# creare-com/pydem

Hardware: AMD Instinct MI355X
Metric: Mcells/s (slope+aspect+UCA+TWI end-to-end) per tile; % HBM roofline (higher is better)
Workload: dtype f64

## Files before the change

pydem_amd/csrc/internal.h:

```cpp
#pragma once
#include <hip/hip_runtime.h>
#include <stdint.h>
#include <stdio.h>
#include <stdlib.h>
#include <string>
#include <vector>
#include <utility>
#include <initializer_list>
#include "../../include/pydem_hip.h"

void pydem_set_error(const char *fmt, ...);
#define HIP_TRY(expr)                                                                          \
    do {                                                                                       \
        hipError_t e_ = (expr);                                                                \
        if (e_ != hipSuccess) {                                                                \
            pydem_set_error("%s:%d: %s -> %s", __FILE__, __LINE__, #expr, hipGetErrorString(e_)); \
            return -1;                                                                         \
        }                                                                                      \
    } while (0)
#define PYDEM_TRY(expr)            \
    do {                           \
        int r_ = (expr);           \
        if (r_ != 0) return r_;    \
    } while (0)

__host__ __device__ constexpr int fe1r(int k) { return k == 1 || k == 2 ? -1 : (k == 5 || k == 6 ? 1 : 0); }
__host__ __device__ constexpr int fe1c(int k) { return k == 0 || k == 7 ? 1 : (k == 3 || k == 4 ? -1 : 0); }
__host__ __device__ constexpr int fe2r(int k) { return k <= 3 ? -1 : 1; }
__host__ __device__ constexpr int fe2c(int k) { return (k == 0 || k == 1 || k == 6 || k == 7) ? 1 : -1; }

struct RowTab {
    double dX, dY;
    double hyp;
    double thA;
    double thB;
    double rdX, rdY, rhyp;
};

struct PitGraph {
    int32_t *raw_src = nullptr, *raw_dst = nullptr; double *raw_w = nullptr;
    int64_t raw_cap = 0, n_raw = 0;
    int64_t n_edges = 0, sorted_cap = 0;
    int32_t *src = nullptr, *dst = nullptr; double *w = nullptr;
    int32_t *in_src = nullptr, *in_dst = nullptr; double *in_w = nullptr;
    void *sort_buf = nullptr; size_t sort_bytes = 0;
};

struct TileBlock { void **slot; size_t bytes; bool cached; };

struct pydem_tile {
    int64_t n = 0, m = 0, NN = 0;
    int device = 0;
    hipStream_t stream = nullptr;
    hipStream_t stream2 = nullptr;
    hipEvent_t ev_fork = nullptr, ev_join = nullptr, ev_snap = nullptr;
    hipEvent_t ev[8] = {};
    double *elev = nullptr, *mag = nullptr, *dir = nullptr, *prop = nullptr, *uca = nullptr, *twi = nullptr;
    double *weight = nullptr, *uca_w = nullptr;
    uint8_t *flats = nullptr, *edge_todo = nullptr, *edge_done = nullptr, *flat0 = nullptr;
    int8_t *section = nullptr;
    bool have[PYDEM_FIELD_COUNT] = {};
    double *dX = nullptr, *dY = nullptr, *dX2 = nullptr, *dY2 = nullptr;
    RowTab *rowtab = nullptr;
    double *sec_theta = nullptr;
    double *row_area = nullptr;
    std::vector<double> h_dX, h_dY, h_dX2, h_dY2;
    bool spacing_set = false;
    int stencil_exact_only = 0;
    bool elev_f32 = false;
    int elev_dtype = 0;
    uint8_t *todo_work = nullptr;
    double *contrib = nullptr;
    uint32_t *cinfo = nullptr;
    int32_t *queue[2] = {nullptr, nullptr}, *labels = nullptr, *flatlist = nullptr;
    int32_t *counters = nullptr;
    int32_t *h_counters = nullptr;
    PitGraph pits;
    int32_t *estamp = nullptr; double *edelta = nullptr, *p_delta = nullptr, *s_data = nullptr;
    uint8_t *p_flags = nullptr, *s_flags = nullptr;
    int32_t eepoch = 0;
    int32_t *eseed = nullptr;
    bool edge_clean = false;
    bool einc_compact = false;
    void *nd_rec = nullptr; size_t nd_bytes = 0; int32_t nd = 0;
    int64_t circular_cells = -1;
    int64_t einc_round = 0;
    bool einc_ready = false;
    std::vector<std::pair<int, int64_t>> watch;
    size_t watch_built = 0;
    bool cond_live = false;
    bool cond_pending = false;
    int32_t cond_nw = 0, cond_nan_cap = 0;
    void *cond_mem = nullptr; size_t cond_bytes = 0;
    void *cond_node = nullptr, *cond_edge = nullptr; double *cond_slot = nullptr;
    int32_t *cond_q0 = nullptr, *cond_q1 = nullptr, *cond_nanq = nullptr, *cond_cnt = nullptr;
    void *cb_mem[3] = {nullptr, nullptr, nullptr}; size_t cb_bytes[3] = {0, 0, 0};
    double *h_strip_d = nullptr; uint8_t *h_strip_f = nullptr; size_t h_strip_cap = 0;
    void *h_stage = nullptr; size_t h_stage_bytes = 0;
    int32_t etodo_prev = 0;
    double *line_stage = nullptr;
    void *lines_stage = nullptr; size_t lines_bytes = 0;
    bool graph_valid = false;
    int flats_state = 0;
    int64_t find_flats_full = 0, find_flats_patch = 0, find_flats_elided = 0;
    bool pit_stash_live = false;
    pydem_options graph_opt = {};
    double *dd_out = nullptr; int32_t *dd_queue = nullptr; uint8_t *dd_mask = nullptr;
    double *ra_seed = nullptr;
    double *fa_mult = nullptr, *fa_cap = nullptr, *fa_inflow = nullptr;
    int32_t *sn_recv = nullptr; uint8_t *sn_code = nullptr;
    uint8_t *ta_sc = nullptr;
    int32_t *dd_ctr = nullptr, *dd_h_ctr = nullptr;
    hipEvent_t dd_ev[2] = {nullptr, nullptr};
    void *scratch = nullptr; size_t scratch_bytes = 0;
    std::vector<pydem_depression> depr;
    std::vector<TileBlock> blocks;
    int64_t device_bytes = 0;
    pydem_timings tm = {};
};

struct ArenaLease {
    int device = -1;
    void *arena = nullptr;
    char *base = nullptr; size_t bytes = 0, off = 0, want = 0;
    std::vector<void *> extra;
    bool held = false;
    ~ArenaLease();
};
int arena_acquire(int device, ArenaLease *L);
void *arena_take(ArenaLease *L, size_t bytes);

int ensure_fields(pydem_tile *t, std::initializer_list<int> fields);
void *plane_take(int device, size_t bytes);
void plane_give(int device, void *q);
hipError_t dev_malloc(void **p, size_t bytes);
void dev_free(void *p);
void devmem_release_all();
struct DevTemp {
    void *p = nullptr;
    ~DevTemp() { dev_free(p); }
    int alloc(size_t bytes) { if (bytes == 0) bytes = 8; HIP_TRY(dev_malloc(&p, bytes)); return 0; }
    template <typename T> T *as() { return (T *)p; }
};
int tile_pinned(pydem_tile *t, size_t bytes, void **out);
int tile_plane_copy(pydem_tile *t, void *dev, void *host, size_t bytes, bool to_host);

int stage_stencil(pydem_tile *t);
int stage_flats(pydem_tile *t);
int stage_section_graph(pydem_tile *t, const pydem_options *opt);
int stage_pits(pydem_tile *t, const pydem_options *opt);
int stage_sweep(pydem_tile *t, const pydem_options *opt);
int stage_uca_weighted(pydem_tile *t, const pydem_options *opt, int scale_by_cell_area);
int stage_twi(pydem_tile *t, const pydem_options *opt);
int stage_edge_update(pydem_tile *t, const pydem_options *opt, const double *const data[4], const uint8_t *const done[4],
                      const uint8_t *const todo[4]);
// ... 38 lines not shown
```

pydem_amd/csrc/tile.hip:

```cpp
#include "internal.h"
#include "uca_graph.h"
#include <cmath>
#include <stdarg.h>
#include <string.h>

static thread_local char g_err[1024] = "";

void pydem_set_error(const char *fmt, ...)
{
    va_list ap;
    va_start(ap, fmt);
    vsnprintf(g_err, sizeof(g_err), fmt, ap);
    va_end(ap);
}

namespace {

template <typename T>
__global__ void k_line_gather(const T *__restrict__ src, int64_t stride, int64_t count, T *__restrict__ dst)
{
    for (int64_t k = (int64_t)blockIdx.x * blockDim.x + threadIdx.x; k < count; k += (int64_t)gridDim.x * blockDim.x) dst[k] = src[k * stride];
}
template <typename T>
__global__ void k_line_scatter(const T *__restrict__ src, int64_t stride, int64_t count, T *__restrict__ dst)
// ... 61 lines not shown
        case PYDEM_F32: return 4;
        case PYDEM_I16: return 2;
        case PYDEM_I32: return 4;
        case PYDEM_U8: return 1;
        case PYDEM_I8: return 1;
    }
    return 0;
}

int field_ptr(pydem_tile *t, int field, void ***pp, size_t *elem)
{
    switch (field) {
        case PYDEM_ELEV: *pp = (void **)&t->elev; *elem = 8; return 0;
        case PYDEM_MAG: *pp = (void **)&t->mag; *elem = 8; return 0;
        case PYDEM_DIRECTION: *pp = (void **)&t->dir; *elem = 8; return 0;
        case PYDEM_FLATS: *pp = (void **)&t->flats; *elem = 1; return 0;
        case PYDEM_SECTION: *pp = (void **)&t->section; *elem = 1; return 0;
        case PYDEM_PROPORTION: *pp = (void **)&t->prop; *elem = 8; return 0;
        case PYDEM_UCA: *pp = (void **)&t->uca; *elem = 8; return 0;
        case PYDEM_TWI: *pp = (void **)&t->twi; *elem = 8; return 0;
        case PYDEM_EDGE_TODO: *pp = (void **)&t->edge_todo; *elem = 1; return 0;
        case PYDEM_EDGE_DONE: *pp = (void **)&t->edge_done; *elem = 1; return 0;
        case PYDEM_WEIGHT: *pp = (void **)&t->weight; *elem = 8; return 0;
        case PYDEM_UCA_WEIGHTED: *pp = (void **)&t->uca_w; *elem = 8; return 0;
    }
    pydem_set_error("unknown field id %d", field);
    return -2;
}

int ensure_field(pydem_tile *t, int field)
{
    void **pp; size_t elem;
    PYDEM_TRY(field_ptr(t, field, &pp, &elem));
    if (elem == 8) return tile_alloc(t, (double **)pp, (size_t)t->NN);
    return tile_alloc(t, (uint8_t **)pp, (size_t)t->NN);
}

}

int ensure_fields(pydem_tile *t, std::initializer_list<int> fields)
{
    for (int f : fields) PYDEM_TRY(ensure_field(t, f));
    return 0;
}

extern "C" {

const char *pydem_hip_last_error(void) { return g_err; }

int pydem_hip_release_scratch(void)
{
    devmem_release_all();
    return 0;
}

int pydem_hip_device_count(int *count)
{
    HIP_TRY(hipGetDeviceCount(count));
    return 0;
}

int pydem_hip_device_memory(int device, int64_t *free_bytes, int64_t *total_bytes)
{
    size_t f = 0, tot = 0;
    HIP_TRY(hipSetDevice(device));
    HIP_TRY(hipMemGetInfo(&f, &tot));
    if (free_bytes) *free_bytes = (int64_t)f;
    if (total_bytes) *total_bytes = (int64_t)tot;
    return 0;
}

int pydem_hip_device_name(int device, char *buf, int buflen)
{
    hipDeviceProp_t p;
    HIP_TRY(hipGetDeviceProperties(&p, device));
    snprintf(buf, buflen, "%s (%s, %d CUs)", p.name, p.gcnArchName, p.multiProcessorCount);
    return 0;
}

static int tile_init(pydem_tile *t)
{
    HIP_TRY(hipStreamCreateWithFlags(&t->stream, hipStreamNonBlocking));
    HIP_TRY(hipStreamCreateWithFlags(&t->stream2, hipStreamNonBlocking));
    HIP_TRY(hipEventCreateWithFlags(&t->ev_fork, hipEventDisableTiming));
    HIP_TRY(hipEventCreateWithFlags(&t->ev_join, hipEventDisableTiming));
    HIP_TRY(hipEventCreateWithFlags(&t->ev_snap, hipEventDisableTiming));
    for (int i = 0; i < 8; i++) HIP_TRY(hipEventCreate(&t->ev[i]));
    PYDEM_TRY(tile_alloc(t, &t->counters, 64));
    HIP_TRY(hipHostMalloc((void **)&t->h_counters, 64 * sizeof(int32_t), hipHostMallocDefault));
    return 0;
}

int pydem_tile_create(int64_t n_rows, int64_t n_cols, int device, pydem_tile **out)
{
    if (n_rows < 3 || n_cols < 3) { pydem_set_error("tile must be at least 3x3 (got %lld x %lld)", (long long)n_rows, (long long)n_cols); return -2; }
    if (n_rows * n_cols >= (int64_t)INT32_MAX) { pydem_set_error("tile too large for int32 cell ids"); return -2; }
    HIP_TRY(hipSetDevice(device));
    pydem_tile *t = new pydem_tile();
    t->n = n_rows; t->m = n_cols; t->NN = n_rows * n_cols; t->device = device;
    const int rc = tile_init(t);
    if (rc != 0) { pydem_tile_destroy(t); return rc; }
    *out = t;
    return 0;
}

int pydem_tile_destroy(pydem_tile *t)
{
    if (!t) return 0;
    (void)hipSetDevice(t->device);
    if (t->stream) (void)hipStreamSynchronize(t->stream);
    if (t->stream2) (void)hipStreamSynchronize(t->stream2);
    tile_release_all(t);
    if (t->h_counters) (void)hipHostFree(t->h_counters);
    if (t->h_strip_d) (void)hipHostFree(t->h_strip_d);
    if (t->h_stage) (void)hipHostFree(t->h_stage);
    if (t->h_strip_f) (void)hipHostFree(t->h_strip_f);
    if (t->dd_h_ctr) (void)hipHostFree(t->dd_h_ctr);
    for (int i = 0; i < 2; i++) if (t->dd_ev[i]) (void)hipEventDestroy(t->dd_ev[i]);
    for (int i = 0; i < 8; i++) if (t->ev[i]) (void)hipEventDestroy(t->ev[i]);
    if (t->ev_fork) (void)hipEventDestroy(t->ev_fork);
    if (t->ev_join) (void)hipEventDestroy(t->ev_join);
    if (t->ev_snap) (void)hipEventDestroy(t->ev_snap);
    if (t->stream2) { (void)hipStreamSynchronize(t->stream2); (void)hipStreamDestroy(t->stream2); }
    if (t->stream) (void)hipStreamDestroy(t->stream);
    delete t;
    return 0;
}

int pydem_tile_set_spacing(pydem_tile *t, const double *dX, const double *dY, const double *dX2, const double *dY2)
{
    HIP_TRY(hipSetDevice(t->device));
    const int64_t n = t->n;
    for (int64_t r = 0; r < n - 1; r++)
        if (!(dX[r] > 0 && dY[r] > 0 && std::isfinite(dX[r]) && std::isfinite(dY[r]))) {
            pydem_set_error("pydem_tile_set_spacing: dX / dY must be finite and > 0 (row %lld: %g, %g)", (long long)r, dX[r], dY[r]);
            return -2;
        }
    for (int64_t r = 0; r < n; r++)
        if (!(dX2[r] * dY2[r] > 0 && std::isfinite(dX2[r] * dY2[r]))) {
            pydem_set_error("pydem_tile_set_spacing: dX2 * dY2 (cell area) must be finite and > 0 (row %lld: %g, %g)", (long long)r, dX2[r], dY2[r]);
            return -2;
        }
    t->h_dX.assign(dX, dX + n - 1); t->h_dY.assign(dY, dY + n - 1);
    t->h_dX2.assign(dX2, dX2 + n); t->h_dY2.assign(dY2, dY2 + n);
    std::vector<RowTab> tab((size_t)(n - 1));
    int exotic = 0;
    for (int64_t r = 0; r < n - 1; r++) {
        RowTab &e = tab[(size_t)r];
        e.dX = dX[r]; e.dY = dY[r];
        e.hyp = sqrt(dX[r] * dX[r] + dY[r] * dY[r]);
        e.thA = atan2(dY[r], dX[r]);
        e.thB = atan2(dX[r], dY[r]);
        e.rdX = 1.0 / e.dX; e.rdY = 1.0 / e.dY; e.rhyp = 1.0 / e.hyp;
        if (!(e.dX > 0x1p-500 && e.dX < 0x1p500 && e.dY > 0x1p-500 && e.dY < 0x1p500 && e.hyp < 0x1p500)) exotic = 1;
    }
    { const char *ev = getenv("PYDEM_STENCIL_EXACT"); if (ev && *ev == '1') exotic = 1; }
    t->stencil_exact_only = exotic;
    std::vector<double> st((size_t)n);
    for (int64_t i = 0; i < n; i++) {
        int64_t r = i - 1;
        if (r < 0) r = 0;
        if (r > n - 3) r = n - 3;
        st[(size_t)i] = atan2(dY[r], dX[r]);
    }
    PYDEM_TRY(tile_alloc(t, &t->dX, (size_t)n)); PYDEM_TRY(tile_alloc(t, &t->dY, (size_t)n));
    PYDEM_TRY(tile_alloc(t, &t->dX2, (size_t)n)); PYDEM_TRY(tile_alloc(t, &t->dY2, (size_t)n));
    PYDEM_TRY(tile_alloc(t, &t->rowtab, (size_t)n)); PYDEM_TRY(tile_alloc(t, &t->sec_theta, (size_t)n));
    HIP_TRY(hipMemcpyAsync(t->dX, dX, (n - 1) * 8, hipMemcpyHostToDevice, t->stream));
    HIP_TRY(hipMemcpyAsync(t->dY, dY, (n - 1) * 8, hipMemcpyHostToDevice, t->stream));
    HIP_TRY(hipMemcpyAsync(t->dX2, dX2, n * 8, hipMemcpyHostToDevice, t->stream));
    HIP_TRY(hipMemcpyAsync(t->dY2, dY2, n * 8, hipMemcpyHostToDevice, t->stream));
    HIP_TRY(hipMemcpyAsync(t->rowtab, tab.data(), (n - 1) * sizeof(RowTab), hipMemcpyHostToDevice, t->stream));
    HIP_TRY(hipMemcpyAsync(t->sec_theta, st.data(), n * 8, hipMemcpyHostToDevice, t->stream));
    HIP_TRY(hipStreamSynchronize(t->stream));
    t->spacing_set = true;
    return 0;
}

int pydem_tile_upload(pydem_tile *t, int field, const void *src, int dtype)
{
    HIP_TRY(hipSetDevice(t->device));
    if (t->einc_ready && field != PYDEM_UCA) PYDEM_TRY(stage_edge_flush(t));
    t->edge_clean = false;
    t->einc_ready = false;
    void **pp; size_t elem;
    PYDEM_TRY(field_ptr(t, field, &pp, &elem));
    PYDEM_TRY(ensure_field(t, field));
    const size_t ds = dtype_size(dtype);
    if (!ds) { pydem_set_error("unknown dtype %d", dtype); return -2; }
    if (ds == elem && (elem == 1 || dtype == PYDEM_F64)) {
        PYDEM_TRY(tile_plane_copy(t, *pp, const_cast<void *>(src), (size_t)t->NN * elem, false));
    } else {
        if (elem != 8) { pydem_set_error("dtype conversion is only supported for float64 fields"); return -2; }
        const size_t bytes = (size_t)t->NN * ds;
        PYDEM_TRY(tile_reserve(t, &t->scratch, &t->scratch_bytes, bytes, bytes, false));
        PYDEM_TRY(tile_plane_copy(t, t->scratch, const_cast<void *>(src), bytes, false));
        const int grid = (int)(cdiv(t->NN, 256) < 8192 ? cdiv(t->NN, 256) : 8192);
        double *dst = (double *)*pp;
        switch (dtype) {
            case PYDEM_F32: hipLaunchKernelGGL(k_convert_to_f64<float>, dim3(grid), dim3(256), 0, t->stream, (const float *)t->scratch, dst, t->NN); break;
            case PYDEM_I16: hipLaunchKernelGGL(k_convert_to_f64<int16_t>, dim3(grid), dim3(256), 0, t->stream, (const int16_t *)t->scratch, dst, t->NN); break;
            case PYDEM_I32: hipLaunchKernelGGL(k_convert_to_f64<int32_t>, dim3(grid), dim3(256), 0, t->stream, (const int32_t *)t->scratch, dst, t->NN); break;
            case PYDEM_U8: hipLaunchKernelGGL(k_convert_to_f64<uint8_t>, dim3(grid), dim3(256), 0, t->stream, (const uint8_t *)t->scratch, dst, t->NN); break;
            case PYDEM_I8: hipLaunchKernelGGL(k_convert_to_f64<int8_t>, dim3(grid), dim3(256), 0, t->stream, (const int8_t *)t->scratch, dst, t->NN); break;
            default: pydem_set_error("bad dtype"); return -2;
// ... 201 lines not shown
int pydem_depressions_table(pydem_tile *t, int64_t rows, pydem_depression *table)
{
    if (rows != (int64_t)t->depr.size() || (rows > 0 && !table)) {
        pydem_set_error("pydem_depressions_table: %lld rows asked, the last pydem_depressions kept %lld", (long long)rows, (long long)t->depr.size());
        return -2;
    }
    if (rows > 0) memcpy(table, t->depr.data(), (size_t)rows * sizeof(pydem_depression));
    return 0;
}

int pydem_pit_candidates(pydem_tile *t, int below_sea, int64_t *npits)
{
    HIP_TRY(hipSetDevice(t->device));
    PYDEM_TRY(need(t, PYDEM_ELEV, "pydem_pit_candidates"));
    t->flats_state = 0;
    return stage_pit_candidates(t, below_sea, npits);
}

int pydem_pit_candidates_read(pydem_tile *t, int64_t npits, int32_t *cells, double *elev)
{
    HIP_TRY(hipSetDevice(t->device));
    return stage_pit_candidates_read(t, npits, cells, elev);
}

int pydem_pit_paths(pydem_tile *t, const int32_t *order, int64_t npits, int max_iter, int max_dist, double max_dist_XY,
                    int64_t *n_failed, int64_t *iter_used, int64_t *rounds, int *needs_host)
{
    t->edge_clean = false;
    t->einc_ready = false;
    HIP_TRY(hipSetDevice(t->device));
    PYDEM_TRY(need(t, PYDEM_ELEV, "pydem_pit_paths"));
    const int dtype_mode = t->elev_dtype == PYDEM_F64 ? 0 : (t->elev_dtype == PYDEM_F32 ? 2 : 1);
    t->graph_valid = false;
    t->flats_state = 0;
    const int r = stage_pit_paths(t, order, npits, max_iter, max_dist, max_dist_XY, n_failed, iter_used, rounds, dtype_mode);
    if (r < 0) return r;
    if (needs_host) *needs_host = r;
    for (int f = PYDEM_MAG; f < PYDEM_FIELD_COUNT; f++) t->have[f] = false;
    return 0;
}

int pydem_find_flats(pydem_tile *t)
{
    t->edge_clean = false;
    HIP_TRY(hipSetDevice(t->device));
    PYDEM_TRY(need(t, PYDEM_MAG, "pydem_find_flats"));
    const bool had_flats = t->flats != nullptr;
    PYDEM_TRY(ensure_field(t, PYDEM_FLATS));
    const bool lean = step_lean();
    if (lean && had_flats && t->have[PYDEM_FLATS] && t->flats_state == 1) {
        t->find_flats_elided++;
    } else if (lean && had_flats && t->have[PYDEM_FLATS] && t->flats_state == 2) {
        if (t->pits.n_raw > 0) {
            const int64_t g = cdiv(t->pits.n_raw, 256);
            hipLaunchKernelGGL(k_find_flats_pits, dim3((unsigned)(g < 1024 ? g : 1024)), dim3(256), 0, t->stream,
                               (const int32_t *)t->pits.raw_src, t->pits.n_raw, t->flats);
            HIP_TRY(hipGetLastError());
        }
        t->find_flats_patch++;
    } else {
        const int grid = (int)(cdiv(t->NN, 256) < 8192 ? cdiv(t->NN, 256) : 8192);
        hipLaunchKernelGGL(k_find_flats, dim3(grid), dim3(256), 0, t->stream, t->mag, t->flats, t->NN);
        HIP_TRY(hipGetLastError());
        if (!lean) HIP_TRY(hipStreamSynchronize(t->stream));
        t->find_flats_full++;
    }
    t->flats_state = 1;
    t->have[PYDEM_FLATS] = true;
    return 0;
}

int pydem_uca(pydem_tile *t, pydem_options *opt)
{
    t->edge_clean = false;
    t->einc_ready = false;
    HIP_TRY(hipSetDevice(t->device));
    PYDEM_TRY(need(t, PYDEM_ELEV, "pydem_uca"));
    PYDEM_TRY(need(t, PYDEM_MAG, "pydem_uca"));
    PYDEM_TRY(need(t, PYDEM_DIRECTION, "pydem_uca"));
    PYDEM_TRY(need(t, PYDEM_FLATS, "pydem_uca"));
    if (!t->spacing_set) { pydem_set_error("pydem_uca: call pydem_tile_set_spacing first"); return -3; }
    PYDEM_TRY(ensure_fields(t, {PYDEM_SECTION, PYDEM_PROPORTION, PYDEM_UCA, PYDEM_EDGE_TODO, PYDEM_EDGE_DONE}));
    t->pit_stash_live = step_lean();
    {
        const int rc = stage_section_graph(t, opt);
        if (rc != 0) { t->pit_stash_live = false; return rc; }
    }
    t->graph_valid = true;
    {
        const int rc = stage_sweep(t, opt);
        t->pit_stash_live = false;
        if (rc != 0) return rc;
    }
    double mn = opt->twi_min_area;
    for (int64_t i = 0; i < t->n; i++) {
        const double a = t->h_dX2[(size_t)i] * t->h_dY2[(size_t)i];
        if (a < mn) mn = a;
    }
    opt->twi_min_area = mn;
    t->have[PYDEM_SECTION] = t->have[PYDEM_PROPORTION] = t->have[PYDEM_UCA] = true;
    t->have[PYDEM_EDGE_TODO] = t->have[PYDEM_EDGE_DONE] = true;
    return 0;
}

static int ensure_graph(pydem_tile *t, pydem_options *opt, const char *who)
{
    if (t->graph_valid) return 0;
    PYDEM_TRY(need(t, PYDEM_ELEV, who));
    PYDEM_TRY(need(t, PYDEM_MAG, who));
    PYDEM_TRY(need(t, PYDEM_DIRECTION, who));
    if (!t->spacing_set) { pydem_set_error("%s: call pydem_tile_set_spacing first", who); return -3; }
    PYDEM_TRY(ensure_fields(t, {PYDEM_SECTION, PYDEM_PROPORTION}));
    t->pit_stash_live = false;
    PYDEM_TRY(stage_section_graph(t, opt));
    t->graph_valid = true;
    t->have[PYDEM_SECTION] = t->have[PYDEM_PROPORTION] = true;
    return 0;
}

static bool same_graph_options(const pydem_options &a, const pydem_options &b)
{
    if (!a.drain_pits && !b.drain_pits) return true;
    const bool xy = (a.drain_pits_max_dist_XY == b.drain_pits_max_dist_XY) ||
                    (a.drain_pits_max_dist_XY != a.drain_pits_max_dist_XY && b.drain_pits_max_dist_XY != b.drain_pits_max_dist_XY);
    return a.drain_pits == b.drain_pits && a.drain_pits_min_border == b.drain_pits_min_border &&
           a.drain_pits_max_iter == b.drain_pits_max_iter && a.drain_pits_max_dist == b.drain_pits_max_dist && xy;
}

int pydem_uca_weighted(pydem_tile *t, pydem_options *opt, int scale_by_cell_area)
{
    HIP_TRY(hipSetDevice(t->device));
    PYDEM_TRY(need(t, PYDEM_WEIGHT, "pydem_uca_weighted"));
    const pydem_timings keep = t->tm;
    const bool own_graph = !t->graph_valid || !same_graph_options(t->graph_opt, *opt);
    DevTemp save, planes;
    struct Kept { void *dst; size_t bytes; size_t off; };
    std::vector<Kept> kept;
    int32_t *save_cells = nullptr;
    double *save_vals = nullptr;
    int64_t nsave = 0;
    if (own_graph) {
        PYDEM_TRY(need(t, PYDEM_FLATS, "pydem_uca_weighted"));
        PYDEM_TRY(need(t, PYDEM_MAG, "pydem_uca_weighted"));
        PYDEM_TRY(ensure_fields(t, {PYDEM_EDGE_TODO, PYDEM_EDGE_DONE}));
        unsigned long long *cnt = reinterpret_cast<unsigned long long *>(t->counters + CS_FLAT_SAVE);
        const int g = (int)(cdiv(t->NN, 256) < 4096 ? cdiv(t->NN, 256) : 4096);
        HIP_TRY(hipMemsetAsync(cnt, 0, 8, t->stream));
        hipLaunchKernelGGL(k_flat_save, dim3(g), dim3(256), 0, t->stream, (const uint8_t *)t->flats, (const double *)t->mag, t->NN,
                           (int32_t *)nullptr, (double *)nullptr, (int64_t)0, cnt);
        unsigned long long hn = 0;
        HIP_TRY(hipMemcpyAsync(&hn, cnt, 8, hipMemcpyDeviceToHost, t->stream));
        HIP_TRY(hipStreamSynchronize(t->stream));
        nsave = (int64_t)hn;
        if (nsave > 0) {
            PYDEM_TRY(save.alloc((size_t)nsave * 12));
            save_vals = (double *)save.p;
            save_cells = (int32_t *)((char *)save.p + (size_t)nsave * 8);
            HIP_TRY(hipMemsetAsync(cnt, 0, 8, t->stream));
            hipLaunchKernelGGL(k_flat_save, dim3(g), dim3(256), 0, t->stream, (const uint8_t *)t->flats, (const double *)t->mag, t->NN,
                               save_cells, save_vals, nsave, cnt);
            HIP_TRY(hipGetLastError());
        }
        size_t off = 0;
        if (t->have[PYDEM_SECTION]) { kept.push_back({t->section, (size_t)t->NN, off}); off += (size_t)t->NN; }
        if (t->have[PYDEM_EDGE_TODO]) { kept.push_back({t->edge_todo, (size_t)t->NN, off}); off += (size_t)t->NN; }
        off = (off + 255) & ~(size_t)255;
        if (t->have[PYDEM_PROPORTION]) { kept.push_back({t->prop, (size_t)t->NN * 8, off}); off += (size_t)t->NN * 8; }
        if (off) PYDEM_TRY(planes.alloc(off));
        for (const Kept &k : kept)
// ... 165 lines not shown
```

pydem_amd/csrc/uca.hip:

```cpp
#include "uca_graph.h"
#include <algorithm>
#include <vector>
#include <math.h>
#include <stdlib.h>
#include <string.h>

#define PI_D 3.141592653589793

namespace {

__global__ __launch_bounds__(256) void k_section_proportion(const double *__restrict__ dir,
                                                            const uint8_t *__restrict__ flats,
                                                            const double *__restrict__ sec_theta, int64_t NN, int n, int m,
                                                            const double *__restrict__ elev,
                                                            int8_t *__restrict__ section, double *__restrict__ prop,
                                                            uint32_t *__restrict__ cinfo)
{
    (void)NN;
    for (int i = blockIdx.y; i < n; i += gridDim.y)
    for (int j = blockIdx.x * blockDim.x + threadIdx.x; j < m; j += gridDim.x * blockDim.x) {
        const int64_t c = (int64_t)i * m + j;
        const double theta = sec_theta[i];
        const double d = dir[c];
        int sec0 = (int)(int8_t)(int)floor(d / PI_D * 2.0);
        const double quadrant = d - PI_D / 2.0 * (double)sec0;
        const int mod2 = sec0 & 1;
        int sec = sec0 * 2 + ((quadrant > theta) && mod2 == 0) + ((quadrant > (PI_D / 2 - theta)) && mod2 == 1);
        sec = (int)(int8_t)sec;
        const bool I1 = sec == 0 || sec == 1 || sec == 4 || sec == 5;
        const double cth = PI_D / 2 - theta;
        const double t1 = I1 ? theta : cth, t2 = I1 ? cth : theta;
        const bool lo = quadrant <= t1, hi = quadrant > t1;
        const double num = lo ? quadrant : quadrant - t1, den = lo ? t1 : t2;
        double p = (lo || hi) ? num / den : NAN;
        if (flats[c]) { sec = -1; p = NAN; }
        if (sec == 8) sec = 0;
        const int a = (sec & 1) ? -1 : 1;
        const double pf = (1 + a) / 2.0 - (double)a * p;
        prop[c] = pf;
        section[c] = (int8_t)sec;
        uint32_t gf = 0;
        if (sec >= 0 && sec <= 7) {
            const double z = elev[c];
            const int i1 = i + fe1r(sec), j1 = j + fe1c(sec), i2 = i + fe2r(sec), j2 = j + fe2c(sec);
            if (i1 >= 0 && i1 < n && j1 >= 0 && j1 < m && keep_edge(pf, elev[(int64_t)i1 * m + j1], z)) gf |= CI_OUT1;
            if (i2 >= 0 && i2 < n && j2 >= 0 && j2 < m && keep_edge(1 - pf, elev[(int64_t)i2 * m + j2], z)) gf |= CI_OUT2;
        }
        cinfo[c] = gf | ((uint32_t)(sec & 7) << CI_SEC_SHIFT);
    }
}

__global__ __launch_bounds__(256) void k_graph_inmask(const double *__restrict__ prop, const double *__restrict__ elev,
                                                      int n, int m, uint32_t *__restrict__ cinfo, uint8_t *__restrict__ todo0,
                                                      uint8_t *__restrict__ todo_work, double *__restrict__ corner_sums)
{
    for (int i = blockIdx.y; i < n; i += gridDim.y)
    for (int j = blockIdx.x * blockDim.x + threadIdx.x; j < m; j += gridDim.x * blockDim.x) {
        const int64_t c = (int64_t)i * m + j;
        const uint32_t cw = cinfo[c] & (CI_OUT1 | CI_OUT2 | (7u << CI_SEC_SHIFT));
        uint32_t im = 0;
#pragma unroll
        for (int d = 0; d < 8; d++) {
            const int ui = i + NB_DI[d], uj = j + NB_DJ[d];
            if (ui < 0 || ui >= n || uj < 0 || uj >= m) continue;
            const uint32_t wu = cinfo[(int64_t)ui * m + uj];
            const int su = (int)((wu >> CI_SEC_SHIFT) & 7u);
            const bool cardinal = (NB_DI[d] == 0) || (NB_DJ[d] == 0);
            if ((su == NB_S0[d] || su == NB_S1[d]) && (wu & (cardinal ? CI_OUT1 : CI_OUT2))) im |= 1u << d;
        }
        cinfo[c] = im | cw | ((im ? CI_LEVEL_INF : 0u) << CI_LEVEL_SHIFT);
        const bool top = i == 0, bot = i == n - 1, left = j == 0, right = j == m - 1;
        if (top || bot || left || right) {
            const double TOL = 1e-2;
            const double p = prop[c], z = elev[c];
            double outsum = 0.0;
            if (cw & CI_OUT1) outsum += p;
            if (cw & CI_OUT2) outsum += 1 - p;
            const int s = (cw & (CI_OUT1 | CI_OUT2)) ? ci_section(cw) : -1;
            bool td = false;
            const bool has_out = outsum > TOL;
            if (left) td = has_out && (s == 6 || s == 7 || s == 0 || s == 1);
            if (right) td = has_out && (s == 2 || s == 3 || s == 4 || s == 5);
            if (top) td = has_out && (s == 4 || s == 5 || s == 6 || s == 7);
            if (bot) td = has_out && (s == 0 || s == 1 || s == 2 || s == 3);
            if ((top || bot) && (left || right)) {
                double insum = 0.0;
                for (int d = 0; d < 8; d++)
                    if (im & (1u << d)) {
                        const int64_t u = (int64_t)(i + NB_DI[d]) * m + (j + NB_DJ[d]);
                        const bool cardinal = (NB_DI[d] == 0) || (NB_DJ[d] == 0);
                        insum += cardinal ? prop[u] : 1 - prop[u];
                    }
                const int q = (top ? 0 : 2) + (left ? 0 : 1);
                corner_sums[q * 3 + 0] = outsum;
                corner_sums[q * 3 + 1] = insum;
                corner_sums[q * 3 + 2] = td ? 1.0 : 0.0;
            }
            if (isnan(z)) td = false;
            todo0[c] = td;
            todo_work[c] = td;
        }
    }
}

template <bool STASH>
__global__ void k_graph_add_pits(const int32_t *__restrict__ src, const int32_t *__restrict__ dst,
                                 const double *__restrict__ w, int64_t ne, int n, int m,
                                 uint32_t *cinfo, double *corner_sums, const int32_t *__restrict__ pin_dst, double *area)
{
    for (int64_t e = (int64_t)blockIdx.x * blockDim.x + threadIdx.x; e < ne; e += (int64_t)gridDim.x * blockDim.x) {
        const int32_t s = src[e], d = dst[e];
        if (STASH) {
            int32_t *slots = reinterpret_cast<int32_t *>(area);
            const int32_t pd = pin_dst[e];
            if (e == 0 || pin_dst[e - 1] != pd) slots[2 * (int64_t)pd] = (int32_t)e;
            if (e == 0 || src[e - 1] != s) slots[2 * (int64_t)s + 1] = (int32_t)e;
        }
        atomicOr(&cinfo[s], CI_PIT_OUT);
        atomicOr(&cinfo[d], CI_PIT_IN | (CI_LEVEL_INF << CI_LEVEL_SHIFT));
        const int corners[4] = {0, m - 1, (n - 1) * m, (n - 1) * m + m - 1};
        for (int q = 0; q < 4; q++) {
            if (s == corners[q]) atomicAdd(&corner_sums[q * 3 + 0], w[e]);
            if (d == corners[q]) atomicAdd(&corner_sums[q * 3 + 1], w[e]);
        }
    }
}

__global__ void k_corner_todo(const double *__restrict__ corner_sums, const double *__restrict__ elev, int n, int m,
                              uint8_t *todo0, uint8_t *todo_work)
{
    const int q = threadIdx.x;
    if (q >= 4) return;
    const int64_t corners[4] = {0, m - 1, (int64_t)(n - 1) * m, (int64_t)(n - 1) * m + m - 1};
    const int64_t c = corners[q];
    bool td = corner_sums[q * 3 + 2] != 0.0;
    td = td || (corner_sums[q * 3 + 0] > 1e-2) || (corner_sums[q * 3 + 1] < 1e-2);
    if (isnan(elev[c])) td = false;
    todo0[c] = td;
    todo_work[c] = td;
}

constexpr int STAGE_CAP = 4096;
constexpr int STAGE_FLUSH = STAGE_CAP - 512;


struct Stage {
    QE buf[STAGE_CAP];
    int32_t cnt;
    int32_t base;
};

__device__ __forceinline__ void stage_push(Stage &S, bool pred, int32_t cell, uint32_t cw)
{
    const unsigned long long bal = __ballot(pred);
    if (bal == 0ull) return;
    const int lane = (int)__lane_id();
    const int leader = __ffsll((long long)bal) - 1;
    int32_t base = 0;
    if (lane == leader) base = atomicAdd(&S.cnt, (int32_t)__popcll(bal));
    base = __shfl(base, leader);
    if (pred) { QE q; q.c = cell; q.cw = cw; S.buf[base + __popcll(bal & ((1ull << lane) - 1ull))] = q; }
}

__device__ __forceinline__ void stage_flush(const SweepArgs &A, Stage &S, QE *__restrict__ qn, int32_t *cn, bool force)
{
    __syncthreads();
    const int32_t c = S.cnt;
    if (c > 0 && (force || c > STAGE_FLUSH)) {
        if (threadIdx.x == 0) S.base = atomicAdd(cn, c);
        __syncthreads();
        const int32_t b = S.base;
        if ((int64_t)b + c <= A.qcap) { for (int32_t k = threadIdx.x; k < c; k += blockDim.x) qn[b + k] = S.buf[k]; }
        else if (threadIdx.x == 0) atomicAdd(A.err, 1);
        __syncthreads();
        if (threadIdx.x == 0) S.cnt = 0;
    }
    __syncthreads();
}

__device__ __forceinline__ int2 pit_stash(const SweepArgs &A, int32_t c) { return reinterpret_cast<const int2 *>(A.area)[c]; }

__global__ void k_pit_stash(const int32_t *__restrict__ pin_dst, const int32_t *__restrict__ pit_src, int64_t ne, double *area)
{
    int32_t *slots = reinterpret_cast<int32_t *>(area);
    for (int64_t e = (int64_t)blockIdx.x * blockDim.x + threadIdx.x; e < ne; e += (int64_t)gridDim.x * blockDim.x) {
        if (e == 0 || pin_dst[e - 1] != pin_dst[e]) slots[2 * (int64_t)pin_dst[e]] = (int32_t)e;
        if (e == 0 || pit_src[e - 1] != pit_src[e]) slots[2 * (int64_t)pit_src[e] + 1] = (int32_t)e;
    }
}

__device__ __forceinline__ void load_upstream_words(const SweepArgs &A, int32_t t, int ti, int tj, uint32_t w[8])
{
#pragma unroll
    for (int d = 0; d < 8; d++) {
        const int ii = ti + NB_DI[d], jj = tj + NB_DJ[d];
        const bool ok = ii >= 0 && ii < A.n && jj >= 0 && jj < A.m;
        w[d] = A.cinfo[ok ? t + NB_DI[d] * A.m + NB_DJ[d] : t];
    }
}

template <bool SPEC>
__device__ __forceinline__ bool owns_target(const SweepArgs &A, int32_t t, int32_t u, uint32_t r, uint32_t ct, const uint32_t w[8],
                                            int32_t in_start)
{
    int32_t owner = -1;
    bool ready = true;
#pragma unroll
    for (int d = 0; d < 8; d++) {
        if (ct & (1u << d)) {
            const int32_t v = t + NB_DI[d] * A.m + NB_DJ[d];
            const uint32_t lv = (v == u) ? r : ci_level(SPEC ? w[d] : A.cinfo[v]);
            ready = ready && (lv <= r);
            if (lv == r) owner = v > owner ? v : owner;
        }
    }
    if (ct & CI_PIT_IN) {
        for (int32_t e = in_start;; e += 4) {
            int32_t d4[4], s4[4];
#pragma unroll
            for (int k = 0; k < 4; k++) {
                const int64_t idx = e + k < A.n_pit ? e + k : A.n_pit - 1;
                d4[k] = A.pin_dst[idx]; s4[k] = A.pin_src[idx];
            }
            uint32_t l4[4];
            bool v4[4];
            bool more = true;
#pragma unroll
            for (int k = 0; k < 4; k++) {
                more = more && e + k < A.n_pit && d4[k] == t;
                v4[k] = more;
                l4[k] = (more && s4[k] != u) ? ci_level(A.cinfo[s4[k]]) : r;
            }
#pragma unroll
            for (int k = 0; k < 4; k++) {
                if (v4[k]) {
                    ready = ready && (l4[k] <= r);
                    if (l4[k] == r) owner = s4[k] > owner ? s4[k] : owner;
                }
            }
            if (!more) break;
        }
    }
    return ready && owner == u;
}

__device__ __forceinline__ void publish_cell(const SweepArgs &A, int32_t c, uint32_t cw, double acc, bool td)
{
    A.area[c] = acc;
    double2 o = make_double2(0.0, 0.0);
    if (cw & (CI_OUT1 | CI_OUT2)) {
        const double p = A.prop[c];
        if (cw & CI_OUT1) o.x = acc * p;
        if (cw & CI_OUT2) o.y = acc * (1 - p);
        if (td) { o.x = -o.x; o.y = -o.y; }
    }
    A.contrib[c] = o;
    if (td) A.todo_work[c] = 1;
}

__device__ __forceinline__ void gather_pit_edges(const SweepArgs &A, int32_t c, int32_t in_start, double &acc, bool &td)
{
    for (int32_t e = in_start;; e += 4) {
        int32_t d4[4], s4[4]; double w4[4];
#pragma unroll
        for (int k = 0; k < 4; k++) {
            const int64_t idx = e + k < A.n_pit ? e + k : A.n_pit - 1;
            d4[k] = A.pin_dst[idx]; s4[k] = A.pin_src[idx]; w4[k] = A.pin_w[idx];
        }
        double a4[4]; uint8_t t4[4];
        bool more = true;
#pragma unroll
        for (int k = 0; k < 4; k++) {
            more = more && e + k < A.n_pit && d4[k] == c;
            a4[k] = more ? A.area[s4[k]] : 0.0;
            t4[k] = more ? A.todo_work[s4[k]] : (uint8_t)0;
        }
        more = true;
#pragma unroll
        for (int k = 0; k < 4; k++) {
            more = more && e + k < A.n_pit && d4[k] == c;
            if (more) { acc += a4[k] * w4[k]; td = td || (t4[k] != 0); }
        }
        if (!more) break;
    }
}

template <bool LOWLAT, typename Push2, typename PushP>
__device__ __forceinline__ void process_cell(const SweepArgs &A, bool active, QE q, uint32_t r, Push2 push2, PushP pushp)
{
    const int32_t c = q.c;
    const uint32_t cw = q.cw;
    int32_t t1 = -1, t2 = -1;
    uint32_t c1 = 0, c2 = 0;
    bool r1 = false, r2 = false;
    int32_t out_start = -1;
    if (active) {
        const int m = A.m;
        const int i = c / m, j = c - i * m;
        const int sct = ci_section(cw);
        uint32_t l1[8], l2[8];
        int2 s1 = make_int2(-1, -1), s2 = make_int2(-1, -1), sc = make_int2(-1, -1);
        if (cw & CI_OUT1) {
            const int dr = fe1r(sct), dc = fe1c(sct);
            t1 = c + dr * m + dc; c1 = A.cinfo[t1];
            if (LOWLAT) { load_upstream_words(A, t1, i + dr, j + dc, l1); s1 = pit_stash(A, t1); }
        }
        if (cw & CI_OUT2) {
            const int dr = fe2r(sct), dc = fe2c(sct);
            t2 = c + dr * m + dc; c2 = A.cinfo[t2];
            if (LOWLAT) { load_upstream_words(A, t2, i + dr, j + dc, l2); s2 = pit_stash(A, t2); }
        }
        if (cw & (CI_PIT_IN | CI_PIT_OUT)) sc = pit_stash(A, c);
        double acc = A.a0[i];
        bool td = (i == 0 || i == A.n - 1 || j == 0 || j == m - 1) && A.todo_work[c] != 0;
#pragma unroll
        for (int d = 0; d < 8; d++) {
            if (cw & (1u << d)) {
                const int32_t u = c + NB_DI[d] * m + NB_DJ[d];
                const bool cardinal = (NB_DI[d] == 0) || (NB_DJ[d] == 0);
                const double x = cardinal ? A.contrib[u].x : A.contrib[u].y;
                acc += fabs(x);
                td = td || (x < 0);
            }
        }
        if (cw & CI_PIT_IN) gather_pit_edges(A, c, sc.x, acc, td);
        out_start = sc.y;
        publish_cell(A, c, cw, acc, td);
        if (t1 >= 0) {
            if (!LOWLAT && (c1 & CI_PIT_IN)) s1 = pit_stash(A, t1);
            r1 = owns_target<LOWLAT>(A, t1, c, r, c1, l1, s1.x);
        }
        if (t2 >= 0) {
            if (!LOWLAT && (c2 & CI_PIT_IN)) s2 = pit_stash(A, t2);
            r2 = owns_target<LOWLAT>(A, t2, c, r, c2, l2, s2.x);
        }
        if (r1) A.cinfo[t1] = ci_with_level(c1, r + 1);
        if (r2) A.cinfo[t2] = ci_with_level(c2, r + 1);
    }
    push2(r1, t1, c1);
    push2(r2, t2, c2);
    if (active && (cw & CI_PIT_OUT)) {
        for (int32_t e = out_start;; e += 4) {
            int32_t s4[4], t4[4];
#pragma unroll
            for (int k = 0; k < 4; k++) {
                const int64_t idx = e + k < A.n_pit ? e + k : A.n_pit - 1;
                s4[k] = A.pit_src[idx]; t4[k] = A.pit_dst[idx];
            }
            bool more = true;
            for (int k = 0; k < 4 && more; k++) {
                more = e + k < A.n_pit && s4[k] == c;
                if (!more) break;
                const int32_t t = t4[k];
                const uint32_t ct = A.cinfo[t];
                const int2 st = pit_stash(A, t);
                uint32_t lw[8];
                load_upstream_words(A, t, t / A.m, t % A.m, lw);
                if (owns_target<true>(A, t, c, r, ct, lw, st.x)) {
                    A.cinfo[t] = ci_with_level(ct, r + 1);
                    pushp(t, ct);
                }
            }
            if (!more) break;
        }
    }
}

#ifdef PYDEM_SWEEP_QUEUE
template <bool LOWLAT>
__global__ __launch_bounds__(256) void k_sweep_round(SweepArgs A, const QE *__restrict__ qc, QE *__restrict__ qn,
                                                     int32_t *cnt3, int r, int32_t *total)
{
    __shared__ Stage S;
    const int32_t nq = cnt3[r % 3];
    if (blockIdx.x == 0 && threadIdx.x == 0) { cnt3[(r + 2) % 3] = 0; if (nq) { atomicAdd(total, nq); atomicAdd(total + 2, 1); } }
    if (nq == 0) return;
    if (threadIdx.x == 0) S.cnt = 0;
    __syncthreads();
    int32_t *cn = &cnt3[(r + 1) % 3];
    for (int32_t base = blockIdx.x * blockDim.x; base < nq; base += gridDim.x * blockDim.x) {
        const int32_t q = base + threadIdx.x;
        const bool active = q < nq;
        QE qe; qe.c = 0; qe.cw = 0;
        if (active) qe = qc[q];
        process_cell<LOWLAT>(A, active, qe, (uint32_t)r,
                             [&](bool pred, int32_t t, uint32_t ct) { stage_push(S, pred, t, ct); },
                             [&](int32_t t, uint32_t ct) {
                                 const int32_t slot = atomicAdd(cn, 1);
                                 if (slot < A.qcap) { QE e; e.c = t; e.cw = ct; qn[slot] = e; }
                                 else atomicAdd(A.err, 1);
                             });
        stage_flush(A, S, qn, cn, false);
    }
    stage_flush(A, S, qn, cn, true);
}

constexpr int SWEEP_SMALL_CAP = 1024;

__global__ __launch_bounds__(1024) void k_sweep_small(SweepArgs A, QE *q0, QE *q1, int32_t *cnt3, int r_start, int r_max,
                                                      int32_t *total, int32_t *state)
{
    __shared__ int s_next;
    int r = r_start;
    int32_t nq = cnt3[r % 3];
    int32_t done = 0, rounds = 0;
    while (nq > 0 && nq <= SWEEP_SMALL_CAP && r < r_max) {
        if (threadIdx.x == 0) s_next = 0;
        __syncthreads();
        const QE *qc = (r % 2) ? q1 : q0;
        QE *qn = (r % 2) ? q0 : q1;
        for (int32_t base = 0; base < nq; base += blockDim.x) {
            const int32_t q = base + threadIdx.x;
            const bool active = q < nq;
            QE qe; qe.c = 0; qe.cw = 0;
            if (active) qe = qc[q];
            auto push = [&](int32_t t, uint32_t ct) {
                const int32_t slot = atomicAdd(&s_next, 1);
                if (slot < A.qcap) { QE e; e.c = t; e.cw = ct; qn[slot] = e; }
                else atomicAdd(A.err, 1);
            };
            process_cell<true>(A, active, qe, (uint32_t)r, [&](bool pred, int32_t t, uint32_t ct) { if (pred) push(t, ct); }, push);
        }
        __syncthreads();
        done += nq; rounds++;
        nq = s_next;
        r++;
        __syncthreads();
    }
    if (threadIdx.x == 0) {
        cnt3[r % 3] = nq; cnt3[(r + 1) % 3] = 0; cnt3[(r + 2) % 3] = 0;
        atomicAdd(total, done); atomicAdd(total + 2, rounds);
        state[0] = r;
    }
}

#endif

#ifndef PYDEM_TH
#define PYDEM_TH 32
#endif
constexpr int TT = 32;
constexpr int TH = PYDEM_TH, HH = TH + 2;
static_assert(TH == 32 || TH == 64, "tile height");
constexpr uint32_t SP_STATE_SHIFT = 14, SP_BLOCKED = 1u << 13;
#ifndef PYDEM_STG_B
#define PYDEM_STG_B 4
#endif
constexpr int TILE_RING = TH == 32 ? 256 : 512;

struct TileW {
    uint32_t cs[TH * TT];
    union {
        unsigned long long fin[HH];
        double a0[TH];
    };
    uint16_t list[TILE_RING];
    int tail;
    int limit;
};

__device__ __forceinline__ uint16_t &sp_of(TileW &L, int idx) { return reinterpret_cast<uint16_t *>(L.cs)[2 * idx]; }
__device__ __forceinline__ uint32_t sp_state(const TileW &L, int idx) { return (L.cs[idx] >> SP_STATE_SHIFT) & 3u; }

__device__ __forceinline__ uint32_t sp_dec(TileW &L, int idx) { return atomicSub(&L.cs[idx], 1u) & 0xFFFFu; }

__device__ __forceinline__ void tile_wave_sync()
{
    __builtin_amdgcn_fence(__ATOMIC_SEQ_CST, "workgroup");
    __builtin_amdgcn_wave_barrier();
}

__device__ __forceinline__ void tile_lds_sync()
{
    __builtin_amdgcn_fence(__ATOMIC_RELEASE, "workgroup", "local");
    __builtin_amdgcn_wave_barrier();
    __builtin_amdgcn_fence(__ATOMIC_ACQUIRE, "workgroup", "local");
}

constexpr int TILE_PEND = 48;
struct TileNext {
    int32_t *flag;
    int32_t *list, *count;
};

__device__ __forceinline__ const double *in_edge_ptr(const SweepArgs &A, int32_t c, int m, int d)
{
    const int q = d + (d >> 2);
    const int di = (q * 11) >> 5;
    const int32_t u = c + (di - 1) * m + (q - 3 * di - 1);
    return reinterpret_cast<const double *>(A.contrib + u) + (((0x5A >> d) & 1) ? 0 : 1);
}
__device__ __forceinline__ double in_edge(const SweepArgs &A, int32_t c, int m, int d) { return *in_edge_ptr(A, c, m, d); }

struct TileBase {
    const char *cinfo, *area, *contrib, *prop, *todo;
    int32_t org;
};
__device__ __forceinline__ TileBase tile_base(const SweepArgs &A, int i0, int j0)
{
    TileBase B;
    const int64_t org = (int64_t)(i0 - 1) * A.m + (j0 - 1);
    B.org = (int32_t)org;
    B.cinfo = reinterpret_cast<const char *>(A.cinfo) + org * 4;
    B.area = reinterpret_cast<const char *>(A.area) + org * 8;
    B.contrib = reinterpret_cast<const char *>(A.contrib) + org * 16;
    B.prop = reinterpret_cast<const char *>(A.prop) + org * 8;
    B.todo = reinterpret_cast<const char *>(A.todo_work) + org;
    return B;
}
template <typename T>
__device__ __forceinline__ T ld_off(const char *base, uint32_t off) { return *reinterpret_cast<const T *>(base + (size_t)off); }
template <typename T>
__device__ __forceinline__ void st_off(const char *base, uint32_t off, T v) { *reinterpret_cast<T *>(const_cast<char *>(base) + (size_t)off) = v; }
__device__ __forceinline__ uint32_t halo_cell(int li, int lj, int m) { return __umul24((uint32_t)li, (uint32_t)m) + (uint32_t)lj; }

__device__ __forceinline__ void fill_nbr16(int32_t *nbr16, int m)
{
    if (threadIdx.x < 8) {
        const int d = threadIdx.x, q = d + (d >> 2), di = q / 3, dj = q - 3 * di;
        nbr16[d] = ((di - 1) * m + (dj - 1)) * 16 + (((0x5A >> d) & 1) ? 0 : 8);
    }
}
__device__ __forceinline__ double in_edge_h(const TileBase &B, const int32_t *nbr16, uint32_t h, int d)
{
#ifdef PYDEM_EXP_AREAONLY
    const uint32_t off16 = h * 16u + (uint32_t)nbr16[d];
    const uint32_t uo = (off16 >> 4) * 8u;
    const double ua = ld_off<double>(B.area, uo), up = ld_off<double>(B.prop, uo);
    return (off16 & 8u) ? ua * (1 - up) : ua * up;
#else
    return ld_off<double>(B.contrib, h * 16u + (uint32_t)nbr16[d]);
#endif
}

__device__ __forceinline__ void tile_stage(const SweepArgs &A, const TileBase &B, TileW &L, uint32_t pass, int i0, int j0, int lane,
                                           uint32_t *hw = nullptr)
{
    const int n = A.n, m = A.m;
    const int half = lane >> 5, l32 = lane & 31;
    constexpr int NSET = TH * TT / 64;
    auto stage_word = [&](int gi, int gj) -> uint32_t {
        return (gi >= 0 && gi < n && gj >= 0 && gj < m) ? A.cinfo[(int64_t)gi * m + gj] : 0xFFFFFFFFu;
    };
    auto final_before = [&](uint32_t w) -> bool {
        if (w == 0xFFFFFFFFu) return true;
        const uint32_t lv = ci_level(w);
        return lv >= 1 && lv < pass;
    };
    unsigned long long colL, colR;
    {
        const uint32_t wr = stage_word(half ? i0 + TH : i0 - 1, j0 + l32);
        uint32_t wk = 0xFFFFFFFFu;
        if (lane < 4) wk = stage_word((lane & 2) ? i0 + TH : i0 - 1, (lane & 1) ? j0 + TT : j0 - 1);
        if (hw) {
            hw[(half ? TT + 2 : 0) + l32 + 1] = wr;
            if (lane < 4) hw[((lane & 2) ? TT + 2 : 0) + ((lane & 1) ? TT + 1 : 0)] = wk;
        }
        if (TH == 32) {
            const uint32_t wc = stage_word(i0 + l32, half ? j0 + TT : j0 - 1);
            if (hw) hw[2 * (TT + 2) + (half ? TH : 0) + l32] = wc;
            const unsigned long long bc = __ballot(final_before(wc));
            colL = bc & 0xFFFFFFFFull; colR = bc >> 32;
        } else {
            const uint32_t wl = stage_word(i0 + lane, j0 - 1), wq = stage_word(i0 + lane, j0 + TT);
            colL = __ballot(final_before(wl)); colR = __ballot(final_before(wq));
        }
        const bool fr = final_before(wr), fk = lane < 4 && final_before(wk);
        const unsigned long long br = __ballot(fr), bk = __ballot(fk);
        if (lane == 0) {
            L.fin[0] = ((br & 0xFFFFFFFFull) << 1) | (bk & 1ull) | (((bk >> 1) & 1ull) << 33);
            L.fin[HH - 1] = ((br >> 32) << 1) | ((bk >> 2) & 1ull) | (((bk >> 3) & 1ull) << 33);
        }
    }
    constexpr int STG_B = PYDEM_STG_B;
#pragma unroll 1
    for (int kb = 0; kb < NSET; kb += STG_B) {
        uint32_t wst[STG_B];
#pragma unroll
        for (int k = 0; k < STG_B; k++) wst[k] = stage_word(i0 + 2 * (kb + k) + half, j0 + l32);
#pragma unroll
        for (int k = 0; k < STG_B; k++) {
            const int r = 2 * (kb + k);
            const bool f = final_before(wst[k]);
            L.cs[lane + 64 * (kb + k)] = ((wst[k] == 0xFFFFFFFFu ? 0u : (wst[k] & CI_STATIC_MASK)) << 16) | ((f ? 1u : 0u) << SP_STATE_SHIFT);
            const unsigned long long b = __ballot(f);
            if (lane == 0) {
                L.fin[r + 1] = ((b & 0xFFFFFFFFull) << 1) | ((colL >> r) & 1ull) | (((colR >> r) & 1ull) << 33);
                L.fin[r + 2] = ((b >> 32) << 1) | ((colL >> (r + 1)) & 1ull) | (((colR >> (r + 1)) & 1ull) << 33);
            }
        }
    }
}

template <bool LISTED, bool WT = false>
__device__ __forceinline__ void sweep_one_tile(const SweepArgs &A, TileW &L, uint32_t pass, int tiles_x, int tid, int lane,
                                               uint8_t *__restrict__ tile_done, int32_t &n_final, const TileNext &N,
                                               int32_t *pend, int &npend, const int32_t *nbr16)
{
    const int by = tid / tiles_x, bx = tid - by * tiles_x;
    const int i0 = by * TH, j0 = bx * TT, n = A.n, m = A.m;
    const TileBase B = tile_base(A, i0, j0);
    const int half = lane >> 5, l32 = lane & 31;
    auto push_ready = [&](int cell, int consumed) {
        const int slot = atomicAdd(&L.tail, 1);
        if (slot - consumed < TILE_RING) L.list[slot % TILE_RING] = (uint16_t)cell;
        else atomicMin(&L.limit, slot);
    };
#ifdef PYDEM_TILE_PROF
    const bool prof = (A.dbg & 4) != 0 && (int)pass >= (A.dbg >> 8);
#else
    constexpr bool prof = false;
#endif
    long long tk0 = 0, tk1 = 0, tk2 = 0, tk3 = 0;
    int nrounds = 0;
    if (prof) tk0 = wall_clock64();
    if (lane == 0) { L.tail = 0; L.limit = INT32_MAX; }
    const double a0_row = (!WT && lane < TH && i0 + lane < n) ? A.a0[i0 + lane] : 0.0;
    constexpr int NSET = TH * TT / 64;
    tile_stage(A, B, L, pass, i0, j0, lane);
    tile_wave_sync();
    if (prof) tk1 = wall_clock64();
    uint32_t pitmask = 0;
    int32_t n_open = 0;
#pragma unroll 2
    for (int k = 0; k < NSET; k++) {
        const int li = 2 * k + half + 1, idx = lane + 64 * k;
        const uint32_t w = L.cs[idx];
        if (!((w >> SP_STATE_SHIFT) & 3u)) {
            const unsigned long long f0 = L.fin[li - 1], f1 = L.fin[li], f2 = L.fin[li + 1];
            const uint32_t nf = ((uint32_t)(f0 >> l32) & 7u) | (((uint32_t)(f1 >> l32) & 1u) << 3) |
                                (((uint32_t)(f1 >> (l32 + 2)) & 1u) << 4) | (((uint32_t)(f2 >> l32) & 7u) << 5);
            const uint32_t pend = __popc((w >> 16) & 0xFFu & ~nf);
            sp_of(L, idx) = (uint16_t)pend;
            n_open++;
            if (w & (CI_PIT_IN << 16)) pitmask |= 1u << k;
            else if (pend == 0) push_ready(lane + 64 * k, 0);
        }
    }
    if (pitmask) {
        constexpr int PB = 4;
#pragma unroll 1
        for (int kb = 0; kb < NSET; kb += PB) {
            if (!((pitmask >> kb) & ((1u << PB) - 1u))) continue;
            int32_t e0[PB];
#pragma unroll
            for (int k = 0; k < PB; k++) {
                e0[k] = 0;
                if (pitmask & (1u << (kb + k))) {
                    const int cell = lane + 64 * (kb + k);
                    e0[k] = ld_off<int2>(B.area, halo_cell((cell >> 5) + 1, (cell & 31) + 1, m) * 8u).x;
                }
            }
#pragma unroll
            for (int k = 0; k < PB; k++) {
                if (!(pitmask & (1u << (kb + k)))) continue;
                const int cell = lane + 64 * (kb + k);
                const int32_t c = B.org + (int32_t)halo_cell((cell >> 5) + 1, (cell & 31) + 1, m);
                const int idx = cell;
                uint32_t pend = sp_of(L, idx);
                for (int32_t e = e0[k];; e += 2) {
                    const int64_t ia = e < A.n_pit ? e : A.n_pit - 1, ib = e + 1 < A.n_pit ? e + 1 : A.n_pit - 1;
                    const int32_t da = A.pin_dst[ia], db = A.pin_dst[ib], sa = A.pin_src[ia], sb = A.pin_src[ib];
                    const bool va = e < A.n_pit && da == c, vb = va && e + 1 < A.n_pit && db == c;
                    auto blocked = [&](int32_t sc) -> uint32_t {
                        const int si = sc / m - i0, sj = sc % m - j0;
                        if (si >= 0 && si < TH && sj >= 0 && sj < TT)
                            return sp_state(L, si * TT + sj) ? 0u : 1u;
                        const uint32_t lv = ci_level(A.cinfo[sc]);
                        return (lv >= 1 && lv < pass) ? 0u : SP_BLOCKED;
                    };
                    uint32_t ba = 0, bb = 0;
                    if (va) ba = blocked(sa);
                    if (vb) bb = blocked(sb);
                    pend = (pend + (ba & 1u) + (bb & 1u)) | ((ba | bb) & SP_BLOCKED);
                    if (!vb) break;
                }
                sp_of(L, idx) = (uint16_t)pend;
                if (pend == 0) push_ready(cell, 0);
            }
        }
    }
    tile_wave_sync();
    if (lane < TH) L.a0[lane] = a0_row;
    tile_wave_sync();
    if (prof) tk2 = wall_clock64();
    int32_t finalized = 0;
    uint32_t wake = 0;
    int head = 0;
    int mycell = -1, cd = -1;
    double cv = 0.0;
    for (;;) {
        const int tail = L.tail < L.limit ? L.tail : L.limit;
        const bool need = mycell < 0;
        const unsigned long long nb = __ballot(need);
        const int rank = __builtin_amdgcn_mbcnt_hi((uint32_t)(nb >> 32), __builtin_amdgcn_mbcnt_lo((uint32_t)nb, 0u));
        const int avail = tail - head, wanted = __popcll(nb);
        if (need && rank < avail) { mycell = L.list[(head + rank) % TILE_RING]; cd = -1; }
        head += wanted < avail ? wanted : avail;
        if (!__ballot(mycell >= 0)) break;
        nrounds++;
        int next = -1, nd = -1;
        double nv = 0.0;
        if (mycell >= 0) {
            const int cell = mycell;
            const int li = (cell >> 5) + 1, lj = (cell & 31) + 1, idx = cell;
            const int gi = i0 + li - 1, gj = j0 + lj - 1;
            const uint32_t h = halo_cell(li, lj, m);
            const int32_t c = B.org + (int32_t)h;
            const uint32_t cw = L.cs[idx] >> 16;
            double pv = 0.0;
            if (cw & (CI_OUT1 | CI_OUT2)) pv = ld_off<double>(B.prop, h * 8u);
            int2 po = make_int2(0, 0);
            if (cw & (CI_PIT_IN | CI_PIT_OUT)) po = ld_off<int2>(B.area, h * 8u);
            uint32_t mm = cw & 0xFFu;
            double xs[4];
#pragma unroll
            for (int q = 0; q < 4; q++) {
                xs[q] = 0.0;
                if (mm) {
                    const int d = __ffs(mm) - 1; mm &= mm - 1u;
                    if (d == cd) xs[q] = cv; else xs[q] = in_edge_h(B, nbr16, h, d);
                }
            }
            double a;
            bool td;
            if constexpr (WT) {
                a = A.a0[c];
                td = false;
#pragma unroll
                for (int q = 0; q < 4; q++) a += xs[q];
            } else {
                a = L.a0[li - 1];
                td = (gi == 0 || gi == n - 1 || gj == 0 || gj == m - 1) && ld_off<uint8_t>(B.todo, h) != 0;
#pragma unroll
                for (int q = 0; q < 4; q++) { a += fabs(xs[q]); td = td || (xs[q] < 0); }
            }
            while (mm) {
                const int d = __ffs(mm) - 1; mm &= mm - 1u;
                const double x = (d == cd) ? cv : in_edge_h(B, nbr16, h, d);
                if constexpr (WT) a += x;
                else { a += fabs(x); td = td || (x < 0); }
            }
            if (cw & CI_PIT_IN)
                for (int32_t e = po.x; e < A.n_pit && A.pin_dst[e] == c; e++) {
                    const int32_t sc = A.pin_src[e];
                    a += A.area[sc] * A.pin_w[e];
                    if constexpr (!WT) td = td || (A.todo_work[sc] != 0);
                }
            double2 o = make_double2(0.0, 0.0);
            if (cw & CI_OUT1) o.x = a * pv;
            if (cw & CI_OUT2) o.y = a * (1 - pv);
            if (td) { o.x = -o.x; o.y = -o.y; }
            st_off<double>(B.area, h * 8u, a);
#ifndef PYDEM_EXP_NOCONTRIB
            st_off<double2>(B.contrib, h * 16u, o);
#endif
            if (LISTED) st_off<uint32_t>(B.cinfo, h * 4u, ci_with_level(cw, pass));
            if (td) st_off<uint8_t>(B.todo, h, (uint8_t)1);
            sp_of(L, idx) = (uint16_t)(2u << SP_STATE_SHIFT);
            finalized++;
            auto release = [&](int ti, int tj, double share, bool chainable) {
                if (ti >= 1 && ti <= TH && tj >= 1 && tj <= TT) {
                    const int tcell = (ti - 1) * TT + (tj - 1);
                    if (sp_dec(L, tcell) == 1u) {
                        if (chainable && next < 0) {
                            const int q = (li - ti + 1) * 3 + (lj - tj + 1);
                            next = tcell; nd = q - (q > 4 ? 1 : 0); nv = share;
                        } else push_ready(tcell, head);
                    }
                } else if (LISTED) {
                    const int dti = ti < 1 ? -1 : (ti > TH ? 1 : 0), dtj = tj < 1 ? -1 : (tj > TT ? 1 : 0);
                    if (ti >= 1 - TH && ti <= 2 * TH && tj >= 1 - TT && tj <= 2 * TT) wake |= 1u << ((dti + 1) * 3 + dtj + 1);
                    else {
                        const int tt = ((i0 + ti - 1) / TH) * tiles_x + (j0 + tj - 1) / TT;
                        if (atomicExch(&N.flag[tt], (int32_t)pass + 1) != (int32_t)pass + 1) N.list[atomicAdd(N.count, 1)] = tt;
                    }
                }
            };
            const int sct = ci_section(cw);
            if (cw & CI_OUT1) release(li + fe1r(sct), lj + fe1c(sct), o.x, true);
            if (cw & CI_OUT2) release(li + fe2r(sct), lj + fe2c(sct), o.y, true);
            if (cw & CI_PIT_OUT)
                for (int32_t e = po.y; e < A.n_pit && A.pit_src[e] == c; e++) {
                    const int32_t dc = A.pit_dst[e];
                    const int ti = dc / m - i0 + 1, tj = dc % m - j0 + 1;
                    release(ti, tj, 0.0, false);
                }
        }
        mycell = next; cd = nd; cv = nv;
        tile_wave_sync();
    }
    if (prof) tk3 = wall_clock64();
    if (!LISTED)
        for (int k = 0; k < NSET; k++) {
            const int li = 2 * k + half + 1, idx = lane + 64 * k;
            const uint32_t w = L.cs[idx];
            if (((w >> SP_STATE_SHIFT) & 3u) == 2u) A.cinfo[(int64_t)(i0 + li - 1) * m + j0 + l32] = ci_with_level(w >> 16, pass);
        }
    for (int off = 32; off > 0; off >>= 1) { finalized += __shfl_down(finalized, off); n_open += __shfl_down(n_open, off); }
    if (LISTED) {
        for (int off = 32; off > 0; off >>= 1) wake |= __shfl_xor(wake, off);
        bool win = false;
        int tt = 0;
        if (lane < 9 && ((wake >> lane) & 1u)) { tt = tid + (lane / 3 - 1) * tiles_x + (lane % 3 - 1); win = true; }
        if (lane == 9 && L.limit != INT32_MAX) { tt = tid; win = true; }
        if (win) win = atomicExch(&N.flag[tt], (int32_t)pass + 1) != (int32_t)pass + 1;
        const unsigned long long bw = __ballot(win);
        if (win) pend[npend + __popcll(bw & ((1ull << lane) - 1ull))] = tt;
        npend += __popcll(bw);
    }
    if (lane == 0) {
        n_final += finalized;
        if (finalized == n_open) tile_done[tid] = 1;
        A.tile_open[tid] = n_open - finalized;
        if (prof) {
            const long long tk4 = wall_clock64();
            unsigned long long *acc = reinterpret_cast<unsigned long long *>(A.err + (CS_TILE_PROF - CS_QUEUE_ERR));
            atomicAdd(acc + 0, (unsigned long long)(tk1 - tk0)); atomicAdd(acc + 1, (unsigned long long)(tk2 - tk1));
            atomicAdd(acc + 2, (unsigned long long)(tk3 - tk2)); atomicAdd(acc + 3, (unsigned long long)(tk4 - tk3));
            atomicAdd(acc + 4, (unsigned long long)nrounds); atomicAdd(acc + 5, 1ull);
            if (finalized == 0) atomicAdd(acc + 6, 1ull);
        }
    }
    tile_wave_sync();
}

#include "uca_sym.inl"

#ifndef PYDEM_SWEEP_STEAL
#define PYDEM_SWEEP_STEAL 1
#endif
#ifndef PYDEM_FULL_WPB
#define PYDEM_FULL_WPB 4
#endif
constexpr int FWPB = PYDEM_FULL_WPB;
template <bool LISTED, bool WT = false>
__global__ __launch_bounds__(64 * FWPB, 32 / FWPB) void k_sweep_tiles(SweepArgs A, uint32_t pass, int tiles_x, int tiles_total,
                                                     uint8_t *__restrict__ tile_done, int32_t *n_final, TileNext N, int32_t *work8)
{
    __shared__ TileW L[FWPB];
    __shared__ int32_t s_pend[FWPB][TILE_PEND];
    __shared__ int32_t s_nbr16[8];
    fill_nbr16(s_nbr16, A.m);
    __syncthreads();
    const int wave = __builtin_amdgcn_readfirstlane(threadIdx.x >> 6), lane = threadIdx.x & 63;
    int32_t fin = 0;
    int npend = 0;
    auto flush = [&]() {
        tile_wave_sync();
        int32_t base = 0;
        if (lane == 0) base = atomicAdd(N.count, npend);
        base = __shfl(base, 0);
        if (lane < npend) N.list[base + lane] = s_pend[wave][lane];
        npend = 0;
        tile_wave_sync();
    };
#ifdef PYDEM_SWEEP_STATIC
    (void)work8;
    const int per4 = (gridDim.x >> 3) * 4;
    for (int tid = (blockIdx.x & 7) * per4 + (blockIdx.x >> 3) * 4 + wave, once = 0; once < 1; once++) {
        if (tid < tiles_total && !tile_done[tid])
            sweep_one_tile<LISTED, WT>(A, L[wave], pass, tiles_x, tid, lane, tile_done, fin, N, s_pend[wave], npend, s_nbr16);
    }
#else
    const int per = (tiles_total + 7) >> 3;
    for (int st = 0; st < PYDEM_SWEEP_STEAL; st++) {
        const int xcd = (int)((blockIdx.x + st) & 7);
        for (;;) {
            int32_t q = 0;
            if (lane == 0) q = atomicAdd(&work8[xcd], 1);
            q = __builtin_amdgcn_readfirstlane(__shfl(q, 0));
            const int tid = xcd * per + q;
            if (q >= per || tid >= tiles_total) break;
            if (tile_done[tid]) continue;
            sweep_one_tile<LISTED, WT>(A, L[wave], pass, tiles_x, tid, lane, tile_done, fin, N, s_pend[wave], npend, s_nbr16);
            if (LISTED && npend > TILE_PEND - 10) flush();
        }
    }
#endif
    if (LISTED && npend) flush();
    if (lane == 0 && fin) atomicAdd(n_final, fin);
}

#ifndef PYDEM_LISTED_OCC
#define PYDEM_LISTED_OCC 6
#endif
#ifndef PYDEM_LISTED_WPB
#define PYDEM_LISTED_WPB 2
#endif
constexpr int LWPB = PYDEM_LISTED_WPB;
template <bool WT = false>
__global__ __launch_bounds__(64 * LWPB, PYDEM_LISTED_OCC) void k_sweep_tiles_listed(SweepArgs A, uint32_t pass, int tiles_x, const int32_t *__restrict__ list_in,
                                                            const int32_t *n_in, uint8_t *__restrict__ tile_done, int32_t *n_final,
                                                            TileNext N, int32_t *clear_count, int32_t *work3, SymArgs Y)
{
    __shared__ TileW L[LWPB];
    __shared__ SymLight SL[LWPB];
    const int wave = threadIdx.x >> 6, lane = threadIdx.x & 63;
    const int32_t nt = *n_in;
#ifdef PYDEM_LISTED_DYNAMIC
    if (blockIdx.x == 0 && threadIdx.x < 8) work3[((pass + 1) % 3) * 8 + threadIdx.x] = 0;
#endif
    if (blockIdx.x == 0 && threadIdx.x == 0) *clear_count = 0;
    __shared__ int32_t s_pend[LWPB][TILE_PEND];
    __shared__ int32_t s_nbr16[8];
    fill_nbr16(s_nbr16, A.m);
    __syncthreads();
    int32_t fin = 0;
    int npend = 0;
    auto flush = [&]() {
        tile_wave_sync();
        int32_t base = 0;
        if (lane == 0) base = atomicAdd(N.count, npend);
        base = __shfl(base, 0);
        if (lane < npend) N.list[base + lane] = s_pend[wave][lane];
        npend = 0;
        tile_wave_sync();
    };
#ifndef PYDEM_LISTED_DYNAMIC
    (void)work3;
    for (int32_t k = __builtin_amdgcn_readfirstlane(blockIdx.x * LWPB + wave); k < nt; k += gridDim.x * LWPB) {
#else
    const int xcd = blockIdx.x & 7;
    const int32_t per = (nt + 7) >> 3;
    int32_t *wk = &work3[(pass % 3) * 8 + xcd];
    for (;;) {
        int32_t k = 0;
        if (lane == 0) k = atomicAdd(wk, 1);
        k = __builtin_amdgcn_readfirstlane(__shfl(k, 0));
        (void)per;
        k = k * 8 + xcd;
        if (k >= nt) break;
#endif
        const int tid = __builtin_amdgcn_readfirstlane(list_in[k]);
        const uint32_t blk = Y.tile_sym ? __builtin_amdgcn_readfirstlane(Y.tile_sym[tid]) : SYM_NONE;
        if (blk != SYM_NONE) sym_light_visit<WT>(A, Y, SL[wave], pass, tiles_x, tid, lane, blk, fin, N, s_pend[wave], npend);
        else sweep_one_tile<true, WT>(A, L[wave], pass, tiles_x, tid, lane, tile_done, fin, N, s_pend[wave], npend, s_nbr16);
        if (npend > TILE_PEND - 10) flush();
    }
    if (npend) flush();
    if (lane == 0 && fin) atomicAdd(n_final, fin);
}

constexpr int DENSE_BAND = 64;
__global__ __launch_bounds__(256) void k_sweep_dense_level(SweepArgs A, uint32_t p, int32_t *n_final)
{
    const int n = A.n, m = A.m;
    int32_t fin = 0;
    const int j = blockIdx.x * blockDim.x + threadIdx.x;
    const int i_end = min(n, (int)(blockIdx.y + 1) * DENSE_BAND);
    if (j < m)
    for (int i = blockIdx.y * DENSE_BAND; i < i_end; i++) {
        const int32_t c = i * m + j;
        const uint32_t w = A.cinfo[c];
        const uint32_t lv = ci_level(w);
        if (lv >= 1 && lv != CI_LEVEL_INF) continue;
        const uint32_t cw = w & CI_STATIC_MASK;
        bool ready = true;
#pragma unroll
        for (int d = 0; d < 8; d++)
            if (cw & (1u << d)) {
                const uint32_t lu = ci_level(A.cinfo[c + NB_DI[d] * m + NB_DJ[d]]);
                ready = ready && lu >= 1 && lu < p;
            }
        if (!ready) continue;
        int2 po = make_int2(0, 0);
        if (cw & CI_PIT_IN) {
            po = pit_stash(A, c);
            for (int32_t e = po.x; e < A.n_pit && A.pin_dst[e] == c; e++) {
                const uint32_t lu = ci_level(A.cinfo[A.pin_src[e]]);
                ready = ready && lu >= 1 && lu < p;
            }
            if (!ready) continue;
        }
        double a = A.a0[i];
        bool td = (i == 0 || i == n - 1 || j == 0 || j == m - 1) && A.todo_work[c] != 0;
#pragma unroll
        for (int d = 0; d < 8; d++)
            if (cw & (1u << d)) { const double x = in_edge(A, c, m, d); a += fabs(x); td = td || (x < 0); }
        if (cw & CI_PIT_IN)
            for (int32_t e = po.x; e < A.n_pit && A.pin_dst[e] == c; e++) {
                const int32_t sc = A.pin_src[e];
                a += A.area[sc] * A.pin_w[e];
                td = td || (A.todo_work[sc] != 0);
            }
        double2 o = make_double2(0.0, 0.0);
        if (cw & (CI_OUT1 | CI_OUT2)) {
            const double pv = A.prop[c];
            if (cw & CI_OUT1) o.x = a * pv;
            if (cw & CI_OUT2) o.y = a * (1 - pv);
            if (td) { o.x = -o.x; o.y = -o.y; }
        }
        A.area[c] = a;
        A.contrib[c] = o;
        A.cinfo[c] = ci_with_level(cw, p);
        if (td) A.todo_work[c] = 1;
        fin++;
    }
    for (int off = 32; off > 0; off >>= 1) fin += __shfl_down(fin, off);
    __shared__ int32_t s_fin;
    if (threadIdx.x == 0) s_fin = 0;
    __syncthreads();
    if ((threadIdx.x & 63) == 0 && fin) atomicAdd(&s_fin, fin);
    __syncthreads();
    if (threadIdx.x == 0 && s_fin) atomicAdd(n_final, s_fin);
}

constexpr int RCAP = 256;
constexpr uint32_t RS_TAINT = 1u << 19, RS_FIN = 1u << 20;
constexpr int RS_OPEN_SHIFT = 11, RS_FINAL_SHIFT = 21;
constexpr uint32_t RS_CELL = (1u << RS_OPEN_SHIFT) - 1u, RS_CELL_OPEN = (1u << 19) - 1u;

struct TileR {
    TileW W;
    uint16_t map[TH * TT];
    double Kd[RCAP];
    double Pd[RCAP];
    uint32_t sm[RCAP];
};

__device__ __forceinline__ int nb_local(int cell, int d)
{
    const int q = d + (d >> 2);
    const int di = (q * 11) >> 5;
    return cell + (di - 1) * TT + (q - 3 * di - 1);
}

template <bool WT = false>
__device__ __forceinline__ void sweep_tile_resident(const SweepArgs &A, TileR &R, uint32_t pass, int tiles_x, int tid, int lane,
                                                    uint8_t *__restrict__ tile_done, int32_t &n_final, const TileNext &N,
                                                    int32_t *pend, int &npend)
{
    TileW &L = R.W;
    const int by = tid / tiles_x, bx = tid - by * tiles_x;
    const int i0 = by * TH, j0 = bx * TT, n = A.n, m = A.m;
    const int half = lane >> 5, l32 = lane & 31;
    constexpr int NSET = TH * TT / 64;
    if (lane == 0) L.tail = 0;
    const double a0_row = (!WT && lane < TH && i0 + lane < n) ? A.a0[i0 + lane] : 0.0;
    tile_stage(A, tile_base(A, i0, j0), L, pass, i0, j0, lane);
    tile_wave_sync();
    uint32_t pitmask = 0;
    int nslot = 0;
#pragma unroll 2
    for (int k = 0; k < NSET; k++) {
        const int li = 2 * k + half + 1, idx = lane + 64 * k;
        const uint32_t w = L.cs[idx];
        const bool open = !((w >> SP_STATE_SHIFT) & 3u);
        const unsigned long long bo = __ballot(open);
        if (open) {
            const unsigned long long f0 = L.fin[li - 1], f1 = L.fin[li], f2 = L.fin[li + 1];
            const uint32_t nf = ((uint32_t)(f0 >> l32) & 7u) | (((uint32_t)(f1 >> l32) & 1u) << 3) |
                                (((uint32_t)(f1 >> (l32 + 2)) & 1u) << 4) | (((uint32_t)(f2 >> l32) & 7u) << 5);
            const uint32_t im = (w >> 16) & 0xFFu;
            const uint32_t cnt = __popc(im & ~nf);
            sp_of(L, idx) = (uint16_t)cnt;
            const int s = nslot + __popcll(bo & ((1ull << lane) - 1ull));
            R.map[idx] = (uint16_t)s;
            R.sm[s] = (uint32_t)idx | ((im & ~nf) << RS_OPEN_SHIFT) | ((im & nf) << RS_FINAL_SHIFT);
            if (w & (CI_PIT_IN << 16)) pitmask |= 1u << k;
            else if (cnt == 0) L.list[atomicAdd(&L.tail, 1)] = (uint16_t)s;
        }
        nslot += __popcll(bo);
    }
    if (pitmask) {
#pragma unroll 1
        for (int k = 0; k < NSET; k++) {
            if (!(pitmask & (1u << k))) continue;
            const int cell = lane + 64 * k;
            const int32_t c = (i0 + (cell >> 5)) * m + j0 + (cell & 31);
            uint32_t cnt = sp_of(L, cell);
            for (int32_t e = pit_stash(A, c).x; e < A.n_pit && A.pin_dst[e] == c; e++) {
                const int32_t sc = A.pin_src[e];
                const int si = sc / m - i0, sj = sc % m - j0;
                if (si >= 0 && si < TH && sj >= 0 && sj < TT) cnt += sp_state(L, si * TT + sj) ? 0u : 1u;
                else { const uint32_t lv = ci_level(A.cinfo[sc]); if (!(lv >= 1 && lv < pass)) cnt |= SP_BLOCKED; }
            }
            sp_of(L, cell) = (uint16_t)cnt;
            if (cnt == 0) L.list[atomicAdd(&L.tail, 1)] = R.map[cell];
        }
    }
    tile_wave_sync();
    if (lane < TH) L.a0[lane] = a0_row;
    tile_wave_sync();
    for (int s = lane; s < nslot; s += 64) {
        uint32_t smv = R.sm[s];
        const int cell = smv & RS_CELL;
        const int gi = i0 + (cell >> 5), gj = j0 + (cell & 31);
        const int32_t c = gi * m + gj;
        const uint32_t cw = L.cs[cell] >> 16;
        double pv = 0.0;
        if (cw & (CI_OUT1 | CI_OUT2)) pv = A.prop[c];
        bool td = !WT && (gi == 0 || gi == n - 1 || gj == 0 || gj == m - 1) && A.todo_work[c] != 0;
        uint32_t mm = (smv >> RS_FINAL_SHIFT) & 0xFFu;
        double xs[4];
#pragma unroll
        for (int q = 0; q < 4; q++) {
            xs[q] = 0.0;
            if (mm) { const int d = __ffs(mm) - 1; mm &= mm - 1u; xs[q] = in_edge(A, c, m, d); }
        }
        double K;
        if constexpr (WT) {
            K = A.a0[c];
#pragma unroll
            for (int q = 0; q < 4; q++) K += xs[q];
            while (mm) { const int d = __ffs(mm) - 1; mm &= mm - 1u; K += in_edge(A, c, m, d); }
        } else {
            K = L.a0[cell >> 5];
#pragma unroll
            for (int q = 0; q < 4; q++) { K += fabs(xs[q]); td = td || (xs[q] < 0); }
            while (mm) { const int d = __ffs(mm) - 1; mm &= mm - 1u; const double x = in_edge(A, c, m, d); K += fabs(x); td = td || (x < 0); }
        }
        R.Kd[s] = K; R.Pd[s] = pv;
        R.sm[s] = (smv & RS_CELL_OPEN) | (td ? RS_TAINT : 0u);
    }
    tile_lds_sync();
    uint32_t wake = 0;
    int head = 0;
    for (;;) {
        const int tail = L.tail;
        if (head >= tail) break;
        const int idx = head + lane;
        if (idx < tail) {
            const int s = L.list[idx];
            const uint32_t smv = R.sm[s];
            const int cell = smv & RS_CELL, li = cell >> 5, lj = cell & 31;
            const uint32_t cw = L.cs[cell] >> 16;
            double a = R.Kd[s];
            bool td = (smv & RS_TAINT) != 0u;
            uint32_t mm = (smv >> RS_OPEN_SHIFT) & 0xFFu;
            while (mm) {
                const int d = __ffs(mm) - 1; mm &= mm - 1u;
                const int ss = R.map[nb_local(cell, d)];
                const double as = R.Kd[ss], ps = R.Pd[ss];
                a += ((0x5A >> d) & 1) ? as * ps : as * (1 - ps);
                td = td || (R.sm[ss] & RS_TAINT);
            }
            const int32_t c = (i0 + li) * m + j0 + lj;
            int2 po = make_int2(0, 0);
            if (cw & (CI_PIT_IN | CI_PIT_OUT)) po = pit_stash(A, c);
            if (cw & CI_PIT_IN)
                for (int32_t e = po.x; e < A.n_pit && A.pin_dst[e] == c; e++) {
                    const int32_t sc = A.pin_src[e];
                    const int si = sc / m - i0, sj = sc % m - j0;
                    bool here = false;
                    if (si >= 0 && si < TH && sj >= 0 && sj < TT) here = sp_state(L, si * TT + sj) == 2u;
                    if (here) { const int ss = R.map[si * TT + sj]; a += R.Kd[ss] * A.pin_w[e]; td = td || (R.sm[ss] & RS_TAINT); }
                    else { a += A.area[sc] * A.pin_w[e]; if constexpr (!WT) td = td || (A.todo_work[sc] != 0); }
                }
            R.Kd[s] = a;
            R.sm[s] = (smv & RS_CELL) | (td ? RS_TAINT : 0u) | RS_FIN;
            sp_of(L, cell) = (uint16_t)(2u << SP_STATE_SHIFT);
            auto release = [&](int ti, int tj) {
                if (ti >= 0 && ti < TH && tj >= 0 && tj < TT) {
                    const int tcell = ti * TT + tj;
                    if (sp_dec(L, tcell) == 1u) L.list[atomicAdd(&L.tail, 1)] = R.map[tcell];
                } else {
                    const int dti = ti < 0 ? -1 : (ti >= TH ? 1 : 0), dtj = tj < 0 ? -1 : (tj >= TT ? 1 : 0);
                    if (ti >= -TH && ti < 2 * TH && tj >= -TT && tj < 2 * TT) wake |= 1u << ((dti + 1) * 3 + dtj + 1);
                    else {
                        const int tt = ((i0 + ti) / TH) * tiles_x + (j0 + tj) / TT;
                        if (atomicExch(&N.flag[tt], (int32_t)pass + 1) != (int32_t)pass + 1) N.list[atomicAdd(N.count, 1)] = tt;
                    }
                }
            };
            const int sct = ci_section(cw);
            if (cw & CI_OUT1) release(li + fe1r(sct), lj + fe1c(sct));
            if (cw & CI_OUT2) release(li + fe2r(sct), lj + fe2c(sct));
            if (cw & CI_PIT_OUT)
                for (int32_t e = po.y; e < A.n_pit && A.pit_src[e] == c; e++) {
                    const int32_t dc = A.pit_dst[e];
                    release(dc / m - i0, dc % m - j0);
                }
        }
        head = tail < head + 64 ? tail : head + 64;
        tile_lds_sync();
    }
    int nfin = 0;
    for (int s = lane; s < nslot; s += 64) {
        const uint32_t smv = R.sm[s];
        if (!(smv & RS_FIN)) continue;
        const int cell = smv & RS_CELL;
        const int32_t c = (i0 + (cell >> 5)) * m + j0 + (cell & 31);
        const uint32_t cw = L.cs[cell] >> 16;
        const double a = R.Kd[s], pv = R.Pd[s];
        double2 o = make_double2(0.0, 0.0);
        if (cw & CI_OUT1) o.x = a * pv;
        if (cw & CI_OUT2) o.y = a * (1 - pv);
        if (smv & RS_TAINT) { o.x = -o.x; o.y = -o.y; A.todo_work[c] = 1; }
        A.area[c] = a;
        A.contrib[c] = o;
        A.cinfo[c] = ci_with_level(cw, pass);
        nfin++;
    }
    for (int off = 32; off > 0; off >>= 1) { nfin += __shfl_down(nfin, off); wake |= __shfl_xor(wake, off); }
    bool win = false;
    int tt = 0;
    if (lane < 9 && ((wake >> lane) & 1u)) { tt = tid + (lane / 3 - 1) * tiles_x + (lane % 3 - 1); win = true; }
    if (win) win = atomicExch(&N.flag[tt], (int32_t)pass + 1) != (int32_t)pass + 1;
    const unsigned long long bw = __ballot(win);
    if (win) pend[npend + __popcll(bw & ((1ull << lane) - 1ull))] = tt;
    npend += __popcll(bw);
    if (lane == 0) {
        n_final += nfin;
        A.tile_open[tid] = nslot - nfin;
        if (nfin == nslot) tile_done[tid] = 1;
    }
    tile_wave_sync();
}

template <bool WT = false>
__global__ __launch_bounds__(64) void k_sweep_tiles_resident(SweepArgs A, uint32_t pass, int tiles_x, const int32_t *__restrict__ list_in,
                                                             const int32_t *n_in, uint8_t *__restrict__ tile_done, int32_t *n_final,
                                                             TileNext N, int32_t *clear_count, SymArgs Y)
{
    __shared__ TileR R;
    __shared__ SymLight SL;
    __shared__ int32_t s_pend[TILE_PEND];
    __shared__ int32_t s_nbr16[8];
    fill_nbr16(s_nbr16, A.m);
    __syncthreads();
    const int lane = threadIdx.x;
    const int32_t nt = *n_in;
    if (blockIdx.x == 0 && lane == 0) *clear_count = 0;
    int32_t fin = 0;
    int npend = 0;
    auto flush = [&]() {
        tile_wave_sync();
        int32_t base = 0;
        if (lane == 0) base = atomicAdd(N.count, npend);
        base = __shfl(base, 0);
        if (lane < npend) N.list[base + lane] = s_pend[lane];
        npend = 0;
        tile_wave_sync();
    };
    for (int32_t k = blockIdx.x; k < nt; k += gridDim.x) {
        const int tid = __builtin_amdgcn_readfirstlane(list_in[k]);
        const uint32_t blk = Y.tile_sym ? __builtin_amdgcn_readfirstlane(Y.tile_sym[tid]) : SYM_NONE;
        if (blk != SYM_NONE) sym_light_visit<WT>(A, Y, SL, pass, tiles_x, tid, lane, blk, fin, N, s_pend, npend);
        else if (__builtin_amdgcn_readfirstlane(A.tile_open[tid]) <= RCAP)
            sweep_tile_resident<WT>(A, R, pass, tiles_x, tid, lane, tile_done, fin, N, s_pend, npend);
        else
            sweep_one_tile<true, WT>(A, R.W, pass, tiles_x, tid, lane, tile_done, fin, N, s_pend, npend, s_nbr16);
        if (npend > TILE_PEND - 10) flush();
    }
    if (npend) flush();
    if (lane == 0 && fin) atomicAdd(n_final, fin);
}

constexpr uint32_t FC_COUNT = 0xFu, FC_BLOCKED = 1u << 8, FC_DONE = 1u << 9, FC_TODO = 1u << 10;

struct TileFirst {
    double2 slot[TT * TT];
    uint32_t cs[TT * TT];
    double a0[TT];
};

__device__ __forceinline__ void lds_sync()
{
    __builtin_amdgcn_fence(__ATOMIC_RELEASE, "workgroup", "local");
    __builtin_amdgcn_s_barrier();
    __builtin_amdgcn_fence(__ATOMIC_ACQUIRE, "workgroup", "local");
}

__global__ __launch_bounds__(256) void k_sweep_first(SweepArgs A, int tiles_x, int tiles_total, uint8_t *__restrict__ tile_done,
                                                     int32_t *n_final)
{
    __shared__ TileFirst L;
    __shared__ int32_t s_fin[2], s_any[2];
    const int t = threadIdx.x;
    const int per = gridDim.x >> 3;
    const int tid = (blockIdx.x & 7) * per + (blockIdx.x >> 3);
    if (tid >= tiles_total) return;
    const int by = tid / tiles_x, bx = tid - by * tiles_x;
    const int i0 = by * TT, j0 = bx * TT, n = A.n, m = A.m;
    const int r0 = t >> 5, l32 = t & 31;
    const int gj = j0 + l32;
    constexpr int NSET = TT * TT / 256;
    uint32_t ingrid = 0;
    if (t < 2) { s_fin[t] = 0; s_any[t] = 0; }
    {
        uint32_t cw[NSET];
        double pv[NSET];
#pragma unroll
        for (int k = 0; k < NSET; k++) {
            const int gi = i0 + 8 * k + r0;
            const bool ok = gi < n && gj < m;
            const int64_t c = (int64_t)gi * m + gj;
            cw[k] = ok ? A.cinfo[c] : 0xFFFFFFFFu;
            pv[k] = ok ? A.prop[c] : 0.0;
        }
        if (t < TT) L.a0[t] = (i0 + t < n) ? A.a0[i0 + t] : 0.0;
        const uint32_t out_col = (l32 == 0 ? 0x29u : 0u) | (l32 == TT - 1 ? 0x94u : 0u);
        const bool edge_col = gj == 0 || gj == m - 1;
#pragma unroll
        for (int k = 0; k < NSET; k++) {
            const int r = 8 * k + r0, gi = i0 + r;
            const uint32_t w = cw[k];
            uint32_t word = FC_BLOCKED;
            if (w != 0xFFFFFFFFu) {
                ingrid |= 1u << k;
                const uint32_t outside = out_col | (r == 0 ? 0x07u : 0u) | (r == TT - 1 ? 0xE0u : 0u);
                const bool blocked = ((w & 0xFFu & outside) != 0u) || (w & (CI_PIT_IN | CI_PIT_OUT));
                word = ((w & CI_STATIC_MASK) << 16) | __popc(w & 0xFFu) | (blocked ? FC_BLOCKED : 0u);
                if (!blocked && (edge_col || gi == 0 || gi == n - 1) && A.todo_work[(int64_t)gi * m + gj] != 0) word |= FC_TODO;
            }
            L.cs[t + 256 * k] = word;
            L.slot[t + 256 * k].x = pv[k];
        }
    }
    lds_sync();
    int ph = 0;
    for (;;) {
        uint32_t ready = 0;
#pragma unroll
        for (int k = 0; k < NSET; k++)
            if ((L.cs[t + 256 * k] & (FC_COUNT | FC_BLOCKED | FC_DONE)) == 0u) ready |= 1u << k;
        if (ready) s_any[ph] = 1;
        lds_sync();
        const bool go = s_any[ph] != 0;
        if (t == 0) s_any[ph ^ 1] = 0;
        ph ^= 1;
        if (!go) break;
        while (ready) {
            const int k = __ffs(ready) - 1; ready &= ready - 1u;
            int cur = t + 256 * k;
            do {
                const int r = cur >> 5, cl = cur & 31;
                const uint32_t word = L.cs[cur], w = word >> 16;
                const double pv = L.slot[cur].x;
                double a = L.a0[r];
                bool td = (word & FC_TODO) != 0u;
                uint32_t mm = w & 0xFFu;
                while (mm) {
                    const int d = __ffs(mm) - 1; mm &= mm - 1u;
                    const int q = d + (d >> 2), di = (q * 11) >> 5;
                    const double2 u = L.slot[cur + (di - 1) * TT + (q - 3 * di - 1)];
                    const double x = ((0x5A >> d) & 1) ? u.x : u.y;
                    a += fabs(x); td = td || (x < 0);
                }
                double2 o = make_double2(0.0, 0.0);
                if (w & CI_OUT1) o.x = a * pv;
                if (w & CI_OUT2) o.y = a * (1 - pv);
                if (td) { o.x = -o.x; o.y = -o.y; }
                L.slot[cur] = o;
                L.cs[cur] = word | FC_DONE | (td ? FC_TODO : 0u);
                A.area[(int64_t)(i0 + r) * m + j0 + cl] = a;
                __builtin_amdgcn_fence(__ATOMIC_RELEASE, "workgroup", "local");
                const int sct = ci_section(w);
                int next = -1;
                if (w & CI_OUT1) {
                    const int tr = r + fe1r(sct), tc = cl + fe1c(sct);
                    if (tr >= 0 && tr < TT && tc >= 0 && tc < TT &&
                        (atomicSub(&L.cs[tr * TT + tc], 1u) & (FC_COUNT | FC_BLOCKED)) == 1u) next = tr * TT + tc;
                }
                if (w & CI_OUT2) {
                    const int tr = r + fe2r(sct), tc = cl + fe2c(sct);
                    if (tr >= 0 && tr < TT && tc >= 0 && tc < TT &&
                        (atomicSub(&L.cs[tr * TT + tc], 1u) & (FC_COUNT | FC_BLOCKED)) == 1u && next < 0) next = tr * TT + tc;
                }
                cur = next;
            } while (cur >= 0);
        }
        lds_sync();
    }
    uint32_t done = 0;
#pragma unroll
    for (int k = 0; k < NSET; k++) {
        const uint32_t word = L.cs[t + 256 * k];
        if (!(word & FC_DONE)) continue;
        done |= 1u << k;
        const int64_t c = (int64_t)(i0 + 8 * k + r0) * m + gj;
        A.contrib[c] = L.slot[t + 256 * k];
        A.cinfo[c] = ci_with_level(word >> 16, 1u);
        if (word & FC_TODO) A.todo_work[c] = 1;
    }
    const int32_t finalized = __popc(done), n_cells = __popc(ingrid);
    if (finalized) atomicAdd(&s_fin[0], finalized);
    if (n_cells) atomicAdd(&s_fin[1], n_cells);
    __syncthreads();
    if (t == 0) {
        if (s_fin[0]) atomicAdd(n_final, s_fin[0]);
        if (s_fin[0] == s_fin[1]) tile_done[tid] = 1;
    }
}

#ifdef PYDEM_SWEEP_QUEUE
__global__ void k_tiles_of_frontier(const QE *__restrict__ q, const int32_t *nq, int m, int tiles_x, int32_t stamp, TileNext N)
{
    const int32_t n = *nq;
    for (int32_t k = blockIdx.x * blockDim.x + threadIdx.x; k < n; k += gridDim.x * blockDim.x) {
        const int32_t c = q[k].c;
        const int tt = (c / m / TH) * tiles_x + (c % m) / TT;
        if (atomicExch(&N.flag[tt], stamp) != stamp) N.list[atomicAdd(N.count, 1)] = tt;
    }
}

__global__ __launch_bounds__(256) void k_sweep_rebuild_frontier(SweepArgs A, uint32_t r, QE *__restrict__ qn, int32_t *cn)
{
    __shared__ Stage S;
    if (threadIdx.x == 0) S.cnt = 0;
    __syncthreads();
    const int64_t NN = (int64_t)A.n * A.m;
    for (int64_t base = (int64_t)blockIdx.x * blockDim.x; base < NN; base += (int64_t)gridDim.x * blockDim.x) {
        const int64_t c = base + threadIdx.x;
        bool push = false;
        uint32_t cw = 0;
        if (c < NN) {
            cw = A.cinfo[c];
            const uint32_t lv = ci_level(cw);
            if (lv == 0 || lv == CI_LEVEL_INF) {
                bool ready = true;
#pragma unroll
                for (int d = 0; d < 8; d++)
                    if (cw & (1u << d)) {
                        const uint32_t lu = ci_level(A.cinfo[c + NB_DI[d] * A.m + NB_DJ[d]]);
                        ready = ready && (lu >= 1 && lu < r);
                    }
                if (ready && (cw & CI_PIT_IN))
                    for (int32_t e = pit_stash(A, (int32_t)c).x; e < A.n_pit && A.pin_dst[e] == (int32_t)c; e++) {
                        const uint32_t lu = ci_level(A.cinfo[A.pin_src[e]]);
                        ready = ready && (lu >= 1 && lu < r);
                    }
                if (ready) { A.cinfo[c] = ci_with_level(cw, r); push = true; }
            }
        }
        stage_push(S, push, (int32_t)c, cw);
        stage_flush(A, S, qn, cn, false);
    }
    stage_flush(A, S, qn, cn, true);
}

#endif

__global__ void k_row_area(const double *__restrict__ dX2, const double *__restrict__ dY2, int n, double *a0)
{
    const int i = blockIdx.x * blockDim.x + threadIdx.x;
    if (i < n) a0[i] = dX2[i] * dY2[i];
}

__global__ void k_weight_seed(const double *__restrict__ dX2, const double *__restrict__ dY2, int n, int m, double *__restrict__ w)
{
    for (int i = blockIdx.y; i < n; i += gridDim.y) {
        const double a0 = dX2[i] * dY2[i];
        for (int j = blockIdx.x * blockDim.x + threadIdx.x; j < m; j += gridDim.x * blockDim.x) w[(int64_t)i * m + j] *= a0;
    }
}

__global__ void k_sweep_rearm(uint32_t *__restrict__ cinfo, int64_t NN)
{
    for (int64_t c = (int64_t)blockIdx.x * blockDim.x + threadIdx.x; c < NN; c += (int64_t)gridDim.x * blockDim.x) {
        const uint32_t w = cinfo[c] & CI_STATIC_MASK;
        cinfo[c] = w | (((w & (0xFFu | CI_PIT_IN)) ? CI_LEVEL_INF : 0u) << CI_LEVEL_SHIFT);
    }
}

__global__ void k_uca_weighted_finalize(double *__restrict__ uca_w, const uint8_t *__restrict__ flats, int64_t NN)
{
    for (int64_t c = (int64_t)blockIdx.x * blockDim.x + threadIdx.x; c < NN; c += (int64_t)gridDim.x * blockDim.x)
        if (flats[c]) uca_w[c] = NAN;
}

struct ReseedCell { int32_t c; int32_t pin_first; int32_t pout_first; int32_t pad; };

__device__ __forceinline__ bool ci_unfinished(uint32_t w) { const uint32_t lv = ci_level(w); return lv == 0 || lv == CI_LEVEL_INF; }

template <bool WT = false>
__device__ void gather_finished(const SweepArgs &A, int32_t c, uint32_t cw, int32_t pin_first, double &a, bool &td)
{
    const int m = A.m, gi = c / m, gj = c - gi * m;
    a = WT ? A.a0[c] : A.a0[gi];
    td = !WT && (gi == 0 || gi == A.n - 1 || gj == 0 || gj == m - 1) && A.todo_work[c] != 0;
    for (int d = 0; d < 8; d++)
        if (cw & (1u << d)) {
            const int32_t u = c + NB_DI[d] * m + NB_DJ[d];
            if (ci_unfinished(A.cinfo[u])) continue;
            const bool cardinal = (NB_DI[d] == 0) || (NB_DJ[d] == 0);
            const double x = cardinal ? A.contrib[u].x : A.contrib[u].y;
            if constexpr (WT) a += x;
            else { a += fabs(x); td = td || (x < 0); }
        }
    if (cw & CI_PIT_IN)
        for (int32_t e = pin_first; e < A.n_pit && A.pin_dst[e] == c; e++) {
            const int32_t sc = A.pin_src[e];
            if (ci_unfinished(A.cinfo[sc])) continue;
            a += A.area[sc] * A.pin_w[e];
            if constexpr (!WT) td = td || (A.todo_work[sc] != 0);
        }
}

__global__ __launch_bounds__(256) void k_reseed_collect(SweepArgs A, ReseedCell *__restrict__ list, int32_t *count, int32_t cap,
                                                        const double *__restrict__ elev, int32_t *nan_flag)
{
    const int64_t NN = (int64_t)A.n * A.m;
    for (int64_t c64 = (int64_t)blockIdx.x * blockDim.x + threadIdx.x; c64 < NN; c64 += (int64_t)gridDim.x * blockDim.x) {
        const int32_t c = (int32_t)c64;
        if (elev[c] != elev[c]) *nan_flag = 1;
        const uint32_t w = A.cinfo[c];
        if (!ci_unfinished(w)) continue;
        int2 po = make_int2(0, 0);
        if (w & (CI_PIT_IN | CI_PIT_OUT)) po = pit_stash(A, c);
        const int32_t slot = atomicAdd(count, 1);
        if (slot < cap) { list[slot].c = c; list[slot].pin_first = po.x; list[slot].pout_first = po.y; list[slot].pad = 0; }
    }
}

__device__ __forceinline__ int reseed_find(const ReseedCell *U, int32_t nU, int32_t c)
{
    int lo = 0, hi = nU - 1;
    while (lo <= hi) { const int mid = (lo + hi) >> 1; if (U[mid].c == c) return mid; if (U[mid].c < c) lo = mid + 1; else hi = mid - 1; }
    return -1;
}

template <bool WT = false>
__global__ void k_reseed_replay(SweepArgs A, const ReseedCell *__restrict__ U, int32_t nU, const double *__restrict__ elev,
                                const double *__restrict__ pit_w, uint8_t *__restrict__ st, uint8_t *__restrict__ tdf,
                                int tile_has_nan, int maxcount, uint32_t pass, int32_t *n_final, int32_t *n_done_out)
{
    if (blockIdx.x != 0 || threadIdx.x != 0) return;
    const int n = A.n, m = A.m;
    auto on_edge = [&](int32_t c) { const int i = c / m, j = c - i * m; return i == 0 || i == n - 1 || j == 0 || j == m - 1; };
    auto is_done = [&](int32_t c) -> bool {
        if (!ci_unfinished(A.cinfo[c])) return true;
        const int k = reseed_find(U, nU, c);
        return k >= 0 && (st[k] & 1u);
    };
    for (int k = 0; k < nU; k++) {
        double a; bool td;
        gather_finished<WT>(A, U[k].c, A.cinfo[U[k].c] & CI_STATIC_MASK, U[k].pin_first, a, td);
        A.area[U[k].c] = a; tdf[k] = td; st[k] = 0;
    }
    int32_t n_done = 0, done_prev = -1;
    for (int count = 2; n_done < nU && count < maxcount && n_done != done_prev; count++) {
        done_prev = n_done;
        double mx = 0.0;
        for (int k = 0; k < nU; k++) if (!(st[k] & 1u) && elev[U[k].c] > mx) mx = elev[U[k].c];
        if (tile_has_nan) mx = NAN;
        for (int k = 0; k < nU; k++) {
            const double v = (st[k] & 1u) ? 0.0 : elev[U[k].c];
            st[k] = (uint8_t)((st[k] & 1u) | (((v - mx) / mx > -0.01) ? 2u : 0u));
        }
        for (int64_t guard = 0; guard < 8 * (int64_t)nU + 64; guard++) {
            for (int k = 0; k < nU; k++) if (st[k] & 2u) { if (!(st[k] & 1u)) n_done++; st[k] |= 1u; }
            for (int k = 0; k < nU; k++) st[k] = (uint8_t)((st[k] & 1u) | ((st[k] & 2u) ? 4u : 0u));
            for (int k = 0; k < nU; k++) {
                if (!(st[k] & 4u)) continue;
                const int32_t i = U[k].c;
                const uint32_t cw = A.cinfo[i] & CI_STATIC_MASK;
                int32_t tg[2]; double fc[2]; int nt = 0;
                if (cw & (CI_OUT1 | CI_OUT2)) {
                    const int sct = ci_section(cw);
                    const double pv = A.prop[i];
                    if (cw & CI_OUT1) { tg[nt] = i + fe1r(sct) * m + fe1c(sct); fc[nt] = pv; nt++; }
                    if (cw & CI_OUT2) { tg[nt] = i + fe2r(sct) * m + fe2c(sct); fc[nt] = 1 - pv; nt++; }
                    if (nt == 2 && tg[1] < tg[0]) { const int32_t tt = tg[0]; tg[0] = tg[1]; tg[1] = tt; const double ff = fc[0]; fc[0] = fc[1]; fc[1] = ff; }
                }
                int32_t e = (cw & CI_PIT_OUT) ? U[k].pout_first : 0;
                for (int q = 0;; q++) {
                    int32_t row; double factor;
                    if (cw & CI_PIT_OUT) { if (!(e < A.n_pit && A.pit_src[e] == i)) break; row = A.pit_dst[e]; factor = pit_w[e]; e++; }
                    else { if (q >= nt) break; row = tg[q]; factor = fc[q]; }
                    const int kr = reseed_find(U, nU, row);
                    if (kr < 0) continue;
                    if ((st[kr] & 1u) && on_edge(row)) continue;
                    A.area[row] += A.area[i] * factor;
                    if (tdf[k]) tdf[kr] = 1;
                    bool wait = false;
                    const uint32_t cwr = A.cinfo[row] & CI_STATIC_MASK;
                    for (int d = 0; d < 8 && !wait; d++)
                        if ((cwr & (1u << d)) && !is_done(row + NB_DI[d] * m + NB_DJ[d])) wait = true;
                    if (!wait && (cwr & CI_PIT_IN))
                        for (int32_t e2 = U[kr].pin_first; e2 < A.n_pit && A.pin_dst[e2] == row; e2++)
                            if (!is_done(A.pin_src[e2])) { wait = true; break; }
                    if (!wait) st[kr] |= 2u;
                }
            }
            bool changed = false;
            for (int k = 0; k < nU; k++) if (((st[k] >> 1) & 1u) != ((st[k] >> 2) & 1u)) changed = true;
            if (!changed) break;
        }
        for (int k = 0; k < nU; k++) st[k] &= 1u;
    }
    for (int k = 0; k < nU; k++) {
        const int32_t c = U[k].c;
        if (tdf[k]) A.todo_work[c] = 1;
        if (st[k] & 1u) A.cinfo[c] = ci_with_level(A.cinfo[c], pass);
    }
    atomicAdd(n_final, n_done);
    *n_done_out = n_done;
}

struct ReseedHost { int32_t c; uint32_t cw; int32_t pin_first, pout_first; double area, elev, prop; int32_t td, pad; };
template <bool WT = false>
__global__ __launch_bounds__(256) void k_reseed_gather(SweepArgs A, const ReseedCell *__restrict__ U, int32_t nU, const double *__restrict__ elev,
                                                       ReseedHost *__restrict__ out)
{
    for (int32_t k = blockIdx.x * blockDim.x + threadIdx.x; k < nU; k += gridDim.x * blockDim.x) {
        ReseedHost h;
        h.c = U[k].c; h.cw = A.cinfo[h.c] & CI_STATIC_MASK; h.pin_first = U[k].pin_first; h.pout_first = U[k].pout_first;
        double a; bool td;
        gather_finished<WT>(A, h.c, h.cw, h.pin_first, a, td);
        h.area = a; h.td = td; h.pad = 0; h.elev = elev[h.c]; h.prop = (h.cw & (CI_OUT1 | CI_OUT2)) ? A.prop[h.c] : 0.0;
        out[k] = h;
    }
}
struct ReseedBack { int32_t c; int32_t flags; double area; };
__global__ __launch_bounds__(256) void k_reseed_scatter(SweepArgs A, const ReseedBack *__restrict__ B, int32_t nU, uint32_t pass)
{
    for (int32_t k = blockIdx.x * blockDim.x + threadIdx.x; k < nU; k += gridDim.x * blockDim.x) {
        const int32_t c = B[k].c;
        A.area[c] = B[k].area;
        if (B[k].flags & 2) A.todo_work[c] = 1;
        if (B[k].flags & 1) A.cinfo[c] = ci_with_level(A.cinfo[c], pass);
    }
}

__device__ __forceinline__ bool finalize_cell(double *__restrict__ uca, const double *__restrict__ elev, int64_t c, uint32_t f, uint32_t td,
                                              int apply_limit, double limit)
{
    if (f) uca[c] = NAN;
    bool dn = !td;
    if (td && isnan(elev[c])) dn = true;
    if (apply_limit && !f && uca[c] > limit) dn = true;
    return dn;
}

__global__ __launch_bounds__(256) void k_uca_finalize(double *__restrict__ uca, const uint8_t *__restrict__ flats,
                                                      const uint8_t *__restrict__ todo_work, const double *__restrict__ elev,
                                                      uint8_t *__restrict__ edge_done, int64_t NN, int apply_limit, double limit)
{
    const int64_t nvec = NN >> 4, stride = (int64_t)gridDim.x * blockDim.x, t0 = (int64_t)blockIdx.x * blockDim.x + threadIdx.x;
    for (int64_t v = t0; v < nvec; v += stride) {
        const uint4 f4 = reinterpret_cast<const uint4 *>(flats)[v], t4 = reinterpret_cast<const uint4 *>(todo_work)[v];
        const uint32_t fw[4] = {f4.x, f4.y, f4.z, f4.w}, tw[4] = {t4.x, t4.y, t4.z, t4.w};
        uint32_t dw[4];
#pragma unroll
        for (int q = 0; q < 4; q++) {
            uint32_t d = 0;
#pragma unroll
            for (int b = 0; b < 4; b++)
                d |= (finalize_cell(uca, elev, v * 16 + q * 4 + b, (fw[q] >> (8 * b)) & 0xFFu, (tw[q] >> (8 * b)) & 0xFFu, apply_limit, limit) ? 1u : 0u) << (8 * b);
            dw[q] = d;
        }
        reinterpret_cast<uint4 *>(edge_done)[v] = make_uint4(dw[0], dw[1], dw[2], dw[3]);
    }
    for (int64_t c = (nvec << 4) + t0; c < NN; c += stride)
        edge_done[c] = finalize_cell(uca, elev, c, flats[c], todo_work[c], apply_limit, limit);
}

__global__ __launch_bounds__(256) void k_twi(const double *__restrict__ uca, const double *__restrict__ mag,
                                             double *__restrict__ twi, int64_t NN, double min_slope, int lim_uca,
                                             double uca_cap, int lim_twi, double twi_cap)
{
    for (int64_t c = (int64_t)blockIdx.x * blockDim.x + threadIdx.x; c < NN; c += (int64_t)gridDim.x * blockDim.x) {
        double t = uca[c];
        if (lim_uca && t > uca_cap) t = uca_cap;
        t = log(t / (mag[c] + min_slope));
        if (lim_twi && t > twi_cap) t = twi_cap;
        twi[c] = t;
    }
}

}

int stage_section_graph(pydem_tile *t, const pydem_options *opt)
{
    const int n = (int)t->n, m = (int)t->m;
    t->graph_opt = *opt;
    t->edge_clean = false;
    t->einc_ready = false;
    PYDEM_TRY(tile_alloc(t, &t->todo_work, (size_t)t->NN));
    PYDEM_TRY(tile_alloc(t, &t->cinfo, (size_t)t->NN));
    const dim3 grid2((unsigned)(cdiv(m, 256) < 64 ? cdiv(m, 256) : 64), (unsigned)(n < 16384 ? n : 16384));
    t->tm.n_pit_edges = 0; t->tm.n_pits_undrained = 0; t->tm.pits_ms = 0;
    t->pits.n_edges = 0; t->pits.n_raw = 0;
    if (t->flats_state == 2) t->flats_state = 0;
    double *corner_sums = (double *)(t->counters + CS_WORK);
    HIP_TRY(hipEventRecord(t->ev_fork, t->stream));
    HIP_TRY(hipStreamWaitEvent(t->stream2, t->ev_fork, 0));
    HIP_TRY(hipMemcpyAsync(t->todo_work, t->flats, (size_t)t->NN, hipMemcpyDeviceToDevice, t->stream2));
    HIP_TRY(hipEventRecord(t->ev_snap, t->stream2));
    HIP_TRY(hipStreamWaitEvent(t->stream, t->ev_snap, 0));
    hipLaunchKernelGGL(k_section_proportion, grid2, dim3(256), 0, t->stream2, t->dir, (const uint8_t *)t->todo_work, t->sec_theta,
                       t->NN, n, m, t->elev, t->section, t->prop, t->cinfo);
    HIP_TRY(hipMemsetAsync(t->counters + CS_WORK, 0, CS_WORK_WORDS * sizeof(int32_t), t->stream2));
    HIP_TRY(hipMemsetAsync(t->edge_todo, 0, (size_t)t->NN, t->stream2));
    HIP_TRY(hipMemsetAsync(t->todo_work, 0, (size_t)t->NN, t->stream2));
    hipLaunchKernelGGL(k_graph_inmask, grid2, dim3(256), 0, t->stream2, t->prop, t->elev, n, m,
                       t->cinfo, t->edge_todo, t->todo_work, corner_sums);
    HIP_TRY(hipEventRecord(t->ev_join, t->stream2));
    static int graph_serial = -1;
    if (graph_serial < 0) { const char *e = getenv("PYDEM_GRAPH_SERIAL"); graph_serial = e ? atoi(e) : 0; }
    if (graph_serial) HIP_TRY(hipStreamWaitEvent(t->stream, t->ev_join, 0));
    HIP_TRY(hipEventRecord(t->ev[0], t->stream));
    if (opt->drain_pits) PYDEM_TRY(stage_pits(t, opt));
    HIP_TRY(hipEventRecord(t->ev[2], t->stream));
    HIP_TRY(hipStreamWaitEvent(t->stream, t->ev_join, 0));
    const bool stash = t->pit_stash_live && t->uca != nullptr;
    t->pit_stash_live = false;
    if (t->pits.n_edges > 0) {
        if (stash) {
            hipLaunchKernelGGL(k_graph_add_pits<true>, dim3(grid_for(t->pits.n_edges, 1024)), dim3(256), 0, t->stream, t->pits.src,
                               t->pits.dst, t->pits.w, t->pits.n_edges, n, m, t->cinfo, corner_sums, (const int32_t *)t->pits.in_dst, t->uca);
            t->pit_stash_live = true;
        } else {
            hipLaunchKernelGGL(k_graph_add_pits<false>, dim3(grid_for(t->pits.n_edges, 1024)), dim3(256), 0, t->stream, t->pits.src,
                               t->pits.dst, t->pits.w, t->pits.n_edges, n, m, t->cinfo, corner_sums, (const int32_t *)nullptr, (double *)nullptr);
        }
    }
    hipLaunchKernelGGL(k_corner_todo, dim3(1), dim3(64), 0, t->stream, corner_sums, t->elev, n, m, t->edge_todo, t->todo_work);
    HIP_TRY(hipEventRecord(t->ev[3], t->stream));
    HIP_TRY(hipGetLastError());
    HIP_TRY(hipEventSynchronize(t->ev[3]));
    float a = 0, b = 0;
    HIP_TRY(hipEventElapsedTime(&a, t->ev[0], t->ev[2]));
    HIP_TRY(hipEventElapsedTime(&b, t->ev[2], t->ev[3]));
    (void)a;
    t->tm.graph_ms = b;
    return 0;
}


static int64_t reseed_replay_host(std::vector<ReseedHost> &H, std::vector<uint8_t> &done, int n, int m, int maxcount, bool tile_has_nan,
                                  const std::vector<int32_t> &pit_src, const std::vector<int32_t> &pit_dst, const std::vector<double> &pit_w,
                                  const std::vector<int32_t> &pin_dst, const std::vector<int32_t> &pin_src)
{
    const int32_t nU = (int32_t)H.size();
    const int64_t n_pit = (int64_t)pit_src.size();
    static const int DI[8] = {-1, -1, -1, 0, 0, 1, 1, 1}, DJ[8] = {-1, 0, 1, -1, 1, -1, 0, 1};
    auto find = [&](int32_t c) -> int32_t {
        int32_t lo = 0, hi = nU - 1;
        while (lo <= hi) { const int32_t mid = (lo + hi) >> 1; if (H[(size_t)mid].c == c) return mid; if (H[(size_t)mid].c < c) lo = mid + 1; else hi = mid - 1; }
        return -1;
    };
    auto on_edge = [&](int32_t c) { const int i = c / m, j = c - i * m; return i == 0 || i == n - 1 || j == 0 || j == m - 1; };
    auto is_done = [&](int32_t c) -> bool { const int32_t k = find(c); return k < 0 || done[(size_t)k]; };
    done.assign((size_t)nU, 0);
    std::vector<uint8_t> in_cur((size_t)nU, 0);
    std::vector<int32_t> cur, prev;
    int64_t n_done = 0, done_prev = -1;
    for (int count = 2; n_done < nU && count < maxcount && n_done != done_prev; count++) {
        done_prev = n_done;
        double mx = 0.0;
        for (int32_t k = 0; k < nU; k++) if (!done[(size_t)k] && H[(size_t)k].elev > mx) mx = H[(size_t)k].elev;
        if (tile_has_nan) mx = NAN;
        cur.clear();
        for (int32_t k = 0; k < nU; k++) {
            const double v = done[(size_t)k] ? 0.0 : H[(size_t)k].elev;
            if ((v - mx) / mx > -0.01) cur.push_back(k);
        }
        for (int64_t guard = 0; guard < 8 * (int64_t)nU + 64; guard++) {
            for (int32_t k : cur) { if (!done[(size_t)k]) n_done++; done[(size_t)k] = 1; }
            prev.swap(cur); cur.clear();
            for (int32_t k : prev) {
                const ReseedHost &S = H[(size_t)k];
                const int32_t i = S.c;
                int32_t tg[2]; double fc[2]; int nt = 0;
                if (S.cw & (CI_OUT1 | CI_OUT2)) {
                    const int sct = (int)((S.cw >> CI_SEC_SHIFT) & 7u);
                    if (S.cw & CI_OUT1) { tg[nt] = i + fe1r(sct) * m + fe1c(sct); fc[nt] = S.prop; nt++; }
                    if (S.cw & CI_OUT2) { tg[nt] = i + fe2r(sct) * m + fe2c(sct); fc[nt] = 1 - S.prop; nt++; }
                    if (nt == 2 && tg[1] < tg[0]) { std::swap(tg[0], tg[1]); std::swap(fc[0], fc[1]); }
                }
                int64_t e = (S.cw & CI_PIT_OUT) ? S.pout_first : 0;
                for (int q = 0;; q++) {
                    int32_t row; double factor;
                    if (S.cw & CI_PIT_OUT) { if (!(e < n_pit && pit_src[(size_t)e] == i)) break; row = pit_dst[(size_t)e]; factor = pit_w[(size_t)e]; e++; }
                    else { if (q >= nt) break; row = tg[q]; factor = fc[q]; }
                    const int32_t kr = find(row);
                    if (kr < 0) continue;
                    if (done[(size_t)kr] && on_edge(row)) continue;
                    H[(size_t)kr].area += S.area * factor;
                    if (S.td) H[(size_t)kr].td = 1;
                    bool wait = false;
                    const uint32_t cwr = H[(size_t)kr].cw;
                    for (int d = 0; d < 8 && !wait; d++)
                        if ((cwr & (1u << d)) && !is_done(row + DI[d] * m + DJ[d])) wait = true;
                    if (!wait && (cwr & CI_PIT_IN))
                        for (int64_t e2 = H[(size_t)kr].pin_first; e2 < n_pit && pin_dst[(size_t)e2] == row; e2++)
                            if (!is_done(pin_src[(size_t)e2])) { wait = true; break; }
                    if (!wait && !in_cur[(size_t)kr]) { in_cur[(size_t)kr] = 1; cur.push_back(kr); }
                }
            }
            std::sort(cur.begin(), cur.end());
            for (int32_t k : cur) in_cur[(size_t)k] = 0;
            if (cur == prev) break;
        }
        cur.clear();
    }
    return n_done;
}

template <bool WT>
static int sweep_schedule(pydem_tile *t, const pydem_options *opt, double *seed)
{
    const int n = (int)t->n, m = (int)t->m;
    if (m >= (1 << 22)) { pydem_set_error("uca: tiles wider than 4 194 303 columns are not supported (this one has %d)", m); return -2; }
    PYDEM_TRY(tile_alloc(t, &t->queue[0], (size_t)t->NN));
    PYDEM_TRY(tile_alloc(t, &t->queue[1], (size_t)t->NN));
    PYDEM_TRY(tile_alloc(t, &t->row_area, (size_t)t->n));
    PYDEM_TRY(tile_alloc(t, &t->contrib, (size_t)t->NN * 2));
    t->circular_cells = 0;
    int32_t *total = t->counters + CS_PROCESSED;
#ifdef PYDEM_SWEEP_QUEUE
    int32_t *cnt3 = t->counters + CS_FRONTIER;
    int32_t *nsrc = t->counters + CS_SOURCES;
    int64_t done_prev = 0;
#endif
    HIP_TRY(hipEventRecord(t->ev[0], t->stream));
    HIP_TRY(hipMemsetAsync(t->counters, 0, CS_WINDOW * sizeof(int32_t), t->stream));
    if (!WT) hipLaunchKernelGGL(k_row_area, dim3((unsigned)cdiv(n, 256)), dim3(256), 0, t->stream, t->dX2, t->dY2, n, t->row_area);
    SweepArgs A;
    fill_sweep_args(t, A);
    if (WT) { A.a0 = seed; A.area = t->uca_w; }
    const bool stashed = !WT && t->pit_stash_live;
    if (!WT) t->pit_stash_live = false;
    if (A.n_pit > 0 && !stashed)
        hipLaunchKernelGGL(k_pit_stash, dim3(grid_for(A.n_pit, 2048)), dim3(256), 0, t->stream, A.pin_dst, A.pit_src, A.n_pit, A.area);
    const int tiles_x = (int)cdiv(m, TT), tiles_total = tiles_x * (int)cdiv(n, TH);
    const size_t tiles_pad = ((size_t)tiles_total + 255) & ~(size_t)255;
    const size_t scratch_need = tiles_pad * (1 + 4 + 4 + 4 + 4 + 4) + 64 * sizeof(int32_t);
    PYDEM_TRY(tile_reserve(t, &t->scratch, &t->scratch_bytes, scratch_need, scratch_need, false));
    uint8_t *tile_done = (uint8_t *)t->scratch;
    int32_t *tile_flag = (int32_t *)(tile_done + tiles_pad);
    int32_t *tile_list[2] = {tile_flag + tiles_pad, tile_flag + 2 * tiles_pad};
    int32_t *cntT = t->counters + CS_TILE_LIST;
    A.tile_open = tile_flag + 3 * tiles_pad;
    static int64_t sym_switch = -1;
    if (sym_switch < 0) { const char *e = getenv("PYDEM_SWEEP_SYM"); sym_switch = e ? atoll(e) : 4096; if (sym_switch < 0) sym_switch = 0; }
    SymArgs Y;
    memset(&Y, 0, sizeof(Y));
    int32_t *symc = tile_flag + 4 * tiles_pad + tiles_pad;
    const bool sym_on = sym_switch > 0 && TH == 32 && t->NN / 2 < ((int64_t)1 << 31);
    if (sym_on) {
        Y.pool0 = (double *)t->queue[0]; Y.pool1 = (double *)t->queue[1];
        Y.nreg = t->NN >= ((int64_t)1 << 22) ? 16 : 2;
        Y.reg_cap = (uint32_t)((t->NN / 2) / (Y.nreg / 2));
        Y.ctr = symc; Y.tile_sym = (uint32_t *)(tile_flag + 4 * tiles_pad); Y.stat = symc + 32;
        HIP_TRY(hipMemsetAsync(Y.tile_sym, 0xff, tiles_pad * 4, t->stream));
        HIP_TRY(hipMemsetAsync(symc, 0, 64 * sizeof(int32_t), t->stream));
    }
    HIP_TRY(hipMemsetAsync(tile_done, 0, tiles_pad * 5, t->stream));
    HIP_TRY(hipMemsetAsync(A.tile_open, 0x7f, tiles_pad * 4, t->stream));
    HIP_TRY(hipMemsetAsync(cntT, 0, 4 * sizeof(int32_t), t->stream));
    if (A.dbg & 4) HIP_TRY(hipMemsetAsync(t->counters + CS_TILE_PROF, 0, CS_TILE_PROF_WORDS * sizeof(int32_t), t->stream));
    int64_t launches = 0;
    uint32_t pass = 0;
    int32_t *work16 = t->counters + CS_WORK, *work3 = t->counters + CS_WORK;
    HIP_TRY(hipMemsetAsync(work16, 0, 16 * sizeof(int32_t), t->stream));
    static int lds_pad = -1;
    if (lds_pad < 0) { const char *e = getenv("PYDEM_TILE_LDS_PAD"); lds_pad = e ? atoi(e) : 0; }
    static int res_switch = -1;
    if (res_switch < 0) { const char *e = getenv("PYDEM_SWEEP_RESIDENT"); res_switch = e ? atoi(e) : 4096; }
    int64_t listed_left = 0;
    auto run_listed = [&](int p, int64_t ntiles, int64_t stop_at) -> int {
        TileNext N;
        N.flag = tile_flag;
        listed_left = ntiles;
        while (ntiles > stop_at) {
            static int dbg_each = -1;
            if (dbg_each < 0) { const char *e = getenv("PYDEM_SWEEP_DEBUG"); dbg_each = (e && atoi(e) >= 2) ? 1 : 0; }
            const int batch = dbg_each ? 1 : ntiles < 2048 ? 16 : 8;
#ifndef PYDEM_LISTED_DYNAMIC
            const int grid = (int)(ntiles < 8192 ? (ntiles > 64 ? ntiles : 64) : 8192) * (4 / LWPB);
#else
            const int64_t want = cdiv(ntiles, 4);
            const int grid = (int)(want < 256 * PYDEM_LISTED_OCC ? (want > 16 ? want : 16) : 256 * PYDEM_LISTED_OCC);
#endif
            const bool resident = ntiles <= res_switch;
            for (int b = 0; b < batch; b++, p++) {
                N.list = tile_list[(p + 1) % 2]; N.count = &cntT[(p + 1) % 3];
                if (resident)
                    hipLaunchKernelGGL(HIP_KERNEL_NAME(k_sweep_tiles_resident<WT>), dim3((unsigned)(ntiles > 256 ? ntiles : 256)), dim3(64), 0, t->stream, A, (uint32_t)p, tiles_x,
                                       (const int32_t *)tile_list[p % 2], (const int32_t *)&cntT[p % 3], tile_done, total, N,
                                       &cntT[(p + 2) % 3], Y);
                else
                    hipLaunchKernelGGL(HIP_KERNEL_NAME(k_sweep_tiles_listed<WT>), dim3(grid), dim3(64 * LWPB), (size_t)lds_pad, t->stream, A, (uint32_t)p, tiles_x,
                                       (const int32_t *)tile_list[p % 2], (const int32_t *)&cntT[p % 3], tile_done, total, N,
                                       &cntT[(p + 2) % 3], work3, Y);
                launches++;
            }
            if (hipMemcpyAsync(t->h_counters, t->counters, CS_END * sizeof(int32_t), hipMemcpyDeviceToHost, t->stream) != hipSuccess) return -1;
            if (hipStreamSynchronize(t->stream) != hipSuccess) return -1;
            ntiles = t->h_counters[CS_TILE_LIST + p % 3];
            listed_left = ntiles;
            if (getenv("PYDEM_SWEEP_DEBUG")) fprintf(stderr, "listed tile pass %d: %lld tiles listed next, processed %d\n", p, (long long)ntiles, t->h_counters[CS_PROCESSED]);
            if (p > (int)CI_LEVEL_INF - 256) return -2;
        }
        return p;
    };
    auto replay_unfinished = [&](uint32_t pass) -> int {
        HIP_TRY(hipMemcpyAsync(t->h_counters, t->counters, CS_END * sizeof(int32_t), hipMemcpyDeviceToHost, t->stream));
        HIP_TRY(hipStreamSynchronize(t->stream));
        if ((int64_t)t->h_counters[CS_PROCESSED] >= t->NN) return 0;
        {
            ReseedCell *U = (ReseedCell *)t->queue[0];
            const int64_t cap64 = std::min<int64_t>(t->NN * 4 / (int64_t)sizeof(ReseedCell), (int64_t)1 << 22);
// ... 27 lines not shown
                std::vector<ReseedHost> H((size_t)nU);
                HIP_TRY(hipMemcpyAsync(H.data(), dH, (size_t)nU * sizeof(ReseedHost), hipMemcpyDeviceToHost, t->stream));
                HIP_TRY(hipMemcpyAsync(t->h_counters, t->counters, CS_END * sizeof(int32_t), hipMemcpyDeviceToHost, t->stream));
                HIP_TRY(hipStreamSynchronize(t->stream));
                const bool has_nan = t->h_counters[CS_RESEED + 1] != 0;
                std::sort(H.begin(), H.end(), [](const ReseedHost &a, const ReseedHost &b) { return a.c < b.c; });
                const size_t np = (size_t)A.n_pit;
                std::vector<int32_t> h_ps(np), h_pd(np), h_is(np), h_id(np); std::vector<double> h_pw(np);
                if (np) {
                    HIP_TRY(hipMemcpy(h_ps.data(), A.pit_src, np * 4, hipMemcpyDeviceToHost));
                    HIP_TRY(hipMemcpy(h_pd.data(), A.pit_dst, np * 4, hipMemcpyDeviceToHost));
                    HIP_TRY(hipMemcpy(h_pw.data(), t->pits.w, np * 8, hipMemcpyDeviceToHost));
                    HIP_TRY(hipMemcpy(h_id.data(), A.pin_dst, np * 4, hipMemcpyDeviceToHost));
                    HIP_TRY(hipMemcpy(h_is.data(), A.pin_src, np * 4, hipMemcpyDeviceToHost));
                }
                std::vector<uint8_t> dn;
                const int64_t n_done = reseed_replay_host(H, dn, n, m, (int)opt->circular_ref_maxcount, has_nan, h_ps, h_pd, h_pw, h_id, h_is);
                std::vector<ReseedBack> back((size_t)nU);
                for (int32_t k = 0; k < nU; k++) { back[(size_t)k].c = H[(size_t)k].c; back[(size_t)k].area = H[(size_t)k].area; back[(size_t)k].flags = (dn[(size_t)k] ? 1 : 0) | (H[(size_t)k].td ? 2 : 0); }
                static_assert(sizeof(ReseedBack) <= sizeof(ReseedHost), "the gather buffer is reused for the results");
                HIP_TRY(hipMemcpy(dH, back.data(), (size_t)nU * sizeof(ReseedBack), hipMemcpyHostToDevice));
                hipLaunchKernelGGL(k_reseed_scatter, dim3(grid_for(nU, 1024)), dim3(256), 0, t->stream, A, (const ReseedBack *)dH, nU, pass);
                HIP_TRY(hipStreamSynchronize(t->stream));
                t->h_counters[CS_PROCESSED] += (int32_t)n_done;
                HIP_TRY(hipMemcpy(t->counters + CS_PROCESSED, t->h_counters + CS_PROCESSED, sizeof(int32_t), hipMemcpyHostToDevice));
                if (getenv("PYDEM_SWEEP_DEBUG")) fprintf(stderr, "circular drainage: %lld unfinished cells, %lld finished by the re-seed replay on the host\n", (long long)unfinished, (long long)n_done);
                return 0;
            }
            std::vector<ReseedCell> hu((size_t)unfinished);
            HIP_TRY(hipMemcpyAsync(hu.data(), U, hu.size() * sizeof(ReseedCell), hipMemcpyDeviceToHost, t->stream));
            HIP_TRY(hipStreamSynchronize(t->stream));
            std::sort(hu.begin(), hu.end(), [](const ReseedCell &a, const ReseedCell &b) { return a.c < b.c; });
            HIP_TRY(hipMemcpyAsync(U, hu.data(), hu.size() * sizeof(ReseedCell), hipMemcpyHostToDevice, t->stream));
            hipLaunchKernelGGL(HIP_KERNEL_NAME(k_reseed_replay<WT>), dim3(1), dim3(64), 0, t->stream, A, (const ReseedCell *)U, (int32_t)unfinished,
                               (const double *)t->elev, (const double *)t->pits.w, stf, stf + unfinished, t->h_counters[CS_RESEED + 1],
                               (int)opt->circular_ref_maxcount, pass, total, rc + 2);
            launches += 2;
            HIP_TRY(hipMemcpyAsync(t->h_counters, t->counters, CS_END * sizeof(int32_t), hipMemcpyDeviceToHost, t->stream));
            HIP_TRY(hipStreamSynchronize(t->stream));
            if (getenv("PYDEM_SWEEP_DEBUG")) fprintf(stderr, "circular drainage: %lld unfinished cells, %d finished by the re-seed replay\n", (long long)unfinished, t->h_counters[CS_RESEED + 2]);
        }
        return 0;
    };
#ifdef PYDEM_SWEEP_QUEUE
    static int sweep_mode = -1;
    if (sweep_mode < 0) { const char *e = getenv("PYDEM_SWEEP_MODE"); sweep_mode = (e && !strcmp(e, "queue")) ? 1 : 0; }
    if (WT && sweep_mode == 1) { pydem_set_error("pydem_uca_weighted: PYDEM_SWEEP_MODE=queue is not supported (the weighted sweep runs the tile passes)"); return -6; }
#else
    constexpr int sweep_mode = 0;
#endif
#ifdef PYDEM_SWEEP_STATIC
    const unsigned full_grid = (unsigned)(((tiles_total + 31) / 32) * 8);
#else
    const unsigned full_grid = (unsigned)std::min<int64_t>(((tiles_total + 31) / 32) * 8, 256 * (32 / FWPB));
#endif

    if (sweep_mode == 0) {
        static int first_kind = -1;
        if (first_kind < 0) { const char *e = getenv("PYDEM_SWEEP_FIRST"); first_kind = (e && !strcmp(e, "lds")) ? 1 : 0; }
        static int dense_levels = -1;
        if (dense_levels < 0) { const char *e = getenv("PYDEM_SWEEP_DENSE"); dense_levels = e ? atoi(e) : 0; if (dense_levels < 0) dense_levels = 0; }
        for (int lv = 1; !WT && lv <= dense_levels; lv++) {
            hipLaunchKernelGGL(k_sweep_dense_level, dim3((unsigned)cdiv(m, 256), (unsigned)cdiv(n, DENSE_BAND)), dim3(256), 0, t->stream,
                               A, (uint32_t)lv, total);
            launches++;
        }
        const uint32_t pb = WT ? 0u : (uint32_t)dense_levels;
        if (!WT && first_kind == 1 && TH == 32 && pb == 0)
            hipLaunchKernelGGL(k_sweep_first, dim3((unsigned)(((tiles_total + 7) / 8) * 8)), dim3(256), 0, t->stream, A, tiles_x, tiles_total, tile_done, total);
        else {
            TileNext N0; N0.flag = nullptr; N0.list = nullptr; N0.count = nullptr;
            hipLaunchKernelGGL(HIP_KERNEL_NAME(k_sweep_tiles<false, WT>), dim3(full_grid), dim3(64 * FWPB), (size_t)lds_pad, t->stream, A, pb + 1u, tiles_x, tiles_total, tile_done, total, N0, work16);
        }
        TileNext N; N.flag = tile_flag; N.list = tile_list[(pb + 3) % 2]; N.count = &cntT[(pb + 3) % 3];
        hipLaunchKernelGGL(HIP_KERNEL_NAME(k_sweep_tiles<true, WT>), dim3(full_grid), dim3(64 * FWPB), (size_t)lds_pad, t->stream, A, pb + 2u, tiles_x, tiles_total, tile_done, total, N, work16 + 8);
        HIP_TRY(hipMemsetAsync(work3, 0, CS_WORK_WORDS * sizeof(int32_t), t->stream));
        launches += 2;
        HIP_TRY(hipMemcpyAsync(t->h_counters, t->counters, CS_END * sizeof(int32_t), hipMemcpyDeviceToHost, t->stream));
        HIP_TRY(hipStreamSynchronize(t->stream));
        if (getenv("PYDEM_SWEEP_DEBUG")) fprintf(stderr, "tile passes %u-%u: %d cells of %lld, %d tiles listed\n", pb + 1, pb + 2, t->h_counters[CS_PROCESSED], (long long)t->NN, t->h_counters[CS_TILE_LIST + (pb + 3) % 3]);
        int p_end = run_listed((int)pb + 3, t->h_counters[CS_TILE_LIST + (pb + 3) % 3], sym_on ? sym_switch : 0);
        if (sym_on && p_end > 0 && listed_left > 0) {
            const uint32_t ps = (uint32_t)p_end;
            TileNext N3; N3.flag = tile_flag; N3.list = tile_list[(ps + 1) % 2]; N3.count = &cntT[(ps + 1) % 3];
            HIP_TRY(hipMemsetAsync(&cntT[(ps + 2) % 3], 0, sizeof(int32_t), t->stream));
            int32_t *cand = tile_list[ps % 2];
            hipLaunchKernelGGL(k_sym_candidates, dim3((unsigned)cdiv(tiles_total, 256)), dim3(256), 0, t->stream, (const uint8_t *)tile_done, (const int32_t *)A.tile_open,
                               tiles_total, 256, cand, symc + 16);
            HIP_TRY(hipEventRecord(t->ev_fork, t->stream));
            HIP_TRY(hipStreamWaitEvent(t->stream2, t->ev_fork, 0));
            hipLaunchKernelGGL(HIP_KERNEL_NAME(k_sweep_sym<256, WT>), dim3(256 * 32), dim3(64), 0, t->stream, A, Y, ps, tiles_x, tiles_total, tile_done, total, N3, (const int32_t *)cand, (const int32_t *)(symc + 16), 0, 0);
            hipLaunchKernelGGL(HIP_KERNEL_NAME(k_sweep_sym<1024, WT>), dim3(256 * 16), dim3(64), 0, t->stream2, A, Y, ps, tiles_x, tiles_total, tile_done, total, N3, (const int32_t *)cand, (const int32_t *)(symc + 17), 1, 256);
            HIP_TRY(hipEventRecord(t->ev_join, t->stream2));
            HIP_TRY(hipStreamWaitEvent(t->stream, t->ev_join, 0));
            launches += 4;
            HIP_TRY(hipMemcpyAsync(t->h_counters, t->counters, CS_END * sizeof(int32_t), hipMemcpyDeviceToHost, t->stream));
            HIP_TRY(hipStreamSynchronize(t->stream));
            if (getenv("PYDEM_SWEEP_DEBUG")) fprintf(stderr, "symbolic pass %u: %d cells of %lld, %d tiles listed\n", ps, t->h_counters[CS_PROCESSED], (long long)t->NN, t->h_counters[CS_TILE_LIST + (ps + 1) % 3]);
            p_end = run_listed((int)ps + 1, t->h_counters[CS_TILE_LIST + (ps + 1) % 3], 0);
        }
        if (p_end == -1) { pydem_set_error("HIP error in the listed tile passes"); return -4; }
        if (p_end == -2) { pydem_set_error("flow paths longer than %u passes are not supported", CI_LEVEL_INF); return -5; }
        pass = (uint32_t)p_end;
        t->tm.sweep_tile_passes = (int64_t)pass;
        if (sym_on) {
            hipLaunchKernelGGL(HIP_KERNEL_NAME(k_sym_finish<WT>), dim3((unsigned)std::min<int64_t>(tiles_total, 256 * 16)), dim3(64), 0, t->stream, A, Y, pass, tiles_x, tiles_total, total);
            launches++;
            if (getenv("PYDEM_SWEEP_DEBUG")) {
                int32_t hs[64];
                HIP_TRY(hipMemcpyAsync(hs, symc, sizeof(hs), hipMemcpyDeviceToHost, t->stream));
                HIP_TRY(hipStreamSynchronize(t->stream));
                int64_t used = 0;
                for (int r = 0; r < Y.nreg; r++) used += hs[r];
                fprintf(stderr, "two-level solve: %d symbolic tiles (%d fell back to numeric visits), %d outlets, %d symbolic cells, pool %lld of %lld doubles\n",
                        hs[32], hs[33], hs[34], hs[35], (long long)used, (long long)Y.reg_cap * Y.nreg);
#ifdef PYDEM_SYM_PROF
                {
                    const unsigned long long *acc = (const unsigned long long *)(hs + 40);
                    const double v = acc[8] ? (double)acc[8] : 1.0;
                    fprintf(stderr, "symbolic visits: %llu, %.1f open cells, %.1f rounds, %.1f pool entries each; us per visit: stage %.1f, inlets %.1f, set-up %.1f, constants %.1f, "
                            "rounds %.1f (%.2f us per round), end %.1f\n", acc[8], acc[9] / v, acc[6] / v, acc[7] / v, acc[0] / v / 100, acc[1] / v / 100, acc[2] / v / 100,
                            acc[3] / v / 100, acc[4] / v / 100, acc[6] ? acc[4] / 100.0 / (double)acc[6] : 0.0, acc[5] / v / 100);
                }
#endif
            }
        }
        HIP_TRY(hipMemcpyAsync(t->h_counters, t->counters, CS_END * sizeof(int32_t), hipMemcpyDeviceToHost, t->stream));
        HIP_TRY(hipStreamSynchronize(t->stream));
        PYDEM_TRY(replay_unfinished(pass));
        if (A.dbg & 4) {
            const unsigned long long *acc = (const unsigned long long *)(t->h_counters + CS_TILE_PROF);
            fprintf(stderr, "tile phases (10 ns ticks summed over %llu tile runs, %llu of them finished nothing): stage %llu, setup %llu, rounds %llu (%llu rounds), stamp %llu\n",
                    acc[5], acc[6], acc[0], acc[1], acc[2], acc[4], acc[3]);
        }
    }
#ifdef PYDEM_SWEEP_QUEUE
    if (sweep_mode == 1) {
    static int max_passes = -1;
    if (max_passes < 0) { const char *e = getenv("PYDEM_TILE_PASSES"); max_passes = e ? atoi(e) : 1; if (max_passes < 1) max_passes = 1; }
    for (;;) {
        pass++;
        { TileNext N0; N0.flag = nullptr; N0.list = nullptr; N0.count = nullptr;
          HIP_TRY(hipMemsetAsync(work16, 0, 16 * sizeof(int32_t), t->stream));
          hipLaunchKernelGGL(k_sweep_tiles<false>, dim3(full_grid), dim3(256), 0, t->stream, A, pass, tiles_x, tiles_total, tile_done, total, N0, work16); }
        launches++;
        HIP_TRY(hipMemcpyAsync(t->h_counters, t->counters, CS_WINDOW * sizeof(int32_t), hipMemcpyDeviceToHost, t->stream));
        HIP_TRY(hipStreamSynchronize(t->stream));
        const int64_t done_now = t->h_counters[CS_PROCESSED];
        const int64_t gained = done_now - done_prev;
        if (getenv("PYDEM_SWEEP_DEBUG")) fprintf(stderr, "tile pass %u: +%lld cells (%.2f%%), total %.2f%%\n", pass, (long long)gained, 100.0 * gained / t->NN, 100.0 * done_now / t->NN);
        done_prev = done_now;
        if (done_now >= t->NN || gained * 64 < t->NN || (int)pass >= max_passes) break;
    }
    t->tm.sweep_tile_passes = (int64_t)pass;
    int r = (int)pass + 1;
    int64_t last = 0;
    if (done_prev < t->NN) {
        hipLaunchKernelGGL(k_sweep_rebuild_frontier, dim3(grid_for(t->NN, 4096)), dim3(256), 0, t->stream, A, (uint32_t)r,
                           (QE *)t->queue[r % 2], &cnt3[r % 3]);
        launches++;
        HIP_TRY(hipMemcpyAsync(t->h_counters, t->counters, CS_WINDOW * sizeof(int32_t), hipMemcpyDeviceToHost, t->stream));
        HIP_TRY(hipStreamSynchronize(t->stream));
        last = t->h_counters[CS_FRONTIER + r % 3];
        if (getenv("PYDEM_SWEEP_DEBUG")) fprintf(stderr, "after rebuild: frontier %lld, processed %d of %lld\n", (long long)last, t->h_counters[CS_PROCESSED], (long long)t->NN);
    }
    (void)nsrc;
// ... 131 lines not shown
```

pydem_amd/csrc/uca_edge.hip:

```cpp
#include "uca_graph.h"
#include <hipcub/hipcub.hpp>
#include <algorithm>
#include <functional>
#include <memory>
#include <thread>
#include <vector>
#include <math.h>
#include <stdlib.h>
#include <string.h>
#include <time.h>

namespace {

constexpr uint32_t EF_S = 1u, EF_SEED = 2u, EF_T = 4u, EF_DONE = 8u;
constexpr uint32_t CI_ESEED = 1u << 31, CI_EONE = 1u << CI_LEVEL_SHIFT;
__device__ __forceinline__ uint32_t ci_ecount(uint32_t w) { return (w >> CI_LEVEL_SHIFT) & 0xFFFFu; }

struct EdgeArgs {
    SweepArgs G;
    uint32_t *flag;
    double *delta;
    const uint8_t *flats;
    uint8_t *edge_done;
    uint8_t *p_done, *p_seed;
// ... 843 lines not shown

__global__ __launch_bounds__(256) void k_cinc_apply(CIncArgs E)
{
    for (int32_t k = blockIdx.x * blockDim.x + threadIdx.x; k < E.nd; k += gridDim.x * blockDim.x) {
        NDRec &R = E.rec[k];
        const uint32_t f = R.flag;
        if ((f & NF_DONE) && !(f & NF_APPLIED)) {
            if (!(f & NF_SEED)) E.uca[R.cell] += R.delta;
            if (E.set_done) E.edge_done[R.cell] = 1;
            R.flag = f | NF_APPLIED;
        }
    }
}


#include "uca_cond.inl"
#include "uca_cbuild.inl"

}

static double host_now_ms()
{
    struct timespec ts;
    clock_gettime(CLOCK_MONOTONIC, &ts);
    return ts.tv_sec * 1e3 + ts.tv_nsec * 1e-6;
}

template <typename Launch>
static int edge_wide_levels(pydem_tile *t, int32_t cap, int &r, int32_t &last, Launch launch)
{
    while (last > cap) {
        const int batch = last > 65536 ? 4 : 16;
        const int grid = grid_for(last, 1024);
        for (int b = 0; b < batch; b++, r++) launch(r, grid);
        HIP_TRY(hipMemcpyAsync(t->h_counters, t->counters, CS_WINDOW * sizeof(int32_t), hipMemcpyDeviceToHost, t->stream));
        HIP_TRY(hipStreamSynchronize(t->stream));
        last = t->h_counters[CS_FRONTIER + r % 3];
        if (r > (1 << 24)) { pydem_set_error("edge update: flow paths too long"); return -5; }
    }
    return 0;
}

struct CascadeDbg {
    int levels = 0, wide = 0, handovers = 0;
    int prev = -1;
    void ran(int kind, int from, int to)
    {
        if (to <= from) return;
        if (prev >= 0 && prev != kind) handovers++;
        if (kind == 1) wide += to - from;
        prev = kind; levels = to;
    }
};

int stage_edge_update(pydem_tile *t, const pydem_options *opt, const double *const data[4], const uint8_t *const done[4],
                      const uint8_t *const todo[4])
{
    (void)opt;
    if (t->einc_ready) PYDEM_TRY(stage_edge_flush(t));
    const double t_begin = host_now_ms();
    const int n = (int)t->n, m = (int)t->m;
    PYDEM_TRY(tile_alloc(t, &t->row_area, (size_t)t->n));
    const int L = n > m ? n : m;
    const int64_t nper = 2 * (int64_t)m + 2 * (int64_t)(n - 2);
    PYDEM_TRY(tile_alloc(t, &t->estamp, (size_t)t->NN));
    PYDEM_TRY(tile_alloc(t, &t->edelta, (size_t)t->NN));
    PYDEM_TRY(tile_alloc(t, &t->labels, (size_t)t->NN));
    PYDEM_TRY(tile_alloc(t, &t->flatlist, (size_t)t->NN));
    PYDEM_TRY(tile_alloc(t, &t->queue[0], (size_t)t->NN));
    PYDEM_TRY(tile_alloc(t, &t->queue[1], (size_t)t->NN));
    PYDEM_TRY(tile_alloc(t, &t->eseed, (size_t)(nper > 0 ? nper : 1) * 2));
    PYDEM_TRY(tile_alloc(t, &t->p_delta, (size_t)nper));
    PYDEM_TRY(tile_alloc(t, &t->p_flags, (size_t)nper * 2));
    PYDEM_TRY(tile_alloc(t, &t->s_data, (size_t)L * 4));
    PYDEM_TRY(tile_alloc(t, &t->s_flags, (size_t)L * 8));
    EdgeArgs E;
    SweepArgs &A = E.G;
    fill_sweep_args(t, A);
    E.flag = (uint32_t *)t->estamp; E.delta = t->edelta; E.flats = t->flats; E.edge_done = t->edge_done;
    E.p_done = t->p_flags; E.p_seed = t->p_flags + nper; E.p_delta = t->p_delta;
    E.rlist = t->labels; E.rcount = t->counters + CS_EDGE_REACHED;
    E.tlist = t->flatlist; E.tcount = t->counters + CS_EDGE_CLEARED;
    PYDEM_TRY(tile_alloc(t, &t->contrib, (size_t)t->NN * 2));
    E.pit_off = reinterpret_cast<const int2 *>(t->contrib);
    if (!t->edge_clean) {
        if (A.n_pit > 0)
            hipLaunchKernelGGL(k_pit_offsets, dim3(grid_for(A.n_pit, 2048)), dim3(256), 0, t->stream, A.pin_dst, A.pit_src, A.n_pit,
                               reinterpret_cast<int2 *>(t->contrib));
        HIP_TRY(hipMemsetAsync(t->estamp, 0, (size_t)t->NN * 4, t->stream));
        hipLaunchKernelGGL(k_edge_clear_levels, dim3(grid_for(t->NN, 8192)), dim3(256), 0, t->stream, A.cinfo, t->NN);
        HIP_TRY(hipMemsetAsync(t->edge_todo, 0, (size_t)t->NN, t->stream));
        HIP_TRY(hipMemsetAsync(t->edge_done, 1, (size_t)t->NN, t->stream));
        t->edge_clean = true;
    } else if (t->etodo_prev > 0) {
        hipLaunchKernelGGL(k_edge_restore, dim3(grid_for(t->etodo_prev, 1024)), dim3(256), 0, t->stream, t->flatlist, t->etodo_prev,
                           t->edge_done);
    }
    if (data) {
        if (t->h_strip_cap < (size_t)L) {
            if (t->h_strip_d) { (void)hipHostFree(t->h_strip_d); (void)hipHostFree(t->h_strip_f); }
            HIP_TRY(hipHostMalloc((void **)&t->h_strip_d, (size_t)L * 4 * sizeof(double)));
            HIP_TRY(hipHostMalloc((void **)&t->h_strip_f, (size_t)L * 8));
            t->h_strip_cap = (size_t)L;
        }
        double *hd = t->h_strip_d;
        uint8_t *hf = t->h_strip_f;
        memset(hd, 0, (size_t)L * 4 * sizeof(double));
        memset(hf, 0, (size_t)L * 8);
        for (int s = 0; s < 4; s++) {
            const int len = s < 2 ? n : m;
            for (int k = 0; k < len; k++) {
                hd[(size_t)s * L + k] = data[s][k];
                hf[(size_t)s * L + k] = done[s][k] != 0;
                hf[(size_t)(4 + s) * L + k] = todo[s][k] != 0;
            }
        }
        HIP_TRY(hipMemcpyAsync(t->s_data, hd, (size_t)L * 4 * 8, hipMemcpyHostToDevice, t->stream));
        HIP_TRY(hipMemcpyAsync(t->s_flags, hf, (size_t)L * 8, hipMemcpyHostToDevice, t->stream));
    }
    HIP_TRY(hipMemsetAsync(t->counters, 0, CS_WINDOW * sizeof(int32_t), t->stream));
    int32_t *cnt3 = t->counters + CS_FRONTIER;
    int32_t *n_seed = t->counters + CS_EDGE_SEEDS;
    QE *q0 = (QE *)t->queue[0], *q1 = (QE *)t->queue[1];
    hipLaunchKernelGGL(k_edge_init, dim3((unsigned)cdiv(nper, 128)), dim3(128), 0, t->stream, E, t->s_data, t->s_flags,
                       t->s_flags + (size_t)4 * L, L, t->uca, t->edge_todo, q0, &cnt3[0], (QE *)t->eseed, n_seed);
    HIP_TRY(hipMemcpyAsync(t->h_counters, t->counters, CS_WINDOW * sizeof(int32_t), hipMemcpyDeviceToHost, t->stream));
    HIP_TRY(hipStreamSynchronize(t->stream));
    const int32_t nflood = t->h_counters[CS_FRONTIER], nseed = t->h_counters[CS_EDGE_SEEDS];
    CascadeDbg dbg[2];
    auto run_levels = [&](int which, int32_t first) -> int {
        int r = 0;
        int32_t last = first;
        int32_t *state = t->counters + CS_CASCADE_STATE;
        static int small_cap = -1;
        if (small_cap < 0) { const char *e = getenv("PYDEM_EDGE_SMALL_CAP"); small_cap = e ? atoi(e) : SMALL_CAP; if (small_cap > SMALL_CAP) small_cap = SMALL_CAP; }
        while (last > 0) {
            if (last <= small_cap) {
                if (which == 0) hipLaunchKernelGGL(k_edge_small<0>, dim3(1), dim3(1024), 0, t->stream, E, q0, q1, cnt3, r, state);
                else hipLaunchKernelGGL(k_edge_small<1>, dim3(1), dim3(1024), 0, t->stream, E, q0, q1, cnt3, r, state);
                HIP_TRY(hipMemcpyAsync(t->h_counters, t->counters, CS_WINDOW * sizeof(int32_t), hipMemcpyDeviceToHost, t->stream));
                HIP_TRY(hipStreamSynchronize(t->stream));
                const int r0 = r;
                r = t->h_counters[CS_CASCADE_STATE];
                last = t->h_counters[CS_FRONTIER + r % 3];
                dbg[which].ran(0, r0, r);
                continue;
            }
            const int r0 = r;
            PYDEM_TRY(edge_wide_levels(t, std::max(small_cap, 0), r, last, [&](int lv, int grid) {
                if (which == 0) hipLaunchKernelGGL(k_edge_level<0>, dim3(grid), dim3(256), 0, t->stream, E, (lv % 2) ? q1 : q0, (lv % 2) ? q0 : q1, cnt3, lv);
                else hipLaunchKernelGGL(k_edge_level<1>, dim3(grid), dim3(256), 0, t->stream, E, (lv % 2) ? q1 : q0, (lv % 2) ? q0 : q1, cnt3, lv);
            }));
            dbg[which].ran(1, r0, r);
        }
        return 0;
    };
    if (nflood > 0) PYDEM_TRY(run_levels(0, nflood));
    if (nseed > 0) {
        int32_t three[3] = {nseed, 0, 0};
        HIP_TRY(hipMemcpyAsync(q0, t->eseed, (size_t)nseed * sizeof(QE), hipMemcpyDeviceToDevice, t->stream));
        HIP_TRY(hipMemcpyAsync(cnt3, three, sizeof(three), hipMemcpyHostToDevice, t->stream));
        PYDEM_TRY(run_levels(1, nseed));
        hipLaunchKernelGGL(k_edge_apply, dim3(grid_for(t->NN < (1 << 20) ? t->NN : (1 << 20), 1024)), dim3(256), 0, t->stream, E, t->uca,
                           E.rcount);
    }
    hipLaunchKernelGGL(k_edge_apply_perimeter, dim3((unsigned)cdiv(nper, 128)), dim3(128), 0, t->stream, E, t->uca);
    hipLaunchKernelGGL(k_edge_cleanup, dim3(256), dim3(256), 0, t->stream, E, (const int32_t *)E.rcount, (const int32_t *)E.tcount);
    HIP_TRY(hipMemcpyAsync(t->h_counters, t->counters, CS_WINDOW * sizeof(int32_t), hipMemcpyDeviceToHost, t->stream));
    HIP_TRY(hipGetLastError());
    HIP_TRY(hipStreamSynchronize(t->stream));
    t->etodo_prev = t->h_counters[CS_EDGE_CLEARED];
    if (getenv("PYDEM_EDGE_DEBUG"))
        fprintf(stderr, "edge round: %d seeds, %d todo cells, %d cells reached; levels: floods %d (%d wide), sweep %d (%d wide); hand-overs %d + %d; %.3f ms\n",
                nseed, t->h_counters[CS_EDGE_CLEARED], t->h_counters[CS_EDGE_REACHED], dbg[0].levels, dbg[0].wide, dbg[1].levels, dbg[1].wide,
                dbg[0].handovers, dbg[1].handovers, host_now_ms() - t_begin);
    return 0;
}

static int einc_args(pydem_tile *t, IncArgs &E)
{
    PYDEM_TRY(tile_alloc(t, &t->row_area, (size_t)t->n));
    PYDEM_TRY(tile_alloc(t, &t->estamp, (size_t)t->NN));
    PYDEM_TRY(tile_alloc(t, &t->edelta, (size_t)t->NN));
    PYDEM_TRY(tile_alloc(t, &t->queue[0], (size_t)t->NN));
    PYDEM_TRY(tile_alloc(t, &t->queue[1], (size_t)t->NN));
    PYDEM_TRY(tile_alloc(t, &t->contrib, (size_t)t->NN * 2));
    fill_sweep_args(t, E.G);
    E.flag = (uint32_t *)t->estamp; E.delta = t->edelta; E.flats = t->flats; E.edge_done = t->edge_done; E.edge_todo = t->edge_todo;
    E.uca = t->uca; E.pit_off = reinterpret_cast<const int2 *>(t->contrib); E.set_done = 1;
    E.prof = t->counters + CS_EINC_PROF;
    E.nanq = reinterpret_cast<int32_t *>(t->queue[1]); E.n_nan = t->counters + CS_NAN_SEEDS;
    E.round16 = (uint32_t)(t->einc_round % 65535) + 1u;
    return 0;
}

static int einc_cascade(pydem_tile *t, const IncArgs &E, CascadeDbg *dbg)
{
    int32_t *cnt3 = t->counters + CS_FRONTIER;
    int32_t *state = t->counters + CS_CASCADE_STATE;
    QE *q0 = (QE *)t->queue[0], *q1 = (QE *)t->queue[1];
    int r = 0;
    for (;;) {
        static int einc_block = -1;
        if (einc_block < 0) { const char *e = getenv("PYDEM_EINC_BLOCK"); einc_block = e ? atoi(e) : 1024; }
        hipLaunchKernelGGL(k_einc_small, dim3(1), dim3(einc_block), 0, t->stream, E, q0, q1, cnt3, r, state);
        HIP_TRY(hipMemcpyAsync(t->h_counters, t->counters, CS_WINDOW * sizeof(int32_t), hipMemcpyDeviceToHost, t->stream));
        HIP_TRY(hipStreamSynchronize(t->stream));
        const int r_small = r;
        r = t->h_counters[CS_CASCADE_STATE];
        if (dbg) dbg->ran(0, r_small, r);
        int32_t last = t->h_counters[CS_FRONTIER + r % 3];
        if (last == 0) break;
        const int r_wide = r;
        PYDEM_TRY(edge_wide_levels(t, SMALL_CAP, r, last, [&](int lv, int grid) {
            hipLaunchKernelGGL(k_einc_level, dim3(grid), dim3(256), 0, t->stream, E, (lv % 2) ? q1 : q0, (lv % 2) ? q0 : q1, cnt3, lv);
        }));
        if (dbg) dbg->ran(1, r_wide, r);
        if (last == 0) break;
    }
    HIP_TRY(hipGetLastError());
    return 0;
}


static int cinc_args(pydem_tile *t, CIncArgs &E)
{
    fill_sweep_args(t, E.G);
    E.rec = (NDRec *)t->nd_rec; E.nd = t->nd; E.cid = t->estamp;
    E.pit_off = reinterpret_cast<const int2 *>(t->contrib);
    E.flats = t->flats; E.edge_done = t->edge_done; E.edge_todo = t->edge_todo; E.uca = t->uca; E.set_done = 1;
    E.prof = t->counters + CS_EINC_PROF;
    E.nanq = reinterpret_cast<int32_t *>(t->edelta); E.n_nan = t->counters + CS_NAN_SEEDS;
    E.round16 = (uint32_t)(t->einc_round % 65535) + 1u;
    return 0;
}

static int cinc_cascade(pydem_tile *t, const CIncArgs &E, CascadeDbg *dbg)
{
    int32_t *cnt3 = t->counters + CS_FRONTIER;
    int32_t *state = t->counters + CS_CASCADE_STATE;
    QE *q0 = (QE *)t->queue[0], *q1 = (QE *)t->queue[1];
    int r = 0;
    for (;;) {
        static int cinc_block = -1;
        if (cinc_block < 0) { const char *e = getenv("PYDEM_EINC_BLOCK"); cinc_block = e ? atoi(e) : 1024; }
        static int cinc_cap = -1;
        if (cinc_cap < 0) { const char *e = getenv("PYDEM_CINC_SMALL"); cinc_cap = e ? std::max(1, std::min(atoi(e), SMALL_CAP)) : 1024; }
        hipLaunchKernelGGL(k_cinc_small, dim3(1), dim3(cinc_block), 0, t->stream, E, q0, q1, cnt3, r, state, cinc_cap);
        hipLaunchKernelGGL(k_cinc_apply, dim3(grid_for(E.nd, 1024)), dim3(256), 0, t->stream, E);
        HIP_TRY(hipMemcpyAsync(t->h_counters, t->counters, CS_WINDOW * sizeof(int32_t), hipMemcpyDeviceToHost, t->stream));
        HIP_TRY(hipStreamSynchronize(t->stream));
        const int r_small = r;
        r = t->h_counters[CS_CASCADE_STATE];
        if (dbg) dbg->ran(0, r_small, r);
        int32_t last = t->h_counters[CS_FRONTIER + r % 3];
        if (last == 0) break;
        const bool wide = last > cinc_cap;
        const int r_wide = r;
        PYDEM_TRY(edge_wide_levels(t, cinc_cap, r, last, [&](int lv, int grid) {
            hipLaunchKernelGGL(k_cinc_level, dim3(grid), dim3(256), 0, t->stream, E, (lv % 2) ? q1 : q0, (lv % 2) ? q0 : q1, cnt3, lv);
        }));
        if (dbg) dbg->ran(1, r_wide, r);
        if (last == 0) {
            if (wide) { hipLaunchKernelGGL(k_cinc_apply, dim3(grid_for(E.nd, 1024)), dim3(256), 0, t->stream, E); HIP_TRY(hipStreamSynchronize(t->stream)); }
            break;
        }
    }
    HIP_TRY(hipGetLastError());
    return 0;
// ... 804 lines not shown
```

pydem_amd/csrc/uca_graph.h:

```cpp
#pragma once
#include "internal.h"
#include <stdlib.h>

namespace {

constexpr uint32_t CI_OUT1 = 1u << 8, CI_OUT2 = 1u << 9, CI_PIT_OUT = 1u << 10, CI_PIT_IN = 1u << 11;
constexpr int CI_SEC_SHIFT = 12, CI_LEVEL_SHIFT = 15;
constexpr uint32_t CI_LEVEL_INF = 0x1FFFFu, CI_STATIC_MASK = 0x7FFFu;
__device__ __forceinline__ uint32_t ci_level(uint32_t w) { return w >> CI_LEVEL_SHIFT; }
__device__ __forceinline__ int ci_section(uint32_t w) { return (int)((w >> CI_SEC_SHIFT) & 7u); }
__device__ __forceinline__ uint32_t ci_with_level(uint32_t w, uint32_t lv) { return (w & CI_STATIC_MASK) | (lv << CI_LEVEL_SHIFT); }

__device__ __constant__ const int NB_DI[8] = {-1, -1, -1, 0, 0, 1, 1, 1};
__device__ __constant__ const int NB_DJ[8] = {-1, 0, 1, -1, 1, -1, 0, 1};
__device__ __constant__ const int NB_S0[8] = {6, 5, 4, 0, 3, 0, 1, 2};
__device__ __constant__ const int NB_S1[8] = {7, 6, 5, 7, 4, 1, 2, 3};

__device__ __forceinline__ bool keep_edge(double w, double z_to, double z_from)
{
    return !isnan(w) && (w > 1e-8) && (z_to <= z_from);
}

struct SweepArgs {
    uint32_t *cinfo;
    const double *prop, *a0;
    double *area;
    double2 *contrib;
    uint8_t *todo_work;
    int n, m;
    const int32_t *pit_src, *pit_dst;
    const int32_t *pin_dst, *pin_src; const double *pin_w;
    int64_t n_pit;
    int dbg;
    int32_t qcap;
    int32_t *err;
    int32_t *tile_open;
};

struct QE { int32_t c; uint32_t cw; };

enum CounterSlot : int {
    CS_FRONTIER = 0,
    CS_PROCESSED = 3,
    CS_SOURCES = 4,
    CS_ROUNDS = 5,
    CS_EDGE_REACHED = 6,
    CS_EDGE_CLEARED = 7,
    CS_EDGE_SEEDS = 8,
    CS_CASCADE_STATE = 12,
    CS_SWEEP_STATE = 14,
    CS_QUEUE_ERR = 15,
    CS_WINDOW = 16,
    CS_H_CB_TOTALS = 16,
    CS_WORK = 16, CS_WORK_WORDS = 24,
    CS_TILE_PROF = 32, CS_TILE_PROF_WORDS = 24,
    CS_EINC_PROF = 40,
    CS_ND_COUNT = 48,
    CS_ND_NEXT = 50,
    CS_NAN_SEEDS = 53,
    CS_COND_EDGES = 54,
    CS_TILE_LIST = 56,
    CS_RESEED = 60,
    CS_FLAT_SAVE = 62,
    CS_END = 64
};
static_assert(CS_FRONTIER + 3 <= CS_PROCESSED && CS_ROUNDS == CS_PROCESSED + 2, "kernels reach the round count through the processed-cells pointer");
static_assert(CS_ROUNDS < CS_EDGE_REACHED && CS_EDGE_SEEDS < CS_CASCADE_STATE && CS_CASCADE_STATE < CS_SWEEP_STATE && CS_SWEEP_STATE < CS_QUEUE_ERR,
              "the scalars of a cascade are live together");
static_assert(CS_QUEUE_ERR < CS_WINDOW && CS_WINDOW <= CS_WORK, "one copy of the window shows the host every scalar of a cascade, and no scratch");
static_assert(CS_WORK + CS_WORK_WORDS <= CS_EINC_PROF, "zeroing the per-tile scratch leaves the fix-up's words alone");
static_assert(CS_TILE_PROF + CS_TILE_PROF_WORDS <= CS_TILE_LIST, "the visit profile ends before the tile lists");
static_assert(CS_EINC_PROF + 8 <= CS_ND_COUNT && CS_ND_COUNT + 2 <= CS_ND_NEXT && CS_ND_NEXT < CS_NAN_SEEDS && CS_NAN_SEEDS < CS_COND_EDGES
              && CS_COND_EDGES < CS_TILE_LIST, "the fix-up's words are live together and stay clear of the sweep's");
static_assert(CS_TILE_LIST + 4 <= CS_RESEED && CS_RESEED + 3 <= CS_END && CS_FLAT_SAVE + 2 <= CS_END, "the sweep's lists and replay words are live together");

inline int grid_for(int64_t work, int cap) { const int64_t g = cdiv(work, 256); return (int)(g < cap ? (g > 0 ? g : 1) : cap); }
}

static void fill_sweep_args(pydem_tile *t, SweepArgs &A)
{
    A.cinfo = t->cinfo; A.prop = t->prop; A.a0 = t->row_area; A.area = t->uca;
    A.contrib = (double2 *)t->contrib; A.todo_work = t->todo_work; A.n = (int)t->n; A.m = (int)t->m;
    A.pit_src = t->pits.src; A.pit_dst = t->pits.dst; A.n_pit = t->pits.n_edges;
    A.pin_dst = t->pits.in_dst; A.pin_src = t->pits.in_src; A.pin_w = t->pits.in_w;
    A.qcap = (int32_t)(t->NN / 2 < INT32_MAX ? t->NN / 2 : INT32_MAX);
    A.err = t->counters + CS_QUEUE_ERR;
    A.tile_open = nullptr;
    { const char *e = getenv("PYDEM_TILE_DEBUG"); A.dbg = e ? atoi(e) : 0; }
}
```

Measured before the change: 5811.

## Replace per-cell contrib outputs with precomputed in-edge weights and signed area

The sweep no longer writes a 16-byte contrib (area times outgoing proportion, negated when tainted) for every finished cell. A new kernel instead precomputes each cell's first two incoming edge weights into the same buffer, running on a third stream that overlaps graph staging. Receivers now form contributions from the upstream area and weights, and the taint is carried in the sign of the stored area, which is made positive again at finalisation. This cuts per-cell write traffic in the sweep, at the cost of extra reads of neighbour area and prop for the third and later in-edges, plus an additional precompute pass.

```diff
diff --git a/pydem_amd/csrc/internal.h b/pydem_amd/csrc/internal.h
--- a/pydem_amd/csrc/internal.h
+++ b/pydem_amd/csrc/internal.h
@@ -53,7 +53,8 @@
     int device = 0;
     hipStream_t stream = nullptr;
     hipStream_t stream2 = nullptr;
-    hipEvent_t ev_fork = nullptr, ev_join = nullptr, ev_snap = nullptr;
+    hipStream_t stream3 = nullptr;
+    hipEvent_t ev_fork = nullptr, ev_join = nullptr, ev_snap = nullptr, ev_inw = nullptr;
     hipEvent_t ev[8] = {};
     double *elev = nullptr, *mag = nullptr, *dir = nullptr, *prop = nullptr, *uca = nullptr, *twi = nullptr;
     double *weight = nullptr, *uca_w = nullptr;
@@ -71,6 +72,8 @@
     int elev_dtype = 0;
     uint8_t *todo_work = nullptr;
     double *contrib = nullptr;
+    bool inw_live = false;
+    bool inw_wanted = false;
     uint32_t *cinfo = nullptr;
     int32_t *queue[2] = {nullptr, nullptr}, *labels = nullptr, *flatlist = nullptr;
     int32_t *counters = nullptr;
diff --git a/pydem_amd/csrc/tile.hip b/pydem_amd/csrc/tile.hip
--- a/pydem_amd/csrc/tile.hip
+++ b/pydem_amd/csrc/tile.hip
@@ -167,9 +167,11 @@
 {
     HIP_TRY(hipStreamCreateWithFlags(&t->stream, hipStreamNonBlocking));
     HIP_TRY(hipStreamCreateWithFlags(&t->stream2, hipStreamNonBlocking));
+    HIP_TRY(hipStreamCreateWithFlags(&t->stream3, hipStreamNonBlocking));
     HIP_TRY(hipEventCreateWithFlags(&t->ev_fork, hipEventDisableTiming));
     HIP_TRY(hipEventCreateWithFlags(&t->ev_join, hipEventDisableTiming));
     HIP_TRY(hipEventCreateWithFlags(&t->ev_snap, hipEventDisableTiming));
+    HIP_TRY(hipEventCreateWithFlags(&t->ev_inw, hipEventDisableTiming));
     for (int i = 0; i < 8; i++) HIP_TRY(hipEventCreate(&t->ev[i]));
     PYDEM_TRY(tile_alloc(t, &t->counters, 64));
     HIP_TRY(hipHostMalloc((void **)&t->h_counters, 64 * sizeof(int32_t), hipHostMallocDefault));
@@ -195,6 +197,7 @@
     (void)hipSetDevice(t->device);
     if (t->stream) (void)hipStreamSynchronize(t->stream);
     if (t->stream2) (void)hipStreamSynchronize(t->stream2);
+    if (t->stream3) (void)hipStreamSynchronize(t->stream3);
     tile_release_all(t);
     if (t->h_counters) (void)hipHostFree(t->h_counters);
     if (t->h_strip_d) (void)hipHostFree(t->h_strip_d);
@@ -206,6 +209,8 @@
     if (t->ev_fork) (void)hipEventDestroy(t->ev_fork);
     if (t->ev_join) (void)hipEventDestroy(t->ev_join);
     if (t->ev_snap) (void)hipEventDestroy(t->ev_snap);
+    if (t->ev_inw) (void)hipEventDestroy(t->ev_inw);
+    if (t->stream3) { (void)hipStreamSynchronize(t->stream3); (void)hipStreamDestroy(t->stream3); }
     if (t->stream2) { (void)hipStreamSynchronize(t->stream2); (void)hipStreamDestroy(t->stream2); }
     if (t->stream) (void)hipStreamDestroy(t->stream);
     delete t;
@@ -573,9 +578,11 @@
     if (!t->spacing_set) { pydem_set_error("pydem_uca: call pydem_tile_set_spacing first"); return -3; }
     PYDEM_TRY(ensure_fields(t, {PYDEM_SECTION, PYDEM_PROPORTION, PYDEM_UCA, PYDEM_EDGE_TODO, PYDEM_EDGE_DONE}));
     t->pit_stash_live = step_lean();
+    t->inw_wanted = true;
     {
         const int rc = stage_section_graph(t, opt);
-        if (rc != 0) { t->pit_stash_live = false; return rc; }
+        t->inw_wanted = false;
+        if (rc != 0) { t->pit_stash_live = false; t->inw_live = false; return rc; }
     }
     t->graph_valid = true;
     {
diff --git a/pydem_amd/csrc/uca.hip b/pydem_amd/csrc/uca.hip
--- a/pydem_amd/csrc/uca.hip
+++ b/pydem_amd/csrc/uca.hip
@@ -103,6 +103,25 @@
     }
 }
 
+__global__ __launch_bounds__(256) void k_graph_inweights(const uint32_t *__restrict__ cinfo, const double *__restrict__ prop, int n, int m,
+                                                         double2 *__restrict__ inw)
+{
+    for (int i = blockIdx.y; i < n; i += gridDim.y)
+    for (int j = blockIdx.x * blockDim.x + threadIdx.x; j < m; j += gridDim.x * blockDim.x) {
+        const int64_t c = (int64_t)i * m + j;
+        uint32_t mm = cinfo[c] & 0xFFu;
+        double w[2] = {0.0, 0.0};
+#pragma unroll
+        for (int q = 0; q < 2; q++)
+            if (mm) {
+                const int d = __ffs(mm) - 1; mm &= mm - 1u;
+                const double pv = prop[c + (int64_t)NB_DI[d] * m + NB_DJ[d]];
+                w[q] = ((0x5A >> d) & 1) ? pv : 1 - pv;
+            }
+        inw[c] = make_double2(w[0], w[1]);
+    }
+}
+
 template <bool STASH>
 __global__ void k_graph_add_pits(const int32_t *__restrict__ src, const int32_t *__restrict__ dst,
                                  const double *__restrict__ w, int64_t ne, int n, int m,
@@ -244,17 +263,18 @@
     return ready && owner == u;
 }
 
-__device__ __forceinline__ void publish_cell(const SweepArgs &A, int32_t c, uint32_t cw, double acc, bool td)
-{
-    A.area[c] = acc;
-    double2 o = make_double2(0.0, 0.0);
-    if (cw & (CI_OUT1 | CI_OUT2)) {
-        const double p = A.prop[c];
-        if (cw & CI_OUT1) o.x = acc * p;
-        if (cw & CI_OUT2) o.y = acc * (1 - p);
-        if (td) { o.x = -o.x; o.y = -o.y; }
-    }
-    A.contrib[c] = o;
+__device__ __forceinline__ double in_edge(const SweepArgs &A, int32_t c, int m, int d)
+{
+    const int q = d + (d >> 2);
+    const int di = (q * 11) >> 5;
+    const int32_t u = c + (di - 1) * m + (q - 3 * di - 1);
+    const double ua = A.area[u], up = A.prop[u];
+    return ((0x5A >> d) & 1) ? ua * up : ua * (1 - up);
+}
+
+__device__ __forceinline__ void publish_cell(const SweepArgs &A, int32_t c, double acc, bool td)
+{
+    A.area[c] = td ? -acc : acc;
     if (td) A.todo_work[c] = 1;
 }
 
@@ -279,7 +299,7 @@
 #pragma unroll
         for (int k = 0; k < 4; k++) {
             more = more && e + k < A.n_pit && d4[k] == c;
-            if (more) { acc += a4[k] * w4[k]; td = td || (t4[k] != 0); }
+            if (more) { acc += fabs(a4[k]) * w4[k]; td = td || (t4[k] != 0); }
         }
         if (!more) break;
     }
@@ -316,16 +336,14 @@
 #pragma unroll
         for (int d = 0; d < 8; d++) {
             if (cw & (1u << d)) {
-                const int32_t u = c + NB_DI[d] * m + NB_DJ[d];
-                const bool cardinal = (NB_DI[d] == 0) || (NB_DJ[d] == 0);
-                const double x = cardinal ? A.contrib[u].x : A.contrib[u].y;
+                const double x = in_edge(A, c, m, d);
                 acc += fabs(x);
                 td = td || (x < 0);
             }
         }
         if (cw & CI_PIT_IN) gather_pit_edges(A, c, sc.x, acc, td);
         out_start = sc.y;
-        publish_cell(A, c, cw, acc, td);
+        publish_cell(A, c, acc, td);
         if (t1 >= 0) {
             if (!LOWLAT && (c1 & CI_PIT_IN)) s1 = pit_stash(A, t1);
             r1 = owns_target<LOWLAT>(A, t1, c, r, c1, l1, s1.x);
@@ -483,17 +501,39 @@
     int32_t *list, *count;
 };
 
-__device__ __forceinline__ const double *in_edge_ptr(const SweepArgs &A, int32_t c, int m, int d)
-{
-    const int q = d + (d >> 2);
-    const int di = (q * 11) >> 5;
-    const int32_t u = c + (di - 1) * m + (q - 3 * di - 1);
-    return reinterpret_cast<const double *>(A.contrib + u) + (((0x5A >> d) & 1) ? 0 : 1);
-}
-__device__ __forceinline__ double in_edge(const SweepArgs &A, int32_t c, int m, int d) { return *in_edge_ptr(A, c, m, d); }
+template <bool WT>
+__device__ __forceinline__ void gather_final_edges(const SweepArgs &A, int32_t c, int m, uint32_t im, uint32_t mm, double &K, bool &td)
+{
+    double2 wv = make_double2(0.0, 0.0);
+    if (mm) wv = A.inw[c];
+    const uint32_t first2 = im & ~((im & (im - 1u)) & ((im & (im - 1u)) - 1u));
+    const uint32_t b0 = im & (0u - im);
+    auto share = [&](int d) -> double {
+        if (!(first2 & (1u << d))) return in_edge(A, c, m, d);
+        const int q = d + (d >> 2), di = (q * 11) >> 5;
+        return A.area[c + (di - 1) * m + (q - 3 * di - 1)] * (((b0 >> d) & 1u) ? wv.x : wv.y);
+    };
+    double xs[4];
+#pragma unroll
+    for (int q = 0; q < 4; q++) {
+        xs[q] = 0.0;
+        if (mm) { const int d = __ffs(mm) - 1; mm &= mm - 1u; xs[q] = share(d); }
+    }
+#pragma unroll
+    for (int q = 0; q < 4; q++) {
+        if constexpr (WT) K += xs[q];
+        else { K += fabs(xs[q]); td = td || (xs[q] < 0); }
+    }
+    while (mm) {
+        const int d = __ffs(mm) - 1; mm &= mm - 1u;
+        const double x = share(d);
+        if constexpr (WT) K += x;
+        else { K += fabs(x); td = td || (x < 0); }
+    }
+}
 
 struct TileBase {
-    const char *cinfo, *area, *contrib, *prop, *todo;
+    const char *cinfo, *area, *inw, *prop, *todo;
     int32_t org;
 };
 __device__ __forceinline__ TileBase tile_base(const SweepArgs &A, int i0, int j0)
@@ -503,7 +543,7 @@
     B.org = (int32_t)org;
     B.cinfo = reinterpret_cast<const char *>(A.cinfo) + org * 4;
     B.area = reinterpret_cast<const char *>(A.area) + org * 8;
-    B.contrib = reinterpret_cast<const char *>(A.contrib) + org * 16;
+    B.inw = reinterpret_cast<const char *>(A.inw) + org * 16;
     B.prop = reinterpret_cast<const char *>(A.prop) + org * 8;
     B.todo = reinterpret_cast<const char *>(A.todo_work) + org;
     return B;
@@ -514,23 +554,17 @@
 __device__ __forceinline__ void st_off(const char *base, uint32_t off, T v) { *reinterpret_cast<T *>(const_cast<char *>(base) + (size_t)off) = v; }
 __device__ __forceinline__ uint32_t halo_cell(int li, int lj, int m) { return __umul24((uint32_t)li, (uint32_t)m) + (uint32_t)lj; }
 
-__device__ __forceinline__ void fill_nbr16(int32_t *nbr16, int m)
+__device__ __forceinline__ void fill_nbr8(int32_t *nbr8, int m)
 {
     if (threadIdx.x < 8) {
         const int d = threadIdx.x, q = d + (d >> 2), di = q / 3, dj = q - 3 * di;
-        nbr16[d] = ((di - 1) * m + (dj - 1)) * 16 + (((0x5A >> d) & 1) ? 0 : 8);
-    }
-}
-__device__ __forceinline__ double in_edge_h(const TileBase &B, const int32_t *nbr16, uint32_t h, int d)
-{
-#ifdef PYDEM_EXP_AREAONLY
-    const uint32_t off16 = h * 16u + (uint32_t)nbr16[d];
-    const uint32_t uo = (off16 >> 4) * 8u;
-    const double ua = ld_off<double>(B.area, uo), up = ld_off<double>(B.prop, uo);
-    return (off16 & 8u) ? ua * (1 - up) : ua * up;
-#else
-    return ld_off<double>(B.contrib, h * 16u + (uint32_t)nbr16[d]);
-#endif
+        nbr8[d] = ((di - 1) * m + (dj - 1)) * 8;
+    }
+}
+__device__ __forceinline__ double in_weight_h(const TileBase &B, const int32_t *nbr8, uint32_t h, int d)
+{
+    const double up = ld_off<double>(B.prop, h * 8u + (uint32_t)nbr8[d]);
+    return ((0x5A >> d) & 1) ? up : 1 - up;
 }
 
 __device__ __forceinline__ void tile_stage(const SweepArgs &A, const TileBase &B, TileW &L, uint32_t pass, int i0, int j0, int lane,
@@ -595,7 +629,7 @@
 template <bool LISTED, bool WT = false>
 __device__ __forceinline__ void sweep_one_tile(const SweepArgs &A, TileW &L, uint32_t pass, int tiles_x, int tid, int lane,
                                                uint8_t *__restrict__ tile_done, int32_t &n_final, const TileNext &N,
-                                               int32_t *pend, int &npend, const int32_t *nbr16)
+                                               int32_t *pend, int &npend, const int32_t *nbr8)
 {
     const int by = tid / tiles_x, bx = tid - by * tiles_x;
     const int i0 = by * TH, j0 = bx * TT, n = A.n, m = A.m;
@@ -708,20 +742,26 @@
             const uint32_t h = halo_cell(li, lj, m);
             const int32_t c = B.org + (int32_t)h;
             const uint32_t cw = L.cs[idx] >> 16;
-            double pv = 0.0;
-            if (cw & (CI_OUT1 | CI_OUT2)) pv = ld_off<double>(B.prop, h * 8u);
+            uint32_t mm = cw & 0xFFu;
+            double2 wv = make_double2(0.0, 0.0);
+            if (mm) wv = ld_off<double2>(B.inw, h * 16u);
             int2 po = make_int2(0, 0);
             if (cw & (CI_PIT_IN | CI_PIT_OUT)) po = ld_off<int2>(B.area, h * 8u);
-            uint32_t mm = cw & 0xFFu;
-            double xs[4];
+            double ua[4], up[2] = {0.0, 0.0};
+            uint32_t card = 0;
 #pragma unroll
             for (int q = 0; q < 4; q++) {
-                xs[q] = 0.0;
+                ua[q] = 0.0;
                 if (mm) {
                     const int d = __ffs(mm) - 1; mm &= mm - 1u;
-                    if (d == cd) xs[q] = cv; else xs[q] = in_edge_h(B, nbr16, h, d);
+                    const uint32_t uo = h * 8u + (uint32_t)nbr8[d];
+                    if (d == cd) ua[q] = cv; else ua[q] = ld_off<double>(B.area, uo);
+                    if (q >= 2) { up[q - 2] = ld_off<double>(B.prop, uo); card |= (uint32_t)((0x5A >> d) & 1) << q; }
                 }
             }
+            double xs[4];
+            xs[0] = ua[0] * wv.x; xs[1] = ua[1] * wv.y;
+            xs[2] = ua[2] * ((card & 4u) ? up[0] : 1 - up[0]); xs[3] = ua[3] * ((card & 8u) ? up[1] : 1 - up[1]);
             double a;
             bool td;
             if constexpr (WT) {
@@ -737,24 +777,19 @@
             }
             while (mm) {
                 const int d = __ffs(mm) - 1; mm &= mm - 1u;
-                const double x = (d == cd) ? cv : in_edge_h(B, nbr16, h, d);
+                const double ua = (d == cd) ? cv : ld_off<double>(B.area, h * 8u + (uint32_t)nbr8[d]);
+                const double x = ua * in_weight_h(B, nbr8, h, d);
                 if constexpr (WT) a += x;
                 else { a += fabs(x); td = td || (x < 0); }
             }
             if (cw & CI_PIT_IN)
                 for (int32_t e = po.x; e < A.n_pit && A.pin_dst[e] == c; e++) {
                     const int32_t sc = A.pin_src[e];
-                    a += A.area[sc] * A.pin_w[e];
-                    if constexpr (!WT) td = td || (A.todo_work[sc] != 0);
+                    if constexpr (WT) a += A.area[sc] * A.pin_w[e];
+                    else { a += fabs(A.area[sc]) * A.pin_w[e]; td = td || (A.todo_work[sc] != 0); }
                 }
-            double2 o = make_double2(0.0, 0.0);
-            if (cw & CI_OUT1) o.x = a * pv;
-            if (cw & CI_OUT2) o.y = a * (1 - pv);
-            if (td) { o.x = -o.x; o.y = -o.y; }
-            st_off<double>(B.area, h * 8u, a);
-#ifndef PYDEM_EXP_NOCONTRIB
-            st_off<double2>(B.contrib, h * 16u, o);
-#endif
+            const double sa = td ? -a : a;
+            st_off<double>(B.area, h * 8u, sa);
             if (LISTED) st_off<uint32_t>(B.cinfo, h * 4u, ci_with_level(cw, pass));
             if (td) st_off<uint8_t>(B.todo, h, (uint8_t)1);
             sp_of(L, idx) = (uint16_t)(2u << SP_STATE_SHIFT);
@@ -778,8 +813,8 @@
                 }
             };
             const int sct = ci_section(cw);
-            if (cw & CI_OUT1) release(li + fe1r(sct), lj + fe1c(sct), o.x, true);
-            if (cw & CI_OUT2) release(li + fe2r(sct), lj + fe2c(sct), o.y, true);
+            if (cw & CI_OUT1) release(li + fe1r(sct), lj + fe1c(sct), sa, true);
+            if (cw & CI_OUT2) release(li + fe2r(sct), lj + fe2c(sct), sa, true);
             if (cw & CI_PIT_OUT)
                 for (int32_t e = po.y; e < A.n_pit && A.pit_src[e] == c; e++) {
                     const int32_t dc = A.pit_dst[e];
@@ -840,8 +875,8 @@
 {
     __shared__ TileW L[FWPB];
     __shared__ int32_t s_pend[FWPB][TILE_PEND];
-    __shared__ int32_t s_nbr16[8];
-    fill_nbr16(s_nbr16, A.m);
+    __shared__ int32_t s_nbr8[8];
+    fill_nbr8(s_nbr8, A.m);
     __syncthreads();
     const int wave = __builtin_amdgcn_readfirstlane(threadIdx.x >> 6), lane = threadIdx.x & 63;
     int32_t fin = 0;
@@ -860,7 +895,7 @@
     const int per4 = (gridDim.x >> 3) * 4;
     for (int tid = (blockIdx.x & 7) * per4 + (blockIdx.x >> 3) * 4 + wave, once = 0; once < 1; once++) {
         if (tid < tiles_total && !tile_done[tid])
-            sweep_one_tile<LISTED, WT>(A, L[wave], pass, tiles_x, tid, lane, tile_done, fin, N, s_pend[wave], npend, s_nbr16);
+            sweep_one_tile<LISTED, WT>(A, L[wave], pass, tiles_x, tid, lane, tile_done, fin, N, s_pend[wave], npend, s_nbr8);
     }
 #else
     const int per = (tiles_total + 7) >> 3;
@@ -873,7 +908,7 @@
             const int tid = xcd * per + q;
             if (q >= per || tid >= tiles_total) break;
             if (tile_done[tid]) continue;
-            sweep_one_tile<LISTED, WT>(A, L[wave], pass, tiles_x, tid, lane, tile_done, fin, N, s_pend[wave], npend, s_nbr16);
+            sweep_one_tile<LISTED, WT>(A, L[wave], pass, tiles_x, tid, lane, tile_done, fin, N, s_pend[wave], npend, s_nbr8);
             if (LISTED && npend > TILE_PEND - 10) flush();
         }
     }
@@ -903,8 +938,8 @@
 #endif
     if (blockIdx.x == 0 && threadIdx.x == 0) *clear_count = 0;
     __shared__ int32_t s_pend[LWPB][TILE_PEND];
-    __shared__ int32_t s_nbr16[8];
-    fill_nbr16(s_nbr16, A.m);
+    __shared__ int32_t s_nbr8[8];
+    fill_nbr8(s_nbr8, A.m);
     __syncthreads();
     int32_t fin = 0;
     int npend = 0;
@@ -935,7 +970,7 @@
         const int tid = __builtin_amdgcn_readfirstlane(list_in[k]);
         const uint32_t blk = Y.tile_sym ? __builtin_amdgcn_readfirstlane(Y.tile_sym[tid]) : SYM_NONE;
         if (blk != SYM_NONE) sym_light_visit<WT>(A, Y, SL[wave], pass, tiles_x, tid, lane, blk, fin, N, s_pend[wave], npend);
-        else sweep_one_tile<true, WT>(A, L[wave], pass, tiles_x, tid, lane, tile_done, fin, N, s_pend[wave], npend, s_nbr16);
+        else sweep_one_tile<true, WT>(A, L[wave], pass, tiles_x, tid, lane, tile_done, fin, N, s_pend[wave], npend, s_nbr8);
         if (npend > TILE_PEND - 10) flush();
     }
     if (npend) flush();
@@ -981,18 +1016,10 @@
         if (cw & CI_PIT_IN)
             for (int32_t e = po.x; e < A.n_pit && A.pin_dst[e] == c; e++) {
                 const int32_t sc = A.pin_src[e];
-                a += A.area[sc] * A.pin_w[e];
+                a += fabs(A.area[sc]) * A.pin_w[e];
                 td = td || (A.todo_work[sc] != 0);
             }
-        double2 o = make_double2(0.0, 0.0);
-        if (cw & (CI_OUT1 | CI_OUT2)) {
-            const double pv = A.prop[c];
-            if (cw & CI_OUT1) o.x = a * pv;
-            if (cw & CI_OUT2) o.y = a * (1 - pv);
-            if (td) { o.x = -o.x; o.y = -o.y; }
-        }
-        A.area[c] = a;
-        A.contrib[c] = o;
+        A.area[c] = td ? -a : a;
         A.cinfo[c] = ci_with_level(cw, p);
         if (td) A.todo_work[c] = 1;
         fin++;
@@ -1092,25 +1119,8 @@
         double pv = 0.0;
         if (cw & (CI_OUT1 | CI_OUT2)) pv = A.prop[c];
         bool td = !WT && (gi == 0 || gi == n - 1 || gj == 0 || gj == m - 1) && A.todo_work[c] != 0;
-        uint32_t mm = (smv >> RS_FINAL_SHIFT) & 0xFFu;
-        double xs[4];
-#pragma unroll
-        for (int q = 0; q < 4; q++) {
-            xs[q] = 0.0;
-            if (mm) { const int d = __ffs(mm) - 1; mm &= mm - 1u; xs[q] = in_edge(A, c, m, d); }
-        }
-        double K;
-        if constexpr (WT) {
-            K = A.a0[c];
-#pragma unroll
-            for (int q = 0; q < 4; q++) K += xs[q];
-            while (mm) { const int d = __ffs(mm) - 1; mm &= mm - 1u; K += in_edge(A, c, m, d); }
-        } else {
-            K = L.a0[cell >> 5];
-#pragma unroll
-            for (int q = 0; q < 4; q++) { K += fabs(xs[q]); td = td || (xs[q] < 0); }
-            while (mm) { const int d = __ffs(mm) - 1; mm &= mm - 1u; const double x = in_edge(A, c, m, d); K += fabs(x); td = td || (x < 0); }
-        }
+        double K = WT ? A.a0[c] : L.a0[cell >> 5];
+        gather_final_edges<WT>(A, c, m, cw & 0xFFu, (smv >> RS_FINAL_SHIFT) & 0xFFu, K, td);
         R.Kd[s] = K; R.Pd[s] = pv;
         R.sm[s] = (smv & RS_CELL_OPEN) | (td ? RS_TAINT : 0u);
     }
@@ -1146,7 +1156,8 @@
                     bool here = false;
                     if (si >= 0 && si < TH && sj >= 0 && sj < TT) here = sp_state(L, si * TT + sj) == 2u;
                     if (here) { const int ss = R.map[si * TT + sj]; a += R.Kd[ss] * A.pin_w[e]; td = td || (R.sm[ss] & RS_TAINT); }
-                    else { a += A.area[sc] * A.pin_w[e]; if constexpr (!WT) td = td || (A.todo_work[sc] != 0); }
+                    else if constexpr (WT) a += A.area[sc] * A.pin_w[e];
+                    else { a += fabs(A.area[sc]) * A.pin_w[e]; td = td || (A.todo_work[sc] != 0); }
                 }
             R.Kd[s] = a;
             R.sm[s] = (smv & RS_CELL) | (td ? RS_TAINT : 0u) | RS_FIN;
@@ -1183,13 +1194,9 @@
         const int cell = smv & RS_CELL;
         const int32_t c = (i0 + (cell >> 5)) * m + j0 + (cell & 31);
         const uint32_t cw = L.cs[cell] >> 16;
-        const double a = R.Kd[s], pv = R.Pd[s];
-        double2 o = make_double2(0.0, 0.0);
-        if (cw & CI_OUT1) o.x = a * pv;
-        if (cw & CI_OUT2) o.y = a * (1 - pv);
-        if (smv & RS_TAINT) { o.x = -o.x; o.y = -o.y; A.todo_work[c] = 1; }
-        A.area[c] = a;
-        A.contrib[c] = o;
+        const double a = R.Kd[s];
+        if (smv & RS_TAINT) A.todo_work[c] = 1;
+        A.area[c] = (smv & RS_TAINT) ? -a : a;
         A.cinfo[c] = ci_with_level(cw, pass);
         nfin++;
     }
@@ -1217,8 +1224,8 @@
     __shared__ TileR R;
     __shared__ SymLight SL;
     __shared__ int32_t s_pend[TILE_PEND];
-    __shared__ int32_t s_nbr16[8];
-    fill_nbr16(s_nbr16, A.m);
+    __shared__ int32_t s_nbr8[8];
+    fill_nbr8(s_nbr8, A.m);
     __syncthreads();
     const int lane = threadIdx.x;
     const int32_t nt = *n_in;
@@ -1241,7 +1248,7 @@
         else if (__builtin_amdgcn_readfirstlane(A.tile_open[tid]) <= RCAP)
             sweep_tile_resident<WT>(A, R, pass, tiles_x, tid, lane, tile_done, fin, N, s_pend, npend);
         else
-            sweep_one_tile<true, WT>(A, R.W, pass, tiles_x, tid, lane, tile_done, fin, N, s_pend, npend, s_nbr16);
+            sweep_one_tile<true, WT>(A, R.W, pass, tiles_x, tid, lane, tile_done, fin, N, s_pend, npend, s_nbr8);
         if (npend > TILE_PEND - 10) flush();
     }
     if (npend) flush();
@@ -1345,7 +1352,7 @@
                 if (td) { o.x = -o.x; o.y = -o.y; }
                 L.slot[cur] = o;
                 L.cs[cur] = word | FC_DONE | (td ? FC_TODO : 0u);
-                A.area[(int64_t)(i0 + r) * m + j0 + cl] = a;
+                A.area[(int64_t)(i0 + r) * m + j0 + cl] = td ? -a : a;
                 __builtin_amdgcn_fence(__ATOMIC_RELEASE, "workgroup", "local");
                 const int sct = ci_section(w);
                 int next = -1;
@@ -1371,7 +1378,6 @@
         if (!(word & FC_DONE)) continue;
         done |= 1u << k;
         const int64_t c = (int64_t)(i0 + 8 * k + r0) * m + gj;
-        A.contrib[c] = L.slot[t + 256 * k];
         A.cinfo[c] = ci_with_level(word >> 16, 1u);
         if (word & FC_TODO) A.todo_work[c] = 1;
     }
@@ -1475,8 +1481,7 @@
         if (cw & (1u << d)) {
             const int32_t u = c + NB_DI[d] * m + NB_DJ[d];
             if (ci_unfinished(A.cinfo[u])) continue;
-            const bool cardinal = (NB_DI[d] == 0) || (NB_DJ[d] == 0);
-            const double x = cardinal ? A.contrib[u].x : A.contrib[u].y;
+            const double x = in_edge(A, c, m, d);
             if constexpr (WT) a += x;
             else { a += fabs(x); td = td || (x < 0); }
         }
@@ -1484,8 +1489,8 @@
         for (int32_t e = pin_first; e < A.n_pit && A.pin_dst[e] == c; e++) {
             const int32_t sc = A.pin_src[e];
             if (ci_unfinished(A.cinfo[sc])) continue;
-            a += A.area[sc] * A.pin_w[e];
-            if constexpr (!WT) td = td || (A.todo_work[sc] != 0);
+            if constexpr (WT) a += A.area[sc] * A.pin_w[e];
+            else { a += fabs(A.area[sc]) * A.pin_w[e]; td = td || (A.todo_work[sc] != 0); }
         }
 }
 
@@ -1619,6 +1624,7 @@
                                               int apply_limit, double limit)
 {
     if (f) uca[c] = NAN;
+    else if (td) uca[c] = fabs(uca[c]);
     bool dn = !td;
     if (td && isnan(elev[c])) dn = true;
     if (apply_limit && !f && uca[c] > limit) dn = true;
@@ -1669,8 +1675,10 @@
     t->graph_opt = *opt;
     t->edge_clean = false;
     t->einc_ready = false;
+    t->inw_live = false;
     PYDEM_TRY(tile_alloc(t, &t->todo_work, (size_t)t->NN));
     PYDEM_TRY(tile_alloc(t, &t->cinfo, (size_t)t->NN));
+    if (!t->contrib) t->inw_wanted = false;
     const dim3 grid2((unsigned)(cdiv(m, 256) < 64 ? cdiv(m, 256) : 64), (unsigned)(n < 16384 ? n : 16384));
     t->tm.n_pit_edges = 0; t->tm.n_pits_undrained = 0; t->tm.pits_ms = 0;
     t->pits.n_edges = 0; t->pits.n_raw = 0;
@@ -1689,6 +1697,13 @@
     hipLaunchKernelGGL(k_graph_inmask, grid2, dim3(256), 0, t->stream2, t->prop, t->elev, n, m,
                        t->cinfo, t->edge_todo, t->todo_work, corner_sums);
     HIP_TRY(hipEventRecord(t->ev_join, t->stream2));
+    if (t->inw_wanted) {
+        HIP_TRY(hipStreamWaitEvent(t->stream3, t->ev_join, 0));
+        hipLaunchKernelGGL(k_graph_inweights, grid2, dim3(256), 0, t->stream3, (const uint32_t *)t->cinfo, (const double *)t->prop, n, m,
+                           (double2 *)t->contrib);
+        HIP_TRY(hipEventRecord(t->ev_inw, t->stream3));
+        t->inw_live = true;
+    }
     static int graph_serial = -1;
     if (graph_serial < 0) { const char *e = getenv("PYDEM_GRAPH_SERIAL"); graph_serial = e ? atoi(e) : 0; }
     if (graph_serial) HIP_TRY(hipStreamWaitEvent(t->stream, t->ev_join, 0));
@@ -1696,6 +1711,7 @@
     if (opt->drain_pits) PYDEM_TRY(stage_pits(t, opt));
     HIP_TRY(hipEventRecord(t->ev[2], t->stream));
     HIP_TRY(hipStreamWaitEvent(t->stream, t->ev_join, 0));
+    if (t->inw_live) HIP_TRY(hipStreamWaitEvent(t->stream, t->ev_inw, 0));
     const bool stash = t->pit_stash_live && t->uca != nullptr;
     t->pit_stash_live = false;
     if (t->pits.n_edges > 0) {
@@ -1813,6 +1829,11 @@
     SweepArgs A;
     fill_sweep_args(t, A);
     if (WT) { A.a0 = seed; A.area = t->uca_w; }
+    if (!t->inw_live) {
+        const dim3 grid2((unsigned)(cdiv(m, 256) < 64 ? cdiv(m, 256) : 64), (unsigned)(n < 16384 ? n : 16384));
+        hipLaunchKernelGGL(k_graph_inweights, grid2, dim3(256), 0, t->stream, (const uint32_t *)t->cinfo, (const double *)t->prop, n, m, A.inw);
+        t->inw_live = true;
+    }
     const bool stashed = !WT && t->pit_stash_live;
     if (!WT) t->pit_stash_live = false;
     if (A.n_pit > 0 && !stashed)
@@ -2006,6 +2027,7 @@
         int p_end = run_listed((int)pb + 3, t->h_counters[CS_TILE_LIST + (pb + 3) % 3], sym_on ? sym_switch : 0);
         if (sym_on && p_end > 0 && listed_left > 0) {
             const uint32_t ps = (uint32_t)p_end;
+            t->inw_live = false;
             TileNext N3; N3.flag = tile_flag; N3.list = tile_list[(ps + 1) % 2]; N3.count = &cntT[(ps + 1) % 3];
             HIP_TRY(hipMemsetAsync(&cntT[(ps + 2) % 3], 0, sizeof(int32_t), t->stream));
             int32_t *cand = tile_list[ps % 2];
diff --git a/pydem_amd/csrc/uca_edge.hip b/pydem_amd/csrc/uca_edge.hip
--- a/pydem_amd/csrc/uca_edge.hip
+++ b/pydem_amd/csrc/uca_edge.hip
@@ -949,6 +949,7 @@
     E.rlist = t->labels; E.rcount = t->counters + CS_EDGE_REACHED;
     E.tlist = t->flatlist; E.tcount = t->counters + CS_EDGE_CLEARED;
     PYDEM_TRY(tile_alloc(t, &t->contrib, (size_t)t->NN * 2));
+    t->inw_live = false;
     E.pit_off = reinterpret_cast<const int2 *>(t->contrib);
     if (!t->edge_clean) {
         if (A.n_pit > 0)
@@ -1052,6 +1053,7 @@
     PYDEM_TRY(tile_alloc(t, &t->queue[0], (size_t)t->NN));
     PYDEM_TRY(tile_alloc(t, &t->queue[1], (size_t)t->NN));
     PYDEM_TRY(tile_alloc(t, &t->contrib, (size_t)t->NN * 2));
+    t->inw_live = false;
     fill_sweep_args(t, E.G);
     E.flag = (uint32_t *)t->estamp; E.delta = t->edelta; E.flats = t->flats; E.edge_done = t->edge_done; E.edge_todo = t->edge_todo;
     E.uca = t->uca; E.pit_off = reinterpret_cast<const int2 *>(t->contrib); E.set_done = 1;
diff --git a/pydem_amd/csrc/uca_graph.h b/pydem_amd/csrc/uca_graph.h
--- a/pydem_amd/csrc/uca_graph.h
+++ b/pydem_amd/csrc/uca_graph.h
@@ -25,7 +25,7 @@
     uint32_t *cinfo;
     const double *prop, *a0;
     double *area;
-    double2 *contrib;
+    double2 *inw;
     uint8_t *todo_work;
     int n, m;
     const int32_t *pit_src, *pit_dst;
@@ -80,7 +80,7 @@
 static void fill_sweep_args(pydem_tile *t, SweepArgs &A)
 {
     A.cinfo = t->cinfo; A.prop = t->prop; A.a0 = t->row_area; A.area = t->uca;
-    A.contrib = (double2 *)t->contrib; A.todo_work = t->todo_work; A.n = (int)t->n; A.m = (int)t->m;
+    A.inw = (double2 *)t->contrib; A.todo_work = t->todo_work; A.n = (int)t->n; A.m = (int)t->m;
     A.pit_src = t->pits.src; A.pit_dst = t->pits.dst; A.n_pit = t->pits.n_edges;
     A.pin_dst = t->pits.in_dst; A.pin_src = t->pits.in_src; A.pin_w = t->pits.in_w;
     A.qcap = (int32_t)(t->NN / 2 < INT32_MAX ? t->NN / 2 : INT32_MAX);
```

Result: no change. 5764 (-0.8%).
